# c976237222/HunyuanVideo_efficiency

Hardware: AMD Instinct MI355X
Metric: denoise-steps/sec (720x1280x129f, HunyuanVideo DiT 20+40 blocks, bf16) (higher is better)
Workload: dtype bf16

## Files before the change

### hunyuanvideo_efficiency_amd/csrc/hv_attention.hip

```cpp
#include "hv_attention.hpp"

using namespace hv_attn;

namespace {

constexpr int QTILE = 256;

__global__ __launch_bounds__(256) void attn_combine_kernel(const float* __restrict__ part_o, const float* __restrict__ part_ml,
                                                            bf16_t* __restrict__ o, int64_t so, int n_q, int n_heads, int n_splits) {
    const int64_t idx = (int64_t)blockIdx.x * blockDim.x + threadIdx.x;
    const int64_t total = (int64_t)n_q * n_heads * 32;
    if (idx >= total) return;
    const int d4 = (int)(idx & 31);
    const int64_t rh = idx >> 5;
    const int head = (int)(rh % n_heads);
    const int64_t row = rh / n_heads;
    float m = -INFINITY;
    for (int s = 0; s < n_splits; ++s) m = fmaxf(m, part_ml[(((int64_t)s * n_q + row) * n_heads + head) * 2]);
    float4 acc = make_float4(0.f, 0.f, 0.f, 0.f);
    float l = 0.f;
    for (int s = 0; s < n_splits; ++s) {
        const int64_t ri = ((int64_t)s * n_q + row) * n_heads + head;
        const float w = __builtin_amdgcn_exp2f(part_ml[ri * 2] - m);
        const float4 v = *reinterpret_cast<const float4*>(part_o + ri * D + d4 * 4);
        acc.x += v.x * w; acc.y += v.y * w; acc.z += v.z * w; acc.w += v.w * w;
        l += part_ml[ri * 2 + 1] * w;
    }
    const float inv = 1.0f / l;
    u32x2 w2;
    w2[0] = pack_bf2(acc.x * inv, acc.y * inv);
    w2[1] = pack_bf2(acc.z * inv, acc.w * inv);
    *reinterpret_cast<u32x2*>(o + row * so + head * D + d4 * 4) = w2;
}

int attn_launch(const AttnArgs& a, dim3 grid, hipStream_t stream) { return launch_w4(a, grid, stream); }

constexpr int KMAX_ROWS = 2048;
__global__ __launch_bounds__(256) void attn_kmax_kernel(const bf16_t* __restrict__ k, int64_t sk, int n_kv, unsigned* __restrict__ out) {
    __shared__ float wmax[4];
    const int head = blockIdx.y, t = threadIdx.x, ch = t & 15;
    const int r0 = blockIdx.x * KMAX_ROWS, r1 = min(r0 + KMAX_ROWS, n_kv);
    float best = 0.f;
    for (int row = r0 + (t >> 4); row < r1; row += 16) {
        const u32x4 w = *reinterpret_cast<const u32x4*>(k + (int64_t)row * sk + head * D + ch * 8);
        float s = 0.f;
#pragma unroll
        for (int j = 0; j < 4; ++j) {
            const float lo = bf2f_lo(w[j]), hi = bf2f_hi(w[j]);
            s += lo * lo + hi * hi;
        }
#pragma unroll
        for (int o = 8; o > 0; o >>= 1) s += __shfl_xor(s, o, 64);
        best = fmaxf(best, s);
    }
    best = fmaxf(best, __shfl_xor(best, 16, 64));
    best = fmaxf(best, __shfl_xor(best, 32, 64));
    if ((t & 63) == 0) wmax[t >> 6] = best;
    __syncthreads();
    if (t == 0) atomicMax(out + head, __float_as_uint(fmaxf(fmaxf(wmax[0], wmax[1]), fmaxf(wmax[2], wmax[3]))));
}

int attn_prepare_kmax(AttnArgs& a, void* workspace, int64_t workspace_bytes, hipStream_t stream) {
    static_assert(HV_ATTN_BOUND_MIN_KV == 64 * KVT, "the pre-pass pays from 64 key tiles on");
    a.kmax2 = nullptr;
    if (!workspace || workspace_bytes < KMAX_BYTES || a.n_heads > KMAX_HEADS || a.n_kv < HV_ATTN_BOUND_MIN_KV) return HV_OK;
    if (hipMemsetAsync(workspace, 0, KMAX_BYTES, stream) != hipSuccess) return HV_ERR_LAUNCH;
    attn_kmax_kernel<<<dim3((unsigned)((a.n_kv + KMAX_ROWS - 1) / KMAX_ROWS), (unsigned)a.n_heads), dim3(256), 0, stream>>>(a.k, a.sk, a.n_kv, (unsigned*)workspace);
    a.kmax2 = (const unsigned*)workspace;
    return HV_OK;
}

int attn_kv_splits(int n_q, int n_kv, int n_heads) {
    const int64_t nwg = (int64_t)((n_q + QTILE - 1) / QTILE) * n_heads;
    const int ntile = (n_kv + KVT - 1) / KVT;
    const double r1 = (double)((nwg + 255) / 256), r2 = 0.5 * (double)((2 * nwg + 255) / 256);
    return (ntile >= 64 && r2 < 0.97 * r1) ? 2 : 1;
}

}

extern "C" int64_t hv_attn_workspace_bytes(int n_q, int n_kv, int n_heads) {
    (void)n_kv;
    return (int64_t)KMAX_BYTES + (int64_t)2 * n_q * n_heads * (128 + 2) * (int64_t)sizeof(float);
}

extern "C" int hv_attn_fwd_bf16(const void* q, const void* k, const void* v, void* o, int64_t stride_q, int64_t stride_k,
                                int64_t stride_v, int64_t stride_o, int n_q, int n_kv, int n_heads, int head_dim,
                                float scale, void* workspace, int64_t workspace_bytes, hipStream_t stream) {
    if (!q || !k || !v || !o || head_dim != D || n_heads <= 0 || n_q < 0 || n_kv < 0 || (stride_q & 7) || (stride_k & 7) ||
        (stride_v & 7) || (stride_o & 3))
        return HV_ERR_ARG;
    if (n_q == 0) return HV_OK;
    if (n_kv == 0) return HV_ERR_ARG;
    AttnArgs a;
    a.q = (const bf16_t*)q; a.k = (const bf16_t*)k; a.v = (const bf16_t*)v; a.o = (bf16_t*)o;
    a.sq = stride_q; a.sk = stride_k; a.sv = stride_v; a.so = stride_o;
    a.n_q = n_q; a.n_kv = n_kv; a.n_heads = n_heads;
    a.n_qtiles = (n_q + QTILE - 1) / QTILE;
    a.scale_log2e = scale * 1.4426950408889634f;
    a.n_splits = 1; a.split_keys = n_kv; a.part_o = nullptr; a.part_ml = nullptr; a.partial = 0;
    if (attn_prepare_kmax(a, workspace, workspace_bytes, stream) != HV_OK) return HV_ERR_LAUNCH;
    if (workspace && attn_kv_splits(n_q, n_kv, n_heads) == 2 && workspace_bytes >= hv_attn_workspace_bytes(n_q, n_kv, n_heads)) {
        a.n_splits = 2;
        a.split_keys = (((n_kv + KVT - 1) / KVT + 1) / 2) * KVT;
        a.part_o = (float*)((char*)workspace + KMAX_BYTES);
        a.part_ml = a.part_o + (int64_t)2 * n_q * n_heads * D;
    }
    if (attn_launch(a, dim3((unsigned)(a.n_qtiles * n_heads), (unsigned)a.n_splits), stream) != HV_OK) return HV_ERR_LAUNCH;
    if (a.n_splits > 1) {
        const int64_t total = (int64_t)n_q * n_heads * 32;
        attn_combine_kernel<<<dim3((unsigned)((total + 255) / 256)), dim3(256), 0, stream>>>(a.part_o, a.part_ml, a.o, a.so, n_q, n_heads,
                                                                                           a.n_splits);
    }
    return hv_check_launch();
}

extern "C" int hv_attn_partial_bf16(const void* q, const void* k, const void* v, int64_t stride_q, int64_t stride_k, int64_t stride_v,
                                    int n_q, int n_kv, int n_heads, int head_dim, float scale, void* part_o, void* part_ml,
                                    int n_slots, int slot, int splits, hipStream_t stream) {
    if (!q || !k || !v || !part_o || !part_ml || head_dim != D || n_heads <= 0 || n_q < 0 || n_kv <= 0 || (stride_q & 7) ||
        (stride_k & 7) || (stride_v & 7) || (splits != 1 && splits != 2) || slot < 0 || slot + splits > n_slots)
        return HV_ERR_ARG;
    if (n_q == 0) return HV_OK;
    const int ntile = (n_kv + KVT - 1) / KVT;
    if (splits == 2 && ntile < 2) return HV_ERR_ARG;
    AttnArgs a;
    a.q = (const bf16_t*)q; a.k = (const bf16_t*)k; a.v = (const bf16_t*)v; a.o = nullptr;
    a.sq = stride_q; a.sk = stride_k; a.sv = stride_v; a.so = 0;
    a.n_q = n_q; a.n_kv = n_kv; a.n_heads = n_heads;
    a.n_qtiles = (n_q + QTILE - 1) / QTILE;
    a.scale_log2e = scale * 1.4426950408889634f;
    a.n_splits = splits;
    a.split_keys = splits == 2 ? ((ntile + 1) / 2) * KVT : n_kv;
    a.part_o = (float*)part_o + (int64_t)slot * n_q * n_heads * D;
    a.part_ml = (float*)part_ml + (int64_t)slot * n_q * n_heads * 2;
    a.partial = 1;
    a.kmax2 = nullptr;
    if (attn_launch(a, dim3((unsigned)(a.n_qtiles * n_heads), (unsigned)splits), stream) != HV_OK) return HV_ERR_LAUNCH;
    return hv_check_launch();
}

extern "C" int hv_attn_merge_bf16(const void* part_o, const void* part_ml, void* o, int64_t stride_o, int n_q, int n_heads, int n_slots,
                                  hipStream_t stream) {
    if (!part_o || !part_ml || !o || n_heads <= 0 || n_q < 0 || n_slots <= 0 || (stride_o & 3)) return HV_ERR_ARG;
    if (n_q == 0) return HV_OK;
    const int64_t total = (int64_t)n_q * n_heads * 32;
    attn_combine_kernel<<<dim3((unsigned)((total + 255) / 256)), dim3(256), 0, stream>>>((const float*)part_o, (const float*)part_ml,
                                                                                       (bf16_t*)o, stride_o, n_q, n_heads, n_slots);
    return hv_check_launch();
}

extern "C" int hv_attn_suggest_splits(int n_q, int n_kv, int n_heads) { return attn_kv_splits(n_q, n_kv, n_heads); }
```

### hunyuanvideo_efficiency_amd/csrc/hv_attention.hpp

```cpp
#pragma once
#include "hv_common.hpp"
#include "../../include/hv_kernels.h"
#include <type_traits>

namespace hv_attn {

constexpr int D = 128;
constexpr int KVT = 64;
constexpr int KV_TILE_BYTES = KVT * D * 2;

struct AttnArgs {
    const bf16_t* q; const bf16_t* k; const bf16_t* v; bf16_t* o;
    int64_t sq, sk, sv, so;
    int n_q, n_kv, n_heads, n_qtiles;
    float scale_log2e;
    int n_splits, split_keys;
    float* part_o;
    float* part_ml;
    int partial;
    const unsigned* kmax2;
};
constexpr int KMAX_BYTES = HV_ATTN_MIN_WORKSPACE_BYTES;
constexpr int KMAX_HEADS = 62;

typedef __attribute__((ext_vector_type(4))) short s16x4;
typedef __attribute__((address_space(3))) s16x4* lds_s16x4_ptr;
typedef __attribute__((address_space(3))) void* lds_void_ptr;

__device__ __forceinline__ float half_swap_max(float v) {
    auto r = __builtin_amdgcn_permlane32_swap(__float_as_uint(v), __float_as_uint(v), false, false);
    return fmaxf(__uint_as_float(r[0]), __uint_as_float(r[1]));
}
__device__ __forceinline__ float half_swap_sum(float v) {
    auto r = __builtin_amdgcn_permlane32_swap(__float_as_uint(v), __float_as_uint(v), false, false);
    return __uint_as_float(r[0]) + __uint_as_float(r[1]);
}

template <int I, int N, typename F>
__device__ __forceinline__ void static_for(F&& f) {
    if constexpr (I < N) {
        f(std::integral_constant<int, I>{});
        static_for<I + 1, N>(f);
    }
}

int launch_w4(const AttnArgs& a, dim3 grid, hipStream_t stream);

}
```

### hunyuanvideo_efficiency_amd/csrc/hv_common.hpp

```cpp
#pragma once
#include <hip/hip_runtime.h>
#include <stdint.h>

#define HV_OK 0
#define HV_ERR_ARG (-1)
#define HV_ERR_LAUNCH (-2)

typedef __attribute__((ext_vector_type(8))) __bf16 bf16x8;
typedef __attribute__((ext_vector_type(4))) __bf16 bf16x4;
typedef __attribute__((ext_vector_type(2))) __bf16 bf16x2;
typedef __attribute__((ext_vector_type(4))) float f32x4;
typedef __attribute__((ext_vector_type(16))) float f32x16;
typedef __attribute__((ext_vector_type(4))) uint32_t u32x4;
typedef __attribute__((ext_vector_type(2))) uint32_t u32x2;
typedef __attribute__((ext_vector_type(2))) float f32x2;

typedef uint16_t bf16_t;

__device__ __forceinline__ float bf2f(bf16_t v) { return __uint_as_float(((uint32_t)v) << 16); }
__device__ __forceinline__ float bf2f_lo(uint32_t w) { return __uint_as_float(w << 16); }
__device__ __forceinline__ float bf2f_hi(uint32_t w) { return __uint_as_float(w & 0xFFFF0000u); }
__device__ __forceinline__ bf16_t f2bf(float f) {
    __bf16 h = (__bf16)f;
    return __builtin_bit_cast(bf16_t, h);
}
__device__ __forceinline__ uint32_t pack_bf2(float lo, float hi) {
    bf16x2 v;
    v[0] = (__bf16)lo;
    v[1] = (__bf16)hi;
    return __builtin_bit_cast(uint32_t, v);
}
__device__ __forceinline__ float rbf(float f) { return bf2f(f2bf(f)); }

__device__ __forceinline__ void unpack8(const u32x4& w, float (&f)[8]) {
#pragma unroll
    for (int i = 0; i < 4; ++i) {
        f[2 * i] = bf2f_lo(w[i]);
        f[2 * i + 1] = bf2f_hi(w[i]);
    }
}
__device__ __forceinline__ u32x4 pack8(const float (&f)[8]) {
    u32x4 w;
#pragma unroll
    for (int i = 0; i < 4; ++i) w[i] = pack_bf2(f[2 * i], f[2 * i + 1]);
    return w;
}

typedef _Float16 h16;
__device__ __forceinline__ float h2f(uint16_t v) { return (float)__builtin_bit_cast(h16, v); }
__device__ __forceinline__ uint16_t f2h(float f) { return __builtin_bit_cast(uint16_t, (h16)f); }
__device__ __forceinline__ float rh(float f) { return (float)(h16)f; }
__device__ __forceinline__ void unpack8h(const u32x4& w, float (&f)[8]) {
#pragma unroll
    for (int i = 0; i < 4; ++i) {
        f[2 * i] = h2f((uint16_t)(w[i] & 0xFFFFu));
        f[2 * i + 1] = h2f((uint16_t)(w[i] >> 16));
    }
}
__device__ __forceinline__ u32x4 pack8h(const float (&f)[8]) {
    u32x4 w;
#pragma unroll
    for (int i = 0; i < 4; ++i) w[i] = (uint32_t)f2h(f[2 * i]) | ((uint32_t)f2h(f[2 * i + 1]) << 16);
    return w;
}

template <typename T, typename Op>
__device__ __forceinline__ T wave_reduce(T v, Op op) {
#pragma unroll
    for (int o = 32; o > 0; o >>= 1) v = op(v, __shfl_xor(v, o, 64));
    return v;
}
struct WaveAdd {
    template <typename T> __device__ __forceinline__ T operator()(T a, T b) const { return a + b; }
};
struct WaveMax {
    __device__ __forceinline__ float operator()(float a, float b) const { return fmaxf(a, b); }
    __device__ __forceinline__ int operator()(int a, int b) const { return max(a, b); }
};
struct WaveMin {
    __device__ __forceinline__ int operator()(int a, int b) const { return min(a, b); }
};
template <typename T> __device__ __forceinline__ T wave_sum(T v) { return wave_reduce(v, WaveAdd{}); }
template <typename T> __device__ __forceinline__ T wave_max(T v) { return wave_reduce(v, WaveMax{}); }
template <typename T> __device__ __forceinline__ T wave_min(T v) { return wave_reduce(v, WaveMin{}); }

__device__ __forceinline__ float gelu_tanh_f(float x) {
    const float k0 = 0.7978845608028654f, k1 = 0.044715f;
    float u = k0 * (x + k1 * x * x * x);
    float e = __builtin_amdgcn_exp2f(u * 2.8853900817779268f);
    float t = 1.0f - 2.0f * __builtin_amdgcn_rcpf(e + 1.0f);
    return 0.5f * x * (1.0f + t);
}
__device__ __forceinline__ float silu_f(float x) { return x * __builtin_amdgcn_rcpf(1.0f + __expf(-x)); }

__device__ __forceinline__ uint32_t quantise(float x, int rescale) {
    if (rescale) x = __fmul_rn(__fadd_rn(x, 1.0f), 0.5f);
    x = fminf(fmaxf(x, 0.0f), 1.0f);
    return (uint32_t)(int)__fmul_rn(x, 255.0f);
}

namespace f32tile {
constexpr int kThreads = 256;
constexpr int BM = 128, BN = 64, BK = 32;
constexpr int LDA = BM + 2;

__device__ __forceinline__ void mma_chunk(const float* sA, const float* sB, int wm, int wn, int lr, int lk, f32x16& acc0, f32x16& acc1) {
#pragma unroll
    for (int ks = 0; ks < BK / 2; ++ks) {
        const int k = ks * 2 + lk;
        const float a0 = sA[k * LDA + wm + lr], a1 = sA[k * LDA + wm + 32 + lr];
        const float b = sB[k * BN + wn + lr];
        acc0 = __builtin_amdgcn_mfma_f32_32x32x2f32(a0, b, acc0, 0, 0, 0);
        acc1 = __builtin_amdgcn_mfma_f32_32x32x2f32(a1, b, acc1, 0, 0, 0);
    }
}
__device__ __forceinline__ int acc_row(int r, int lk) { return (r & 3) + 8 * (r >> 2) + 4 * lk; }
}

static inline bool hv_aligned16(const void* p) { return ((uintptr_t)p & 15) == 0; }

struct HvPerDeviceOnce { bool done[64] = {}; };
static inline int hv_set_max_lds(HvPerDeviceOnce& once, const void* fn, int bytes) {
    int dev = 0;
    if (hipGetDevice(&dev) != hipSuccess || dev < 0 || dev >= 64) return HV_ERR_LAUNCH;
    if (!once.done[dev]) {
        if (hipFuncSetAttribute(fn, hipFuncAttributeMaxDynamicSharedMemorySize, bytes) != hipSuccess) return HV_ERR_LAUNCH;
        once.done[dev] = true;
    }
    return HV_OK;
}

static inline int hv_check_launch() {
    hipError_t e = hipGetLastError();
    return e == hipSuccess ? HV_OK : HV_ERR_LAUNCH;
}

__device__ __forceinline__ f32x2 f16x2_minus(uint32_t w, float plo, float phi) {
    float lo, hi;
    asm("v_fma_mix_f32 %0, %1, 1.0, -%2 op_sel_hi:[1,0,0]" : "=v"(lo) : "v"(w), "v"(plo));
    asm("v_fma_mix_f32 %0, %1, 1.0, -%2 op_sel:[1,0,0] op_sel_hi:[1,0,0]" : "=v"(hi) : "v"(w), "v"(phi));
    return f32x2{lo, hi};
}
```

### hunyuanvideo_efficiency_amd/csrc/hv_rowwise.hip

```cpp
#include "hv_common.hpp"
#include "../../include/hv_kernels.h"
#include <type_traits>


template <int MAXC>
__device__ __forceinline__ float ln_load_row(const bf16_t* xr, int lane, int nchunk, float (&v)[MAXC][8]) {
    float s = 0.f;
#pragma unroll
    for (int c = 0; c < MAXC; ++c) {
        const int ch = lane + c * 64;
        if (ch < nchunk) {
            unpack8(*reinterpret_cast<const u32x4*>(xr + ch * 8), v[c]);
#pragma unroll
            for (int j = 0; j < 8; ++j) s += v[c][j];
        }
    }
    return s;
}
__device__ __forceinline__ void ln_load_coeffs(const bf16_t* mul, const bf16_t* add, int ch, int mode,
                                               float (&m)[8], float (&a)[8]) {
    if (mul) {
        unpack8(*reinterpret_cast<const u32x4*>(mul + ch * 8), m);
        if (mode == 0) {
#pragma unroll
            for (int j = 0; j < 8; ++j) m[j] = rbf(1.0f + m[j]);
        }
    } else {
#pragma unroll
        for (int j = 0; j < 8; ++j) m[j] = 1.0f;
    }
    if (add) {
        unpack8(*reinterpret_cast<const u32x4*>(add + ch * 8), a);
    } else {
#pragma unroll
        for (int j = 0; j < 8; ++j) a[j] = 0.0f;
    }
}

template <int MAXC>
__global__ __launch_bounds__(256) void ln_mod_kernel(const bf16_t* __restrict__ x, const bf16_t* __restrict__ add,
                                                      const bf16_t* __restrict__ mul, bf16_t* __restrict__ out,
                                                      int64_t M, int D, int64_t ldx, int64_t ldo, float eps, int mode) {
    const int lane = threadIdx.x & 63;
    const int64_t row = (int64_t)blockIdx.x * 4 + (threadIdx.x >> 6);
    if (row >= M) return;
    const int nchunk = D >> 3;
    float v[MAXC][8];
    const float mean = wave_sum(ln_load_row<MAXC>(x + row * ldx, lane, nchunk, v)) / (float)D;
    float q = 0.f;
#pragma unroll
    for (int c = 0; c < MAXC; ++c) {
        const int ch = lane + c * 64;
        if (ch < nchunk) {
#pragma unroll
            for (int j = 0; j < 8; ++j) {
                float d = v[c][j] - mean;
                q += d * d;
            }
        }
    }
    const float rstd = rsqrtf(wave_sum(q) / (float)D + eps);
    bf16_t* orow = out + row * ldo;
#pragma unroll
    for (int c = 0; c < MAXC; ++c) {
        const int ch = lane + c * 64;
        if (ch < nchunk) {
            float m[8], a[8], o[8];
            ln_load_coeffs(mul, add, ch, mode, m, a);
#pragma unroll
            for (int j = 0; j < 8; ++j) o[j] = (v[c][j] - mean) * rstd * m[j] + a[j];
            *reinterpret_cast<u32x4*>(orow + ch * 8) = pack8(o);
        }
    }
}

template <typename Launch>
static inline void ln_dispatch_maxc(int D, Launch launch) {
    if (D <= 512)
        launch(std::integral_constant<int, 1>{});
    else if (D <= 2048)
        launch(std::integral_constant<int, 4>{});
    else if (D <= 3072)
        launch(std::integral_constant<int, 6>{});
    else
        launch(std::integral_constant<int, 8>{});
}

extern "C" int hv_ln_modulate_bf16(const void* x, const void* shift_or_bias, const void* scale_or_weight, void* out,
                                   int64_t M, int D, int64_t ldx, int64_t ldo, float eps, int mode, hipStream_t stream) {
    if (!x || !out || M < 0 || D <= 0 || (D & 7) || D > 4096 || (ldx & 7) || (ldo & 7) || (mode != 0 && mode != 1))
        return HV_ERR_ARG;
    if (M == 0) return HV_OK;
    dim3 grid((unsigned)((M + 3) / 4)), block(256);
    const bf16_t *xp = (const bf16_t*)x, *ap = (const bf16_t*)shift_or_bias, *mp = (const bf16_t*)scale_or_weight;
    ln_dispatch_maxc(D, [&](auto maxc) {
        ln_mod_kernel<decltype(maxc)::value><<<grid, block, 0, stream>>>(xp, ap, mp, (bf16_t*)out, M, D, ldx, ldo, eps, mode);
    });
    return hv_check_launch();
}

__device__ __forceinline__ uint32_t pack4_fp8(float a, float b, float c, float d) {
    uint32_t w = 0;
    w = __builtin_amdgcn_cvt_pk_fp8_f32(a, b, w, false);
    w = __builtin_amdgcn_cvt_pk_fp8_f32(c, d, w, true);
    return w;
}
constexpr float HV_FP8_MIN_ROW_SCALE = 1.17549435e-38f;
__device__ __forceinline__ float fp8_row_scale(float amax) {
    return amax > 0.f ? fmaxf(amax * (1.0f / 448.0f), HV_FP8_MIN_ROW_SCALE) : 1.0f;
}
__device__ __forceinline__ float clamp448(float v) { return __builtin_amdgcn_fmed3f(v, -448.0f, 448.0f); }
__device__ __forceinline__ u32x2 pack8_fp8(const float (&v)[8], float inv) {
    u32x2 w;
    w[0] = pack4_fp8(clamp448(v[0] * inv), clamp448(v[1] * inv), clamp448(v[2] * inv), clamp448(v[3] * inv));
    w[1] = pack4_fp8(clamp448(v[4] * inv), clamp448(v[5] * inv), clamp448(v[6] * inv), clamp448(v[7] * inv));
    return w;
}
template <int MAXC>
__global__ __launch_bounds__(256) void ln_mod_fp8_kernel(const bf16_t* __restrict__ x, const bf16_t* __restrict__ add,
                                                          const bf16_t* __restrict__ mul, uint8_t* __restrict__ out,
                                                          float* __restrict__ row_scale, int64_t M, int D, int64_t ldx,
                                                          int64_t ldo, float eps) {
    const int lane = threadIdx.x & 63;
    const int64_t row = (int64_t)blockIdx.x * 4 + (threadIdx.x >> 6);
    if (row >= M) return;
    const int nchunk = D >> 3;
    float v[MAXC][8];
    const float mean = wave_sum(ln_load_row<MAXC>(x + row * ldx, lane, nchunk, v)) / (float)D;
    float q = 0.f;
#pragma unroll
    for (int c = 0; c < MAXC; ++c) {
        const int ch = lane + c * 64;
        if (ch < nchunk) {
#pragma unroll
            for (int j = 0; j < 8; ++j) {
                float d = v[c][j] - mean;
                q += d * d;
            }
        }
    }
    const float rstd = rsqrtf(wave_sum(q) / (float)D + eps);
    float amax = 0.f;
#pragma unroll
    for (int c = 0; c < MAXC; ++c) {
        const int ch = lane + c * 64;
        if (ch < nchunk) {
            float m[8], a[8];
            ln_load_coeffs(mul, add, ch, 0, m, a);
#pragma unroll
            for (int j = 0; j < 8; ++j) {
                v[c][j] = rbf((v[c][j] - mean) * rstd * m[j] + a[j]);
                amax = fmaxf(amax, fabsf(v[c][j]));
            }
        }
    }
    const float sc = fp8_row_scale(wave_max(amax));
    const float inv = 1.0f / sc;
    if (lane == 0) row_scale[row] = sc;
    uint8_t* orow = out + row * ldo;
#pragma unroll
    for (int c = 0; c < MAXC; ++c) {
        const int ch = lane + c * 64;
        if (ch < nchunk) *reinterpret_cast<u32x2*>(orow + ch * 8) = pack8_fp8(v[c], inv);
    }
}

extern "C" int hv_ln_modulate_fp8(const void* x, const void* shift, const void* scale, void* out_q, float* out_row_scale, int64_t M,
                                  int D, int64_t ldx, int64_t ldq, float eps, hipStream_t stream) {
    if (!x || !out_q || !out_row_scale || M < 0 || D <= 0 || (D & 7) || D > 4096 || (ldx & 7) || (ldq & 15)) return HV_ERR_ARG;
    if (M == 0) return HV_OK;
    dim3 grid((unsigned)((M + 3) / 4)), block(256);
    const bf16_t *xp = (const bf16_t*)x, *ap = (const bf16_t*)shift, *mp = (const bf16_t*)scale;
    ln_dispatch_maxc(D, [&](auto maxc) {
        ln_mod_fp8_kernel<decltype(maxc)::value><<<grid, block, 0, stream>>>(xp, ap, mp, (uint8_t*)out_q, out_row_scale, M, D, ldx, ldq, eps);
    });
    return hv_check_launch();
}

__global__ __launch_bounds__(256) void quant_rows_fp8_kernel(const bf16_t* __restrict__ x, int64_t ldx, uint8_t* __restrict__ out,
                                                              int64_t ldo, float* __restrict__ row_scale, int64_t M, int K) {
    const int lane = threadIdx.x & 63;
    const int64_t row = (int64_t)blockIdx.x * 4 + (threadIdx.x >> 6);
    if (row >= M) return;
    const bf16_t* xr = x + row * ldx;
    const int nchunk = K >> 3;
    float amax = 0.f;
    for (int ch = lane; ch < nchunk; ch += 64) {
        float f[8];
        unpack8(*reinterpret_cast<const u32x4*>(xr + ch * 8), f);
#pragma unroll
        for (int j = 0; j < 8; ++j) amax = fmaxf(amax, fabsf(f[j]));
    }
    const float sc = fp8_row_scale(wave_max(amax));
    const float inv = 1.0f / sc;
    if (lane == 0) row_scale[row] = sc;
    uint8_t* orow = out + row * ldo;
    for (int ch = lane; ch < nchunk; ch += 64) {
        float f[8];
        unpack8(*reinterpret_cast<const u32x4*>(xr + ch * 8), f);
        *reinterpret_cast<u32x2*>(orow + ch * 8) = pack8_fp8(f, inv);
    }
}

extern "C" int hv_quant_rows_fp8(const void* x, int64_t ldx, void* out_q, int64_t ldq, float* out_row_scale, int64_t M, int K,
                                 hipStream_t stream) {
    if (!x || !out_q || !out_row_scale || M < 0 || K <= 0 || (K & 7) || (ldx & 7) || (ldq & 15)) return HV_ERR_ARG;
    if (M == 0) return HV_OK;
    quant_rows_fp8_kernel<<<dim3((unsigned)((M + 3) / 4)), dim3(256), 0, stream>>>((const bf16_t*)x, ldx, (uint8_t*)out_q, ldq,
                                                                                  out_row_scale, M, K);
    return hv_check_launch();
}

__global__ __launch_bounds__(256) void qknorm_rope_kernel(bf16_t* __restrict__ qkv, const bf16_t* __restrict__ qw,
                                                           const bf16_t* __restrict__ kw, const float* __restrict__ cosT,
                                                           const float* __restrict__ sinT, int64_t n_rows, int64_t n_rope,
                                                           int H, int64_t ld, int64_t k_off, float eps, bf16_t* __restrict__ dst,
                                                           int64_t dst_ld, int hpb, int64_t dst_bs) {
    const int64_t row = blockIdx.x;
    const int sub = threadIdx.x & 15;
    const int grp = threadIdx.x >> 4;
    float wq[8], wk[8], c[8], s[8];
    unpack8(*reinterpret_cast<const u32x4*>(qw + sub * 8), wq);
    unpack8(*reinterpret_cast<const u32x4*>(kw + sub * 8), wk);
    const bool rope = row < n_rope;
    if (rope) {
        const float4* cp = reinterpret_cast<const float4*>(cosT + row * 128 + sub * 8);
        const float4* sp = reinterpret_cast<const float4*>(sinT + row * 128 + sub * 8);
        float4 c0 = cp[0], c1 = cp[1], s0 = sp[0], s1 = sp[1];
        c[0] = c0.x, c[1] = c0.y, c[2] = c0.z, c[3] = c0.w, c[4] = c1.x, c[5] = c1.y, c[6] = c1.z, c[7] = c1.w;
        s[0] = s0.x, s[1] = s0.y, s[2] = s0.z, s[3] = s0.w, s[4] = s1.x, s[5] = s1.y, s[6] = s1.z, s[7] = s1.w;
    }
    for (int hv = grp; hv < 2 * H; hv += 16) {
        const bool is_k = hv >= H;
        const int h = is_k ? hv - H : hv;
        bf16_t* p = qkv + row * ld + (is_k ? k_off : 0) + h * 128 + sub * 8;
        float x[8];
        unpack8(*reinterpret_cast<const u32x4*>(p), x);
        if (dst) p = dst + (int64_t)(hv / hpb) * dst_bs + row * dst_ld + (hv % hpb) * 128 + sub * 8;
        float ss = 0.f;
#pragma unroll
        for (int j = 0; j < 8; ++j) ss += x[j] * x[j];
#pragma unroll
        for (int o = 8; o > 0; o >>= 1) ss += __shfl_xor(ss, o, 16);
        const float r = rsqrtf(ss * (1.0f / 128.0f) + eps);
        float y[8];
#pragma unroll
        for (int j = 0; j < 8; ++j) y[j] = rbf(rbf(x[j] * r) * (is_k ? wk[j] : wq[j]));
        if (rope) {
            float o[8];
#pragma unroll
            for (int j = 0; j < 8; j += 2) {
                o[j] = y[j] * c[j] - y[j + 1] * s[j];
                o[j + 1] = y[j + 1] * c[j + 1] + y[j] * s[j + 1];
            }
            *reinterpret_cast<u32x4*>(p) = pack8(o);
        } else {
            *reinterpret_cast<u32x4*>(p) = pack8(y);
        }
    }
}

extern "C" int hv_qknorm_rope_bf16(void* qkv, const void* q_weight, const void* k_weight, const float* cos_tab,
                                   const float* sin_tab, int64_t n_rows, int64_t n_rope, int n_heads, int head_dim,
                                   int64_t ld, int64_t k_offset, float eps, hipStream_t stream) {
    if (!qkv || !q_weight || !k_weight || head_dim != 128 || n_heads <= 0 || n_rows < 0 || n_rope < 0 ||
        n_rope > n_rows || (ld & 7) || (k_offset & 7) || (n_rope > 0 && (!cos_tab || !sin_tab)))
        return HV_ERR_ARG;
    if (n_rows == 0) return HV_OK;
    qknorm_rope_kernel<<<dim3((unsigned)n_rows), dim3(256), 0, stream>>>((bf16_t*)qkv, (const bf16_t*)q_weight,
                                                                          (const bf16_t*)k_weight, cos_tab, sin_tab, n_rows,
                                                                          n_rope, n_heads, ld, k_offset, eps, nullptr, 0, 1, 0);
    return hv_check_launch();
}

extern "C" int hv_qknorm_rope_scatter_bf16(const void* qkv, const void* q_weight, const void* k_weight, const float* cos_tab,
                                           const float* sin_tab, int64_t n_rows, int64_t n_rope, int n_heads, int head_dim,
                                           int64_t ld, int64_t k_offset, float eps, void* dst, int64_t dst_ld,
                                           int heads_per_block, int64_t dst_block_stride, hipStream_t stream) {
    if (!qkv || !dst || !q_weight || !k_weight || head_dim != 128 || n_heads <= 0 || n_rows < 0 || n_rope < 0 || n_rope > n_rows ||
        (ld & 7) || (k_offset & 7) || (dst_ld & 7) || (dst_block_stride & 7) || heads_per_block <= 0 ||
        (n_rope > 0 && (!cos_tab || !sin_tab)))
        return HV_ERR_ARG;
    if (n_rows == 0) return HV_OK;
    qknorm_rope_kernel<<<dim3((unsigned)n_rows), dim3(256), 0, stream>>>((bf16_t*)const_cast<void*>(qkv), (const bf16_t*)q_weight,
                                                                          (const bf16_t*)k_weight, cos_tab, sin_tab, n_rows, n_rope,
                                                                          n_heads, ld, k_offset, eps, (bf16_t*)dst, dst_ld,
                                                                          heads_per_block, dst_block_stride);
    return hv_check_launch();
}

template <int MM>
__global__ __launch_bounds__(256) void gemv_kernel(const bf16_t* __restrict__ x, const bf16_t* __restrict__ W,
                                                    const bf16_t* __restrict__ b, const bf16_t* __restrict__ addend,
                                                    bf16_t* __restrict__ out, int N, int K, int64_t ldx, int64_t ldo, int act) {
    const int lane = threadIdx.x & 63;
    const int n = blockIdx.x * 4 + (threadIdx.x >> 6);
    if (n >= N) return;
    float acc[MM];
#pragma unroll
    for (int m = 0; m < MM; ++m) acc[m] = 0.f;
    const bf16_t* wr = W + (int64_t)n * K;
    for (int k0 = lane * 8; k0 < K; k0 += 512) {
        float w[8];
        unpack8(*reinterpret_cast<const u32x4*>(wr + k0), w);
#pragma unroll
        for (int m = 0; m < MM; ++m) {
            float xv[8];
            unpack8(*reinterpret_cast<const u32x4*>(x + m * ldx + k0), xv);
#pragma unroll
            for (int j = 0; j < 8; ++j) {
                float a = xv[j];
                if (act & 1) a = rbf(silu_f(a));
                acc[m] += a * w[j];
            }
        }
    }
#pragma unroll
    for (int m = 0; m < MM; ++m) {
        float r = wave_sum(acc[m]);
        if (lane == 0) {
            if (b) r += bf2f(b[n]);
            if (act & 2) r = silu_f(rbf(r));
            if (addend) r = rbf(r) + bf2f(addend[m * ldo + n]);
            out[m * ldo + n] = f2bf(r);
        }
    }
}

extern "C" int hv_linear_smallm_bf16(const void* x, const void* W, const void* bias, const void* addend, void* out, int M,
                                     int N, int K, int64_t ldx, int64_t ldo, int act, hipStream_t stream) {
    if (!x || !W || !out || M < 1 || M > 4 || N < 1 || K < 8 || (K & 7) || (ldx & 7)) return HV_ERR_ARG;
    dim3 grid((N + 3) / 4), block(256);
    const bf16_t *xp = (const bf16_t*)x, *wp = (const bf16_t*)W, *bp = (const bf16_t*)bias, *ap = (const bf16_t*)addend;
    bf16_t* op = (bf16_t*)out;
    switch (M) {
        case 1: gemv_kernel<1><<<grid, block, 0, stream>>>(xp, wp, bp, ap, op, N, K, ldx, ldo, act); break;
        case 2: gemv_kernel<2><<<grid, block, 0, stream>>>(xp, wp, bp, ap, op, N, K, ldx, ldo, act); break;
        case 3: gemv_kernel<3><<<grid, block, 0, stream>>>(xp, wp, bp, ap, op, N, K, ldx, ldo, act); break;
        default: gemv_kernel<4><<<grid, block, 0, stream>>>(xp, wp, bp, ap, op, N, K, ldx, ldo, act); break;
    }
    return hv_check_launch();
}

__global__ __launch_bounds__(256) void patchify_kernel(const float* __restrict__ x, bf16_t* __restrict__ A, int C, int T,
                                                        int H, int W) {
    const int Hp = H >> 1, Wp = W >> 1;
    const int64_t ntok = (int64_t)T * Hp * Wp;
    const int64_t idx = (int64_t)blockIdx.x * blockDim.x + threadIdx.x;
    if (idx >= ntok * C) return;
    const int c = (int)(idx % C);
    const int64_t tok = idx / C;
    const int w = (int)(tok % Wp), h = (int)((tok / Wp) % Hp), t = (int)(tok / ((int64_t)Wp * Hp));
    const float* p = x + (((int64_t)c * T + t) * H + 2 * h) * W + 2 * w;
    float2 r0 = *reinterpret_cast<const float2*>(p);
    float2 r1 = *reinterpret_cast<const float2*>(p + W);
    u32x2 o;
    o[0] = pack_bf2(r0.x, r0.y);
    o[1] = pack_bf2(r1.x, r1.y);
    *reinterpret_cast<u32x2*>(A + tok * (C * 4) + c * 4) = o;
}

extern "C" int hv_patchify_f32_bf16(const float* x, void* A, int C, int T, int H, int W, hipStream_t stream) {
    if (!x || !A || C <= 0 || T <= 0 || H <= 0 || W <= 0 || (H & 1) || (W & 1)) return HV_ERR_ARG;
    const int64_t n = (int64_t)T * (H / 2) * (W / 2) * C;
    patchify_kernel<<<dim3((unsigned)((n + 255) / 256)), dim3(256), 0, stream>>>(x, (bf16_t*)A, C, T, H, W);
    return hv_check_launch();
}

__global__ __launch_bounds__(256) void unpatchify_kernel(const bf16_t* __restrict__ y, bf16_t* __restrict__ out, int C,
                                                          int T, int H, int W, int64_t ldy) {
    const int Hp = H >> 1, Wp = W >> 1;
    const int64_t ntok = (int64_t)T * Hp * Wp;
    const int64_t idx = (int64_t)blockIdx.x * blockDim.x + threadIdx.x;
    if (idx >= ntok * C) return;
    const int64_t tok = idx % ntok;
    const int c = (int)(idx / ntok);
    const int w = (int)(tok % Wp), h = (int)((tok / Wp) % Hp), t = (int)(tok / ((int64_t)Wp * Hp));
    u32x2 v = *reinterpret_cast<const u32x2*>(y + tok * ldy + c * 4);
    bf16_t* p = out + (((int64_t)c * T + t) * H + 2 * h) * W + 2 * w;
    *reinterpret_cast<uint32_t*>(p) = v[0];
    *reinterpret_cast<uint32_t*>(p + W) = v[1];
}

extern "C" int hv_unpatchify_bf16(const void* y, void* out, int C, int T, int H, int W, int64_t ldy, hipStream_t stream) {
    if (!y || !out || C <= 0 || T <= 0 || (H & 1) || (W & 1) || (ldy & 3)) return HV_ERR_ARG;
    const int64_t n = (int64_t)T * (H / 2) * (W / 2) * C;
    unpatchify_kernel<<<dim3((unsigned)((n + 255) / 256)), dim3(256), 0, stream>>>((const bf16_t*)y, (bf16_t*)out, C, T, H,
                                                                                  W, ldy);
    return hv_check_launch();
}

__global__ __launch_bounds__(256) void euler_kernel(float* __restrict__ s, const bf16_t* __restrict__ v, float dt, int64_t n) {
    const int64_t i = ((int64_t)blockIdx.x * blockDim.x + threadIdx.x) * 4;
    if (i + 3 < n) {
        float4 a = *reinterpret_cast<float4*>(s + i);
        u32x2 w = *reinterpret_cast<const u32x2*>(v + i);
        a.x += bf2f_lo(w[0]) * dt, a.y += bf2f_hi(w[0]) * dt, a.z += bf2f_lo(w[1]) * dt, a.w += bf2f_hi(w[1]) * dt;
        *reinterpret_cast<float4*>(s + i) = a;
    } else {
        for (int64_t j = i; j < n; ++j) s[j] += bf2f(v[j]) * dt;
    }
}

extern "C" int hv_euler_step_f32(float* sample, const void* model_out_bf16, float dt, int64_t n, hipStream_t stream) {
    if (!sample || !model_out_bf16 || n < 0) return HV_ERR_ARG;
    if (n == 0) return HV_OK;
    euler_kernel<<<dim3((unsigned)((n / 4 + 256) / 256)), dim3(256), 0, stream>>>(sample, (const bf16_t*)model_out_bf16, dt, n);
    return hv_check_launch();
}

__global__ __launch_bounds__(256) void euler_f32_kernel(float* __restrict__ s, const float* __restrict__ v, float dt, int64_t n) {
    const int64_t i = ((int64_t)blockIdx.x * blockDim.x + threadIdx.x) * 4;
    if (i + 3 < n) {
        float4 a = *reinterpret_cast<float4*>(s + i);
        const float4 b = *reinterpret_cast<const float4*>(v + i);
        a.x += b.x * dt, a.y += b.y * dt, a.z += b.z * dt, a.w += b.w * dt;
        *reinterpret_cast<float4*>(s + i) = a;
    } else {
        for (int64_t j = i; j < n; ++j) s[j] += v[j] * dt;
    }
}

extern "C" int hv_euler_step_f32_f32(float* sample, const float* model_out_f32, float dt, int64_t n, hipStream_t stream) {
    if (!sample || !model_out_f32 || n < 0) return HV_ERR_ARG;
    if (n == 0) return HV_OK;
    euler_f32_kernel<<<dim3((unsigned)((n / 4 + 256) / 256)), dim3(256), 0, stream>>>(sample, model_out_f32, dt, n);
    return hv_check_launch();
}

__global__ __launch_bounds__(256) void masked_mean_kernel(const bf16_t* __restrict__ x, const int* __restrict__ mask,
                                                           bf16_t* __restrict__ out, int L, int D) {
    const int d = blockIdx.x * blockDim.x + threadIdx.x;
    if (d >= D) return;
    float s = 0.f, c = 0.f;
    for (int l = 0; l < L; ++l) {
        const float m = mask ? (float)mask[l] : 1.0f;
        s += bf2f(x[(int64_t)l * D + d]) * m;
        c += m;
    }
    out[d] = f2bf(s / c);
}

extern "C" int hv_masked_mean_bf16(const void* x, const int* mask, void* out, int L, int D, hipStream_t stream) {
    if (!x || !out || L <= 0 || D <= 0) return HV_ERR_ARG;
    masked_mean_kernel<<<dim3((D + 255) / 256), dim3(256), 0, stream>>>((const bf16_t*)x, mask, (bf16_t*)out, L, D);
    return hv_check_launch();
}

__global__ __launch_bounds__(256) void bcast_row_kernel(const bf16_t* __restrict__ src, bf16_t* __restrict__ dst, int64_t n,
                                                         int D, int64_t ld) {
    const int64_t i = (int64_t)blockIdx.x * blockDim.x + threadIdx.x;
    if (i >= n * D) return;
    dst[(i / D) * ld + (i % D)] = src[i % D];
}

extern "C" int hv_broadcast_row_bf16(const void* src, void* dst, int64_t n_rows, int D, int64_t ld, hipStream_t stream) {
    if (!src || !dst || n_rows < 0 || D <= 0) return HV_ERR_ARG;
    if (n_rows == 0) return HV_OK;
    bcast_row_kernel<<<dim3((unsigned)((n_rows * D + 255) / 256)), dim3(256), 0, stream>>>((const bf16_t*)src, (bf16_t*)dst,
                                                                                          n_rows, D, ld);
    return hv_check_launch();
}

__global__ void timestep_embedding_kernel(const float* __restrict__ t, bf16_t* __restrict__ out, int n_t, int dim, float max_period) {
    const int half = dim >> 1;
    const int idx = blockIdx.x * blockDim.x + threadIdx.x;
    if (idx >= n_t * half) return;
    const int b = idx / half, i = idx % half;
    const float f = expf(-logf(max_period) * (float)i / (float)half);
    const float a = t[b] * f;
    out[b * dim + i] = f2bf(cosf(a));
    out[b * dim + half + i] = f2bf(sinf(a));
}

extern "C" int hv_timestep_embedding_bf16(const float* t, void* out, int n_t, int dim, float max_period, hipStream_t stream) {
    if (!t || !out || n_t <= 0 || dim <= 0 || (dim & 1)) return HV_ERR_ARG;
    const int n = n_t * (dim / 2);
    timestep_embedding_kernel<<<dim3((n + 127) / 128), dim3(128), 0, stream>>>(t, (bf16_t*)out, n_t, dim, max_period);
    return hv_check_launch();
}

__global__ __launch_bounds__(256) void copy3d_kernel(const bf16_t* __restrict__ src, bf16_t* __restrict__ dst, int rows,
                                                      int cvec, int64_t src_bs, int64_t src_ld, int64_t dst_bs, int64_t dst_ld) {
    const int b = blockIdx.z;
    const int64_t total = (int64_t)rows * cvec;
    for (int64_t i = (int64_t)blockIdx.x * blockDim.x + threadIdx.x; i < total; i += (int64_t)gridDim.x * blockDim.x) {
        const int64_t r = i / cvec;
        const int c = (int)(i % cvec) * 8;
        *reinterpret_cast<u32x4*>(dst + b * dst_bs + r * dst_ld + c) =
            *reinterpret_cast<const u32x4*>(src + b * src_bs + r * src_ld + c);
    }
}

extern "C" int hv_copy3d_bf16(const void* src, void* dst, int n_batch, int64_t rows, int cols, int64_t src_batch_stride,
                              int64_t src_ld, int64_t dst_batch_stride, int64_t dst_ld, hipStream_t stream) {
    if (!src || !dst || n_batch < 0 || rows < 0 || cols <= 0 || (cols & 7) || (src_ld & 7) || (dst_ld & 7) ||
        (src_batch_stride & 7) || (dst_batch_stride & 7) || rows > 0x7fffffff)
        return HV_ERR_ARG;
    if (n_batch == 0 || rows == 0) return HV_OK;
    const int64_t total = rows * (cols / 8);
    const unsigned gx = (unsigned)((total + 255) / 256 > 4096 ? 4096 : (total + 255) / 256);
    copy3d_kernel<<<dim3(gx, 1, (unsigned)n_batch), dim3(256), 0, stream>>>((const bf16_t*)src, (bf16_t*)dst, (int)rows, cols / 8,
                                                                            src_batch_stride, src_ld, dst_batch_stride, dst_ld);
    return hv_check_launch();
}

__device__ __forceinline__ float e4m3fn_to_f32(uint32_t b) {
    const uint32_t s = (b & 0x80u) << 24, e = (b >> 3) & 0xFu, m = b & 7u;
    float v;
    if (e == 0) v = (float)m * 0.001953125f;
    else if (e == 15 && m == 7) v = __uint_as_float(0x7FC00000u);
    else v = __uint_as_float(((e + 120u) << 23) | (m << 20));
    return __uint_as_float(__float_as_uint(v) | s);
}

__global__ __launch_bounds__(256) void fp8_dequant_kernel(const uint8_t* __restrict__ w8, const bf16_t* __restrict__ scale,
                                                           bf16_t* __restrict__ out, int64_t n) {
    const float sc = bf2f(scale[0]);
    for (int64_t i = ((int64_t)blockIdx.x * blockDim.x + threadIdx.x) * 8; i < n; i += (int64_t)gridDim.x * blockDim.x * 8) {
        if (i + 8 <= n) {
            const u32x2 p = *reinterpret_cast<const u32x2*>(w8 + i);
            float f[8];
#pragma unroll
            for (int j = 0; j < 8; ++j) f[j] = e4m3fn_to_f32((p[j >> 2] >> ((j & 3) * 8)) & 0xFFu) * sc;
            *reinterpret_cast<u32x4*>(out + i) = pack8(f);
        } else {
            for (int64_t j = i; j < n; ++j) out[j] = f2bf(e4m3fn_to_f32(w8[j]) * sc);
        }
    }
}

extern "C" int hv_fp8_dequant_bf16(const void* w_e4m3fn, const void* scale_bf16, void* out_bf16, int64_t n, hipStream_t stream) {
    if (!w_e4m3fn || !scale_bf16 || !out_bf16 || n <= 0 || (n & 7)) return HV_ERR_ARG;
    const int64_t nv = n / 8;
    const unsigned gx = (unsigned)((nv + 255) / 256 > 16384 ? 16384 : (nv + 255) / 256);
    fp8_dequant_kernel<<<dim3(gx), dim3(256), 0, stream>>>((const uint8_t*)w_e4m3fn, (const bf16_t*)scale_bf16, (bf16_t*)out_bf16, n);
    return hv_check_launch();
}
```

### hunyuanvideo_efficiency_amd/csrc/hv_torch_ops.cpp

```cpp
#include <torch/library.h>
#include <ATen/core/Tensor.h>
#include <c10/hip/HIPStream.h>
#include <c10/hip/HIPGuard.h>
#include <optional>
#include <vector>
#include "../../include/hv_kernels.h"

namespace {
using OptT = std::optional<at::Tensor>;

struct Dev {
    c10::DeviceIndex idx = -1;
    const char* op;
    explicit Dev(const char* o) : op(o) {}
    void* p(const OptT& t, const char* name) {
        if (!t.has_value() || !t->defined()) return nullptr;
        TORCH_CHECK(t->is_cuda(), "hv::", op, ": ", name, " must be a GPU tensor (this library has no CPU path), got ", t->device());
        if (idx < 0) idx = t->device().index();
        TORCH_CHECK(t->device().index() == idx, "hv::", op, ": ", name, " is on a different GPU than the other tensors");
        return t->data_ptr();
    }
};

inline void check_rc(int rc, const char* op) {
    TORCH_CHECK(rc == 0, "hv::", op, " failed with code ", rc, rc == -1 ? " (bad argument)" : rc == -2 ? " (launch failure)" : "");
}

int64_t op_abi_version() {
    return (int64_t)hv_abi_version();
}

void op_ln_modulate_bf16(const OptT& x, const OptT& shift_or_bias, const OptT& scale_or_weight, const OptT& out, int64_t M, int64_t D, int64_t ldx, int64_t ldo, double eps, int64_t mode) {
    Dev dev("ln_modulate_bf16");
    auto a0 = (const void*)dev.p(x, "x");
    auto a1 = (const void*)dev.p(shift_or_bias, "shift_or_bias");
    auto a2 = (const void*)dev.p(scale_or_weight, "scale_or_weight");
    auto a3 = (void*)dev.p(out, "out");
    TORCH_CHECK(dev.idx >= 0, "hv::ln_modulate_bf16: needs at least one GPU tensor");
    c10::hip::HIPGuard guard(dev.idx);
    hipStream_t stream = c10::hip::getCurrentHIPStream(dev.idx).stream();
    check_rc(hv_ln_modulate_bf16(a0, a1, a2, a3, (int64_t)M, (int)D, (int64_t)ldx, (int64_t)ldo, (float)eps, (int)mode, stream), "ln_modulate_bf16");
}

void op_qknorm_rope_bf16(const OptT& qkv, const OptT& q_weight, const OptT& k_weight, const OptT& cos_tab, const OptT& sin_tab, int64_t n_rows, int64_t n_rope, int64_t n_heads, int64_t head_dim, int64_t ld, int64_t k_offset, double eps) {
    Dev dev("qknorm_rope_bf16");
    auto a0 = (void*)dev.p(qkv, "qkv");
    auto a1 = (const void*)dev.p(q_weight, "q_weight");
    auto a2 = (const void*)dev.p(k_weight, "k_weight");
    auto a3 = (const float*)dev.p(cos_tab, "cos_tab");
    auto a4 = (const float*)dev.p(sin_tab, "sin_tab");
    TORCH_CHECK(dev.idx >= 0, "hv::qknorm_rope_bf16: needs at least one GPU tensor");
    c10::hip::HIPGuard guard(dev.idx);
    hipStream_t stream = c10::hip::getCurrentHIPStream(dev.idx).stream();
    check_rc(hv_qknorm_rope_bf16(a0, a1, a2, a3, a4, (int64_t)n_rows, (int64_t)n_rope, (int)n_heads, (int)head_dim, (int64_t)ld, (int64_t)k_offset, (float)eps, stream), "qknorm_rope_bf16");
}

void op_qknorm_rope_scatter_bf16(const OptT& qkv, const OptT& q_weight, const OptT& k_weight, const OptT& cos_tab, const OptT& sin_tab, int64_t n_rows, int64_t n_rope, int64_t n_heads, int64_t head_dim, int64_t ld, int64_t k_offset, double eps, const OptT& dst, int64_t dst_ld, int64_t heads_per_block, int64_t dst_block_stride) {
    Dev dev("qknorm_rope_scatter_bf16");
    auto a0 = (const void*)dev.p(qkv, "qkv");
    auto a1 = (const void*)dev.p(q_weight, "q_weight");
    auto a2 = (const void*)dev.p(k_weight, "k_weight");
    auto a3 = (const float*)dev.p(cos_tab, "cos_tab");
    auto a4 = (const float*)dev.p(sin_tab, "sin_tab");
    auto a12 = (void*)dev.p(dst, "dst");
    TORCH_CHECK(dev.idx >= 0, "hv::qknorm_rope_scatter_bf16: needs at least one GPU tensor");
    c10::hip::HIPGuard guard(dev.idx);
    hipStream_t stream = c10::hip::getCurrentHIPStream(dev.idx).stream();
    check_rc(hv_qknorm_rope_scatter_bf16(a0, a1, a2, a3, a4, (int64_t)n_rows, (int64_t)n_rope, (int)n_heads, (int)head_dim, (int64_t)ld, (int64_t)k_offset, (float)eps, a12, (int64_t)dst_ld, (int)heads_per_block, (int64_t)dst_block_stride, stream), "qknorm_rope_scatter_bf16");
}

void op_gemm_bf16(const OptT& A, int64_t lda, const OptT& W, int64_t ldw, const OptT& bias, int64_t M, int64_t N, int64_t K, const OptT& out0, int64_t ld0, int64_t act0, int64_t n_split, const OptT& out1, int64_t ld1, int64_t act1, const OptT& gate, const OptT& res, int64_t ld_res) {
    Dev dev("gemm_bf16");
    auto a0 = (const void*)dev.p(A, "A");
    auto a2 = (const void*)dev.p(W, "W");
    auto a4 = (const void*)dev.p(bias, "bias");
    auto a8 = (void*)dev.p(out0, "out0");
    auto a12 = (void*)dev.p(out1, "out1");
    auto a15 = (const void*)dev.p(gate, "gate");
    auto a16 = (const void*)dev.p(res, "res");
    TORCH_CHECK(dev.idx >= 0, "hv::gemm_bf16: needs at least one GPU tensor");
    c10::hip::HIPGuard guard(dev.idx);
    hipStream_t stream = c10::hip::getCurrentHIPStream(dev.idx).stream();
    check_rc(hv_gemm_bf16(a0, (int64_t)lda, a2, (int64_t)ldw, a4, (int)M, (int)N, (int)K, a8, (int64_t)ld0, (int)act0, (int)n_split, a12, (int64_t)ld1, (int)act1, a15, a16, (int64_t)ld_res, stream), "gemm_bf16");
}

void op_linear_smallm_bf16(const OptT& x, const OptT& W, const OptT& bias, const OptT& addend, const OptT& out, int64_t M, int64_t N, int64_t K, int64_t ldx, int64_t ldo, int64_t act) {
    Dev dev("linear_smallm_bf16");
    auto a0 = (const void*)dev.p(x, "x");
    auto a1 = (const void*)dev.p(W, "W");
    auto a2 = (const void*)dev.p(bias, "bias");
    auto a3 = (const void*)dev.p(addend, "addend");
    auto a4 = (void*)dev.p(out, "out");
    TORCH_CHECK(dev.idx >= 0, "hv::linear_smallm_bf16: needs at least one GPU tensor");
    c10::hip::HIPGuard guard(dev.idx);
    hipStream_t stream = c10::hip::getCurrentHIPStream(dev.idx).stream();
    check_rc(hv_linear_smallm_bf16(a0, a1, a2, a3, a4, (int)M, (int)N, (int)K, (int64_t)ldx, (int64_t)ldo, (int)act, stream), "linear_smallm_bf16");
}

void op_timestep_embedding_bf16(const OptT& t, const OptT& out, int64_t n_t, int64_t dim, double max_period) {
    Dev dev("timestep_embedding_bf16");
    auto a0 = (const float*)dev.p(t, "t");
    auto a1 = (void*)dev.p(out, "out");
    TORCH_CHECK(dev.idx >= 0, "hv::timestep_embedding_bf16: needs at least one GPU tensor");
    c10::hip::HIPGuard guard(dev.idx);
    hipStream_t stream = c10::hip::getCurrentHIPStream(dev.idx).stream();
    check_rc(hv_timestep_embedding_bf16(a0, a1, (int)n_t, (int)dim, (float)max_period, stream), "timestep_embedding_bf16");
}

void op_attn_fwd_bf16(const OptT& q, const OptT& k, const OptT& v, const OptT& o, int64_t stride_q, int64_t stride_k, int64_t stride_v, int64_t stride_o, int64_t n_q, int64_t n_kv, int64_t n_heads, int64_t head_dim, double scale, const OptT& workspace, int64_t workspace_bytes) {
    Dev dev("attn_fwd_bf16");
    auto a0 = (const void*)dev.p(q, "q");
    auto a1 = (const void*)dev.p(k, "k");
    auto a2 = (const void*)dev.p(v, "v");
    auto a3 = (void*)dev.p(o, "o");
    auto a13 = (void*)dev.p(workspace, "workspace");
    TORCH_CHECK(dev.idx >= 0, "hv::attn_fwd_bf16: needs at least one GPU tensor");
    c10::hip::HIPGuard guard(dev.idx);
    hipStream_t stream = c10::hip::getCurrentHIPStream(dev.idx).stream();
    check_rc(hv_attn_fwd_bf16(a0, a1, a2, a3, (int64_t)stride_q, (int64_t)stride_k, (int64_t)stride_v, (int64_t)stride_o, (int)n_q, (int)n_kv, (int)n_heads, (int)head_dim, (float)scale, a13, (int64_t)workspace_bytes, stream), "attn_fwd_bf16");
}

int64_t op_attn_workspace_bytes(int64_t n_q, int64_t n_kv, int64_t n_heads) {
    return (int64_t)hv_attn_workspace_bytes((int)n_q, (int)n_kv, (int)n_heads);
}

int64_t op_attn_w4_loop_signature() {
    return (int64_t)hv_attn_w4_loop_signature();
}

void op_attn_partial_bf16(const OptT& q, const OptT& k, const OptT& v, int64_t stride_q, int64_t stride_k, int64_t stride_v, int64_t n_q, int64_t n_kv, int64_t n_heads, int64_t head_dim, double scale, const OptT& part_o, const OptT& part_ml, int64_t n_slots, int64_t slot, int64_t splits) {
    Dev dev("attn_partial_bf16");
    auto a0 = (const void*)dev.p(q, "q");
    auto a1 = (const void*)dev.p(k, "k");
    auto a2 = (const void*)dev.p(v, "v");
    auto a11 = (void*)dev.p(part_o, "part_o");
    auto a12 = (void*)dev.p(part_ml, "part_ml");
    TORCH_CHECK(dev.idx >= 0, "hv::attn_partial_bf16: needs at least one GPU tensor");
    c10::hip::HIPGuard guard(dev.idx);
    hipStream_t stream = c10::hip::getCurrentHIPStream(dev.idx).stream();
    check_rc(hv_attn_partial_bf16(a0, a1, a2, (int64_t)stride_q, (int64_t)stride_k, (int64_t)stride_v, (int)n_q, (int)n_kv, (int)n_heads, (int)head_dim, (float)scale, a11, a12, (int)n_slots, (int)slot, (int)splits, stream), "attn_partial_bf16");
}

void op_attn_merge_bf16(const OptT& part_o, const OptT& part_ml, const OptT& o, int64_t stride_o, int64_t n_q, int64_t n_heads, int64_t n_slots) {
    Dev dev("attn_merge_bf16");
    auto a0 = (const void*)dev.p(part_o, "part_o");
    auto a1 = (const void*)dev.p(part_ml, "part_ml");
    auto a2 = (void*)dev.p(o, "o");
    TORCH_CHECK(dev.idx >= 0, "hv::attn_merge_bf16: needs at least one GPU tensor");
    c10::hip::HIPGuard guard(dev.idx);
    hipStream_t stream = c10::hip::getCurrentHIPStream(dev.idx).stream();
    check_rc(hv_attn_merge_bf16(a0, a1, a2, (int64_t)stride_o, (int)n_q, (int)n_heads, (int)n_slots, stream), "attn_merge_bf16");
}

int64_t op_attn_suggest_splits(int64_t n_q, int64_t n_kv, int64_t n_heads) {
    return (int64_t)hv_attn_suggest_splits((int)n_q, (int)n_kv, (int)n_heads);
}

void op_patchify_f32_bf16(const OptT& x, const OptT& A, int64_t C, int64_t T, int64_t H, int64_t W) {
    Dev dev("patchify_f32_bf16");
    auto a0 = (const float*)dev.p(x, "x");
    auto a1 = (void*)dev.p(A, "A");
    TORCH_CHECK(dev.idx >= 0, "hv::patchify_f32_bf16: needs at least one GPU tensor");
    c10::hip::HIPGuard guard(dev.idx);
    hipStream_t stream = c10::hip::getCurrentHIPStream(dev.idx).stream();
    check_rc(hv_patchify_f32_bf16(a0, a1, (int)C, (int)T, (int)H, (int)W, stream), "patchify_f32_bf16");
}

void op_unpatchify_bf16(const OptT& y, const OptT& out, int64_t C, int64_t T, int64_t H, int64_t W, int64_t ldy) {
    Dev dev("unpatchify_bf16");
    auto a0 = (const void*)dev.p(y, "y");
    auto a1 = (void*)dev.p(out, "out");
    TORCH_CHECK(dev.idx >= 0, "hv::unpatchify_bf16: needs at least one GPU tensor");
    c10::hip::HIPGuard guard(dev.idx);
    hipStream_t stream = c10::hip::getCurrentHIPStream(dev.idx).stream();
    check_rc(hv_unpatchify_bf16(a0, a1, (int)C, (int)T, (int)H, (int)W, (int64_t)ldy, stream), "unpatchify_bf16");
}

void op_euler_step_f32(const OptT& sample, const OptT& model_out_bf16, double dt, int64_t n) {
    Dev dev("euler_step_f32");
    auto a0 = (float*)dev.p(sample, "sample");
    auto a1 = (const void*)dev.p(model_out_bf16, "model_out_bf16");
    TORCH_CHECK(dev.idx >= 0, "hv::euler_step_f32: needs at least one GPU tensor");
    c10::hip::HIPGuard guard(dev.idx);
    hipStream_t stream = c10::hip::getCurrentHIPStream(dev.idx).stream();
    check_rc(hv_euler_step_f32(a0, a1, (float)dt, (int64_t)n, stream), "euler_step_f32");
}

void op_euler_step_f32_f32(const OptT& sample, const OptT& model_out_f32, double dt, int64_t n) {
    Dev dev("euler_step_f32_f32");
    auto a0 = (float*)dev.p(sample, "sample");
    auto a1 = (const float*)dev.p(model_out_f32, "model_out_f32");
    TORCH_CHECK(dev.idx >= 0, "hv::euler_step_f32_f32: needs at least one GPU tensor");
    c10::hip::HIPGuard guard(dev.idx);
    hipStream_t stream = c10::hip::getCurrentHIPStream(dev.idx).stream();
    check_rc(hv_euler_step_f32_f32(a0, a1, (float)dt, (int64_t)n, stream), "euler_step_f32_f32");
}

void op_masked_mean_bf16(const OptT& x, const OptT& mask, const OptT& out, int64_t L, int64_t D) {
    Dev dev("masked_mean_bf16");
    auto a0 = (const void*)dev.p(x, "x");
    auto a1 = (const int*)dev.p(mask, "mask");
    auto a2 = (void*)dev.p(out, "out");
    TORCH_CHECK(dev.idx >= 0, "hv::masked_mean_bf16: needs at least one GPU tensor");
    c10::hip::HIPGuard guard(dev.idx);
    hipStream_t stream = c10::hip::getCurrentHIPStream(dev.idx).stream();
    check_rc(hv_masked_mean_bf16(a0, a1, a2, (int)L, (int)D, stream), "masked_mean_bf16");
}

void op_broadcast_row_bf16(const OptT& src, const OptT& dst, int64_t n_rows, int64_t D, int64_t ld) {
    Dev dev("broadcast_row_bf16");
    auto a0 = (const void*)dev.p(src, "src");
    auto a1 = (void*)dev.p(dst, "dst");
    TORCH_CHECK(dev.idx >= 0, "hv::broadcast_row_bf16: needs at least one GPU tensor");
    c10::hip::HIPGuard guard(dev.idx);
    hipStream_t stream = c10::hip::getCurrentHIPStream(dev.idx).stream();
    check_rc(hv_broadcast_row_bf16(a0, a1, (int64_t)n_rows, (int)D, (int64_t)ld, stream), "broadcast_row_bf16");
}

void op_copy3d_bf16(const OptT& src, const OptT& dst, int64_t n_batch, int64_t rows, int64_t cols, int64_t src_batch_stride, int64_t src_ld, int64_t dst_batch_stride, int64_t dst_ld) {
    Dev dev("copy3d_bf16");
    auto a0 = (const void*)dev.p(src, "src");
    auto a1 = (void*)dev.p(dst, "dst");
    TORCH_CHECK(dev.idx >= 0, "hv::copy3d_bf16: needs at least one GPU tensor");
    c10::hip::HIPGuard guard(dev.idx);
    hipStream_t stream = c10::hip::getCurrentHIPStream(dev.idx).stream();
    check_rc(hv_copy3d_bf16(a0, a1, (int)n_batch, (int64_t)rows, (int)cols, (int64_t)src_batch_stride, (int64_t)src_ld, (int64_t)dst_batch_stride, (int64_t)dst_ld, stream), "copy3d_bf16");
}

void op_fp8_dequant_bf16(const OptT& w_e4m3fn, const OptT& scale_bf16, const OptT& out_bf16, int64_t n) {
    Dev dev("fp8_dequant_bf16");
    auto a0 = (const void*)dev.p(w_e4m3fn, "w_e4m3fn");
    auto a1 = (const void*)dev.p(scale_bf16, "scale_bf16");
    auto a2 = (void*)dev.p(out_bf16, "out_bf16");
    TORCH_CHECK(dev.idx >= 0, "hv::fp8_dequant_bf16: needs at least one GPU tensor");
    c10::hip::HIPGuard guard(dev.idx);
    hipStream_t stream = c10::hip::getCurrentHIPStream(dev.idx).stream();
    check_rc(hv_fp8_dequant_bf16(a0, a1, a2, (int64_t)n, stream), "fp8_dequant_bf16");
}

void op_ln_modulate_fp8(const OptT& x, const OptT& shift, const OptT& scale, const OptT& out_q, const OptT& out_row_scale, int64_t M, int64_t D, int64_t ldx, int64_t ldq, double eps) {
    Dev dev("ln_modulate_fp8");
    auto a0 = (const void*)dev.p(x, "x");
    auto a1 = (const void*)dev.p(shift, "shift");
    auto a2 = (const void*)dev.p(scale, "scale");
    auto a3 = (void*)dev.p(out_q, "out_q");
    auto a4 = (float*)dev.p(out_row_scale, "out_row_scale");
    TORCH_CHECK(dev.idx >= 0, "hv::ln_modulate_fp8: needs at least one GPU tensor");
    c10::hip::HIPGuard guard(dev.idx);
    hipStream_t stream = c10::hip::getCurrentHIPStream(dev.idx).stream();
    check_rc(hv_ln_modulate_fp8(a0, a1, a2, a3, a4, (int64_t)M, (int)D, (int64_t)ldx, (int64_t)ldq, (float)eps, stream), "ln_modulate_fp8");
}

void op_quant_rows_fp8(const OptT& x, int64_t ldx, const OptT& out_q, int64_t ldq, const OptT& out_row_scale, int64_t M, int64_t K) {
    Dev dev("quant_rows_fp8");
    auto a0 = (const void*)dev.p(x, "x");
    auto a2 = (void*)dev.p(out_q, "out_q");
    auto a4 = (float*)dev.p(out_row_scale, "out_row_scale");
    TORCH_CHECK(dev.idx >= 0, "hv::quant_rows_fp8: needs at least one GPU tensor");
    c10::hip::HIPGuard guard(dev.idx);
    hipStream_t stream = c10::hip::getCurrentHIPStream(dev.idx).stream();
    check_rc(hv_quant_rows_fp8(a0, (int64_t)ldx, a2, (int64_t)ldq, a4, (int64_t)M, (int)K, stream), "quant_rows_fp8");
}

void op_gemm_fp8(const OptT& A_q, int64_t lda, const OptT& a_row_scale, const OptT& W_q, int64_t ldw, const OptT& w_scale_bf16, const OptT& bias, int64_t M, int64_t N, int64_t K, const OptT& out0, int64_t ld0, int64_t act0, int64_t n_split, const OptT& out1, int64_t ld1, int64_t act1, const OptT& gate, const OptT& res, int64_t ld_res) {
    Dev dev("gemm_fp8");
    auto a0 = (const void*)dev.p(A_q, "A_q");
    auto a2 = (const float*)dev.p(a_row_scale, "a_row_scale");
    auto a3 = (const void*)dev.p(W_q, "W_q");
    auto a5 = (const void*)dev.p(w_scale_bf16, "w_scale_bf16");
    auto a6 = (const void*)dev.p(bias, "bias");
    auto a10 = (void*)dev.p(out0, "out0");
    auto a14 = (void*)dev.p(out1, "out1");
    auto a17 = (const void*)dev.p(gate, "gate");
    auto a18 = (const void*)dev.p(res, "res");
    TORCH_CHECK(dev.idx >= 0, "hv::gemm_fp8: needs at least one GPU tensor");
    c10::hip::HIPGuard guard(dev.idx);
    hipStream_t stream = c10::hip::getCurrentHIPStream(dev.idx).stream();
    check_rc(hv_gemm_fp8(a0, (int64_t)lda, a2, a3, (int64_t)ldw, a5, a6, (int)M, (int)N, (int)K, a10, (int64_t)ld0, (int)act0, (int)n_split, a14, (int64_t)ld1, (int)act1, a17, a18, (int64_t)ld_res, stream), "gemm_fp8");
}

void op_gemm_f16(const OptT& A, int64_t lda, const OptT& W, int64_t ldw, const OptT& bias, int64_t M, int64_t N, int64_t K, const OptT& out, int64_t ldo, int64_t out_is_f32, const OptT& res, int64_t ld_res) {
    Dev dev("gemm_f16");
    auto a0 = (const void*)dev.p(A, "A");
    auto a2 = (const void*)dev.p(W, "W");
    auto a4 = (const void*)dev.p(bias, "bias");
    auto a8 = (void*)dev.p(out, "out");
    auto a11 = (const void*)dev.p(res, "res");
    TORCH_CHECK(dev.idx >= 0, "hv::gemm_f16: needs at least one GPU tensor");
    c10::hip::HIPGuard guard(dev.idx);
    hipStream_t stream = c10::hip::getCurrentHIPStream(dev.idx).stream();
    check_rc(hv_gemm_f16(a0, (int64_t)lda, a2, (int64_t)ldw, a4, (int)M, (int)N, (int)K, a8, (int64_t)ldo, (int)out_is_f32, a11, (int64_t)ld_res, stream), "gemm_f16");
}

void op_conv3d_causal_f16(const OptT& x, int64_t ldx, const OptT& w_taps, const OptT& bias, const OptT& out, int64_t ldo, int64_t T, int64_t H, int64_t W, int64_t Cin, int64_t Cout, int64_t up_t, int64_t up_hw, const OptT& res, int64_t ld_res, const OptT& gn_partial, int64_t gn_partial_floats) {
    Dev dev("conv3d_causal_f16");
    auto a0 = (const void*)dev.p(x, "x");
    auto a2 = (const void*)dev.p(w_taps, "w_taps");
    auto a3 = (const void*)dev.p(bias, "bias");
    auto a4 = (void*)dev.p(out, "out");
    auto a13 = (const void*)dev.p(res, "res");
    auto a15 = (float*)dev.p(gn_partial, "gn_partial");
    TORCH_CHECK(dev.idx >= 0, "hv::conv3d_causal_f16: needs at least one GPU tensor");
    c10::hip::HIPGuard guard(dev.idx);
    hipStream_t stream = c10::hip::getCurrentHIPStream(dev.idx).stream();
    check_rc(hv_conv3d_causal_f16(a0, (int64_t)ldx, a2, a3, a4, (int64_t)ldo, (int)T, (int)H, (int)W, (int)Cin, (int)Cout, (int)up_t, (int)up_hw, a13, (int64_t)ld_res, a15, (int64_t)gn_partial_floats, stream), "conv3d_causal_f16");
}

int64_t op_gn_partial_rows(int64_t M) {
    return (int64_t)hv_gn_partial_rows((int64_t)M);
}

int64_t op_subpixel_gn_partial_rows(int64_t sT, int64_t sH, int64_t sW, int64_t up_t) {
    return (int64_t)hv_subpixel_gn_partial_rows((int)sT, (int)sH, (int)sW, (int)up_t);
}

void op_conv3d_upsampled_subpixel_f16(const OptT& x, int64_t ldx, const OptT& w_sub, const OptT& tap_table, int64_t ntap, const OptT& bias, const OptT& out, int64_t ldo, int64_t sT, int64_t sH, int64_t sW, int64_t Cin, int64_t Cout, int64_t up_t, const OptT& gn_partial, int64_t gn_partial_floats) {
    Dev dev("conv3d_upsampled_subpixel_f16");
    auto a0 = (const void*)dev.p(x, "x");
    auto a2 = (const void*)dev.p(w_sub, "w_sub");
    auto a3 = (const void*)dev.p(tap_table, "tap_table");
    auto a5 = (const void*)dev.p(bias, "bias");
    auto a6 = (void*)dev.p(out, "out");
    auto a14 = (float*)dev.p(gn_partial, "gn_partial");
    TORCH_CHECK(dev.idx >= 0, "hv::conv3d_upsampled_subpixel_f16: needs at least one GPU tensor");
    c10::hip::HIPGuard guard(dev.idx);
    hipStream_t stream = c10::hip::getCurrentHIPStream(dev.idx).stream();
    check_rc(hv_conv3d_upsampled_subpixel_f16(a0, (int64_t)ldx, a2, a3, (int)ntap, a5, a6, (int64_t)ldo, (int)sT, (int)sH, (int)sW, (int)Cin, (int)Cout, (int)up_t, a14, (int64_t)gn_partial_floats, stream), "conv3d_upsampled_subpixel_f16");
}

void op_conv3d_cout4_f16(const OptT& x, int64_t ldx, const OptT& affine, int64_t silu, const OptT& w_frag, const OptT& bias, const OptT& out, int64_t ldo, int64_t T, int64_t H, int64_t W, int64_t Cin, int64_t Cout, const OptT& planes, int64_t planes_floats) {
    Dev dev("conv3d_cout4_f16");
    auto a0 = (const void*)dev.p(x, "x");
    auto a2 = (const float*)dev.p(affine, "affine");
    auto a4 = (const void*)dev.p(w_frag, "w_frag");
    auto a5 = (const void*)dev.p(bias, "bias");
    auto a6 = (void*)dev.p(out, "out");
    auto a13 = (float*)dev.p(planes, "planes");
    TORCH_CHECK(dev.idx >= 0, "hv::conv3d_cout4_f16: needs at least one GPU tensor");
    c10::hip::HIPGuard guard(dev.idx);
    hipStream_t stream = c10::hip::getCurrentHIPStream(dev.idx).stream();
    check_rc(hv_conv3d_cout4_f16(a0, (int64_t)ldx, a2, (int)silu, a4, a5, a6, (int64_t)ldo, (int)T, (int)H, (int)W, (int)Cin, (int)Cout, a13, (int64_t)planes_floats, stream), "conv3d_cout4_f16");
}

int64_t op_conv3d_cout4_planes_floats(int64_t M) {
    return (int64_t)hv_conv3d_cout4_planes_floats((int64_t)M);
}

void op_conv3d_causal_strided_f16(const OptT& x, int64_t ldx, const OptT& w_taps, const OptT& bias, const OptT& out, int64_t ldo, int64_t sT, int64_t sH, int64_t sW, int64_t Cin, int64_t Cout, int64_t stride_t, int64_t stride_h, int64_t stride_w) {
    Dev dev("conv3d_causal_strided_f16");
    auto a0 = (const void*)dev.p(x, "x");
    auto a2 = (const void*)dev.p(w_taps, "w_taps");
    auto a3 = (const void*)dev.p(bias, "bias");
    auto a4 = (void*)dev.p(out, "out");
    TORCH_CHECK(dev.idx >= 0, "hv::conv3d_causal_strided_f16: needs at least one GPU tensor");
    c10::hip::HIPGuard guard(dev.idx);
    hipStream_t stream = c10::hip::getCurrentHIPStream(dev.idx).stream();
    check_rc(hv_conv3d_causal_strided_f16(a0, (int64_t)ldx, a2, a3, a4, (int64_t)ldo, (int)sT, (int)sH, (int)sW, (int)Cin, (int)Cout, (int)stride_t, (int)stride_h, (int)stride_w, stream), "conv3d_causal_strided_f16");
}

void op_temporal_resample_f16(const OptT& x, int64_t ldx, const OptT& out, int64_t ldo, int64_t T_in, int64_t HW, int64_t C, int64_t mode, int64_t k, int64_t s) {
    Dev dev("temporal_resample_f16");
    auto a0 = (const void*)dev.p(x, "x");
    auto a2 = (void*)dev.p(out, "out");
    TORCH_CHECK(dev.idx >= 0, "hv::temporal_resample_f16: needs at least one GPU tensor");
    c10::hip::HIPGuard guard(dev.idx);
    hipStream_t stream = c10::hip::getCurrentHIPStream(dev.idx).stream();
    check_rc(hv_temporal_resample_f16(a0, (int64_t)ldx, a2, (int64_t)ldo, (int)T_in, (int64_t)HW, (int)C, (int)mode, (int)k, (int)s, stream), "temporal_resample_f16");
}

void op_groupnorm_affine_f16(const OptT& x, int64_t ldx, int64_t M, int64_t C, int64_t groups, double eps, const OptT& weight, const OptT& bias, const OptT& partial_ws, int64_t partial_ws_floats, const OptT& affine_out) {
    Dev dev("groupnorm_affine_f16");
    auto a0 = (const void*)dev.p(x, "x");
    auto a6 = (const void*)dev.p(weight, "weight");
    auto a7 = (const void*)dev.p(bias, "bias");
    auto a8 = (float*)dev.p(partial_ws, "partial_ws");
    auto a10 = (float*)dev.p(affine_out, "affine_out");
    TORCH_CHECK(dev.idx >= 0, "hv::groupnorm_affine_f16: needs at least one GPU tensor");
    c10::hip::HIPGuard guard(dev.idx);
    hipStream_t stream = c10::hip::getCurrentHIPStream(dev.idx).stream();
    check_rc(hv_groupnorm_affine_f16(a0, (int64_t)ldx, (int64_t)M, (int)C, (int)groups, (float)eps, a6, a7, a8, (int64_t)partial_ws_floats, a10, stream), "groupnorm_affine_f16");
}

void op_groupnorm_finalize_f16(const OptT& partial, int64_t partial_floats, int64_t nrow, int64_t M, int64_t C, int64_t groups, double eps, const OptT& weight, const OptT& bias, const OptT& affine_out) {
    Dev dev("groupnorm_finalize_f16");
    auto a0 = (const float*)dev.p(partial, "partial");
    auto a7 = (const void*)dev.p(weight, "weight");
    auto a8 = (const void*)dev.p(bias, "bias");
    auto a9 = (float*)dev.p(affine_out, "affine_out");
    TORCH_CHECK(dev.idx >= 0, "hv::groupnorm_finalize_f16: needs at least one GPU tensor");
    c10::hip::HIPGuard guard(dev.idx);
    hipStream_t stream = c10::hip::getCurrentHIPStream(dev.idx).stream();
    check_rc(hv_groupnorm_finalize_f16(a0, (int64_t)partial_floats, (int64_t)nrow, (int64_t)M, (int)C, (int)groups, (float)eps, a7, a8, a9, stream), "groupnorm_finalize_f16");
}

void op_groupnorm_apply_f16(const OptT& x, int64_t ldx, const OptT& y, int64_t ldy, int64_t M, int64_t C, const OptT& affine, int64_t silu) {
    Dev dev("groupnorm_apply_f16");
    auto a0 = (const void*)dev.p(x, "x");
    auto a2 = (void*)dev.p(y, "y");
    auto a6 = (const float*)dev.p(affine, "affine");
    TORCH_CHECK(dev.idx >= 0, "hv::groupnorm_apply_f16: needs at least one GPU tensor");
    c10::hip::HIPGuard guard(dev.idx);
    hipStream_t stream = c10::hip::getCurrentHIPStream(dev.idx).stream();
    check_rc(hv_groupnorm_apply_f16(a0, (int64_t)ldx, a2, (int64_t)ldy, (int64_t)M, (int)C, a6, (int)silu, stream), "groupnorm_apply_f16");
}

void op_softmax_rows_f32_f16(const OptT& S, int64_t ld_s, const OptT& P, int64_t ld_p, int64_t rows, int64_t cols, int64_t cols_pad, double scale, int64_t causal_block) {
    Dev dev("softmax_rows_f32_f16");
    auto a0 = (const float*)dev.p(S, "S");
    auto a2 = (void*)dev.p(P, "P");
    TORCH_CHECK(dev.idx >= 0, "hv::softmax_rows_f32_f16: needs at least one GPU tensor");
    c10::hip::HIPGuard guard(dev.idx);
    hipStream_t stream = c10::hip::getCurrentHIPStream(dev.idx).stream();
    check_rc(hv_softmax_rows_f32_f16(a0, (int64_t)ld_s, a2, (int64_t)ld_p, (int)rows, (int)cols, (int)cols_pad, (float)scale, (int)causal_block, stream), "softmax_rows_f32_f16");
}

void op_transpose_16b(const OptT& src, int64_t ld_src, const OptT& dst, int64_t ld_dst, int64_t R, int64_t C) {
    Dev dev("transpose_16b");
    auto a0 = (const void*)dev.p(src, "src");
    auto a2 = (void*)dev.p(dst, "dst");
    TORCH_CHECK(dev.idx >= 0, "hv::transpose_16b: needs at least one GPU tensor");
    c10::hip::HIPGuard guard(dev.idx);
    hipStream_t stream = c10::hip::getCurrentHIPStream(dev.idx).stream();
    check_rc(hv_transpose_16b(a0, (int64_t)ld_src, a2, (int64_t)ld_dst, (int)R, (int)C, stream), "transpose_16b");
}

void op_vae_latent_tile_f16(const OptT& z, int64_t sc, int64_t st, int64_t sh, int64_t sw, int64_t C, int64_t T, int64_t H, int64_t W, int64_t Cpad, const OptT& out) {
    Dev dev("vae_latent_tile_f16");
    auto a0 = (const float*)dev.p(z, "z");
    auto a10 = (void*)dev.p(out, "out");
    TORCH_CHECK(dev.idx >= 0, "hv::vae_latent_tile_f16: needs at least one GPU tensor");
    c10::hip::HIPGuard guard(dev.idx);
    hipStream_t stream = c10::hip::getCurrentHIPStream(dev.idx).stream();
    check_rc(hv_vae_latent_tile_f16(a0, (int64_t)sc, (int64_t)st, (int64_t)sh, (int64_t)sw, (int)C, (int)T, (int)H, (int)W, (int)Cpad, a10, stream), "vae_latent_tile_f16");
}

void op_vae_blend_f16(const OptT& a, at::IntArrayRef a_strides, const OptT& b, at::IntArrayRef b_strides, at::IntArrayRef dims, int64_t axis, int64_t extent) {
    Dev dev("vae_blend_f16");
    TORCH_CHECK(a_strides.size() == 4, "hv::vae_blend_f16: a_strides must have 4 elements, got ", a_strides.size());
    TORCH_CHECK(b_strides.size() == 4, "hv::vae_blend_f16: b_strides must have 4 elements, got ", b_strides.size());
    TORCH_CHECK(dims.size() == 4, "hv::vae_blend_f16: dims must have 4 elements, got ", dims.size());
    std::vector<int> dims_i(dims.begin(), dims.end());
    auto a0 = (const void*)dev.p(a, "a");
    auto a2 = (void*)dev.p(b, "b");
    TORCH_CHECK(dev.idx >= 0, "hv::vae_blend_f16: needs at least one GPU tensor");
    c10::hip::HIPGuard guard(dev.idx);
    hipStream_t stream = c10::hip::getCurrentHIPStream(dev.idx).stream();
    check_rc(hv_vae_blend_f16(a0, a_strides.data(), a2, b_strides.data(), dims_i.data(), (int)axis, (int)extent, stream), "vae_blend_f16");
}

void op_copy4d_16b(const OptT& src, at::IntArrayRef src_strides, const OptT& dst, at::IntArrayRef dst_strides, at::IntArrayRef dims) {
    Dev dev("copy4d_16b");
    TORCH_CHECK(src_strides.size() == 4, "hv::copy4d_16b: src_strides must have 4 elements, got ", src_strides.size());
    TORCH_CHECK(dst_strides.size() == 4, "hv::copy4d_16b: dst_strides must have 4 elements, got ", dst_strides.size());
    TORCH_CHECK(dims.size() == 4, "hv::copy4d_16b: dims must have 4 elements, got ", dims.size());
    std::vector<int> dims_i(dims.begin(), dims.end());
    auto a0 = (const void*)dev.p(src, "src");
    auto a2 = (void*)dev.p(dst, "dst");
    TORCH_CHECK(dev.idx >= 0, "hv::copy4d_16b: needs at least one GPU tensor");
    c10::hip::HIPGuard guard(dev.idx);
    hipStream_t stream = c10::hip::getCurrentHIPStream(dev.idx).stream();
    check_rc(hv_copy4d_16b(a0, src_strides.data(), a2, dst_strides.data(), dims_i.data(), stream), "copy4d_16b");
}

void op_vae_postprocess_f16_f32(const OptT& x, const OptT& out, int64_t n) {
    Dev dev("vae_postprocess_f16_f32");
    auto a0 = (const void*)dev.p(x, "x");
    auto a1 = (float*)dev.p(out, "out");
    TORCH_CHECK(dev.idx >= 0, "hv::vae_postprocess_f16_f32: needs at least one GPU tensor");
    c10::hip::HIPGuard guard(dev.idx);
    hipStream_t stream = c10::hip::getCurrentHIPStream(dev.idx).stream();
    check_rc(hv_vae_postprocess_f16_f32(a0, a1, (int64_t)n, stream), "vae_postprocess_f16_f32");
}

void op_video_metrics(const OptT& a, int64_t a_sc, int64_t a_st, int64_t a_sh, const OptT& b, int64_t b_sc, int64_t b_st, int64_t b_sh, int64_t dtype, int64_t C, int64_t T, int64_t H, int64_t W, int64_t rescale, int64_t passes, const OptT& sse, const OptT& minmax, const OptT& ssim_sum, const OptT& workspace, int64_t workspace_bytes) {
    Dev dev("video_metrics");
    auto a0 = (const void*)dev.p(a, "a");
    auto a4 = (const void*)dev.p(b, "b");
    auto a15 = (void*)dev.p(sse, "sse");
    auto a16 = (void*)dev.p(minmax, "minmax");
    auto a17 = (void*)dev.p(ssim_sum, "ssim_sum");
    auto a18 = (void*)dev.p(workspace, "workspace");
    TORCH_CHECK(dev.idx >= 0, "hv::video_metrics: needs at least one GPU tensor");
    c10::hip::HIPGuard guard(dev.idx);
    hipStream_t stream = c10::hip::getCurrentHIPStream(dev.idx).stream();
    check_rc(hv_video_metrics(a0, (int64_t)a_sc, (int64_t)a_st, (int64_t)a_sh, a4, (int64_t)b_sc, (int64_t)b_st, (int64_t)b_sh, (int)dtype, (int)C, (int)T, (int)H, (int)W, (int)rescale, (int)passes, a15, a16, a17, a18, (int64_t)workspace_bytes, stream), "video_metrics");
}

int64_t op_video_metrics_workspace_bytes(int64_t C, int64_t T, int64_t H, int64_t W) {
    return (int64_t)hv_video_metrics_workspace_bytes((int)C, (int)T, (int)H, (int)W);
}

void op_lpips_conv1_f32(const OptT& a, int64_t a_sc, int64_t a_st, int64_t a_sh, const OptT& b, int64_t b_sc, int64_t b_st, int64_t b_sh, int64_t dtype, int64_t T, int64_t H, int64_t W, int64_t rescale, const OptT& lut, const OptT& w, const OptT& bias, const OptT& y) {
    Dev dev("lpips_conv1_f32");
    auto a0 = (const void*)dev.p(a, "a");
    auto a4 = (const void*)dev.p(b, "b");
    auto a13 = (const float*)dev.p(lut, "lut");
    auto a14 = (const float*)dev.p(w, "w");
    auto a15 = (const float*)dev.p(bias, "bias");
    auto a16 = (float*)dev.p(y, "y");
    TORCH_CHECK(dev.idx >= 0, "hv::lpips_conv1_f32: needs at least one GPU tensor");
    c10::hip::HIPGuard guard(dev.idx);
    hipStream_t stream = c10::hip::getCurrentHIPStream(dev.idx).stream();
    check_rc(hv_lpips_conv1_f32(a0, (int64_t)a_sc, (int64_t)a_st, (int64_t)a_sh, a4, (int64_t)b_sc, (int64_t)b_st, (int64_t)b_sh, (int)dtype, (int)T, (int)H, (int)W, (int)rescale, a13, a14, a15, a16, stream), "lpips_conv1_f32");
}

void op_lpips_conv2d_f32(const OptT& x, const OptT& w, const OptT& bias, const OptT& y, int64_t N, int64_t H, int64_t W, int64_t Cin, int64_t Cout, int64_t ksize, int64_t pad) {
    Dev dev("lpips_conv2d_f32");
    auto a0 = (const float*)dev.p(x, "x");
    auto a1 = (const float*)dev.p(w, "w");
    auto a2 = (const float*)dev.p(bias, "bias");
    auto a3 = (float*)dev.p(y, "y");
    TORCH_CHECK(dev.idx >= 0, "hv::lpips_conv2d_f32: needs at least one GPU tensor");
    c10::hip::HIPGuard guard(dev.idx);
    hipStream_t stream = c10::hip::getCurrentHIPStream(dev.idx).stream();
    check_rc(hv_lpips_conv2d_f32(a0, a1, a2, a3, (int)N, (int)H, (int)W, (int)Cin, (int)Cout, (int)ksize, (int)pad, stream), "lpips_conv2d_f32");
}

void op_lpips_maxpool_f32(const OptT& x, const OptT& y, int64_t N, int64_t H, int64_t W, int64_t C) {
    Dev dev("lpips_maxpool_f32");
    auto a0 = (const float*)dev.p(x, "x");
    auto a1 = (float*)dev.p(y, "y");
    TORCH_CHECK(dev.idx >= 0, "hv::lpips_maxpool_f32: needs at least one GPU tensor");
    c10::hip::HIPGuard guard(dev.idx);
    hipStream_t stream = c10::hip::getCurrentHIPStream(dev.idx).stream();
    check_rc(hv_lpips_maxpool_f32(a0, a1, (int)N, (int)H, (int)W, (int)C, stream), "lpips_maxpool_f32");
}

void op_lpips_distance_f32(const OptT& f, const OptT& lin, int64_t T, int64_t P, int64_t C, int64_t layer, const OptT& out, const OptT& workspace, int64_t workspace_bytes) {
    Dev dev("lpips_distance_f32");
    auto a0 = (const float*)dev.p(f, "f");
    auto a1 = (const float*)dev.p(lin, "lin");
    auto a6 = (double*)dev.p(out, "out");
    auto a7 = (void*)dev.p(workspace, "workspace");
    TORCH_CHECK(dev.idx >= 0, "hv::lpips_distance_f32: needs at least one GPU tensor");
    c10::hip::HIPGuard guard(dev.idx);
    hipStream_t stream = c10::hip::getCurrentHIPStream(dev.idx).stream();
    check_rc(hv_lpips_distance_f32(a0, a1, (int)T, (int64_t)P, (int)C, (int)layer, a6, a7, (int64_t)workspace_bytes, stream), "lpips_distance_f32");
}

int64_t op_lpips_distance_workspace_bytes(int64_t T, int64_t P) {
    return (int64_t)hv_lpips_distance_workspace_bytes((int)T, (int64_t)P);
}

void op_temporal_spectrum(const OptT& x, int64_t sc, int64_t st, int64_t sh, int64_t dtype, int64_t mode, int64_t C, int64_t T, int64_t H, int64_t W, int64_t rescale, int64_t wr, int64_t wg, int64_t wb, int64_t round, int64_t shift, const OptT& twiddle, int64_t twiddle_floats, const OptT& mag_sum, const OptT& pow_sum, const OptT& workspace, int64_t workspace_bytes) {
    Dev dev("temporal_spectrum");
    auto a0 = (const void*)dev.p(x, "x");
    auto a16 = (const float*)dev.p(twiddle, "twiddle");
    auto a18 = (double*)dev.p(mag_sum, "mag_sum");
    auto a19 = (double*)dev.p(pow_sum, "pow_sum");
    auto a20 = (void*)dev.p(workspace, "workspace");
    TORCH_CHECK(dev.idx >= 0, "hv::temporal_spectrum: needs at least one GPU tensor");
    c10::hip::HIPGuard guard(dev.idx);
    hipStream_t stream = c10::hip::getCurrentHIPStream(dev.idx).stream();
    check_rc(hv_temporal_spectrum(a0, (int64_t)sc, (int64_t)st, (int64_t)sh, (int)dtype, (int)mode, (int)C, (int)T, (int)H, (int)W, (int)rescale, (int)wr, (int)wg, (int)wb, (int)round, (int)shift, a16, (int64_t)twiddle_floats, a18, a19, a20, (int64_t)workspace_bytes, stream), "temporal_spectrum");
}

int64_t op_temporal_spectrum_workspace_bytes(int64_t mode, int64_t C, int64_t T, int64_t H, int64_t W) {
    return (int64_t)hv_temporal_spectrum_workspace_bytes((int)mode, (int)C, (int)T, (int)H, (int)W);
}

void op_i3d_preprocess(const OptT& x, int64_t x_sc, int64_t x_st, int64_t x_sh, int64_t dtype, int64_t T, int64_t H, int64_t W, int64_t RH, int64_t RW, int64_t rescale, const OptT& y) {
    Dev dev("i3d_preprocess");
    auto a0 = (const void*)dev.p(x, "x");
    auto a11 = (float*)dev.p(y, "y");
    TORCH_CHECK(dev.idx >= 0, "hv::i3d_preprocess: needs at least one GPU tensor");
    c10::hip::HIPGuard guard(dev.idx);
    hipStream_t stream = c10::hip::getCurrentHIPStream(dev.idx).stream();
    check_rc(hv_i3d_preprocess(a0, (int64_t)x_sc, (int64_t)x_st, (int64_t)x_sh, (int)dtype, (int)T, (int)H, (int)W, (int)RH, (int)RW, (int)rescale, a11, stream), "i3d_preprocess");
}

void op_i3d_conv3d_f32(const OptT& x, int64_t ldx, const OptT& w, const OptT& sc, const OptT& sh, const OptT& y, int64_t ldy, int64_t T, int64_t H, int64_t W, int64_t Cin, int64_t Cout, int64_t kt, int64_t kh, int64_t kw, int64_t stride_t, int64_t stride_h, int64_t stride_w, int64_t pad_t, int64_t pad_h, int64_t pad_w, int64_t relu) {
    Dev dev("i3d_conv3d_f32");
    auto a0 = (const float*)dev.p(x, "x");
    auto a2 = (const float*)dev.p(w, "w");
    auto a3 = (const float*)dev.p(sc, "sc");
    auto a4 = (const float*)dev.p(sh, "sh");
    auto a5 = (float*)dev.p(y, "y");
    TORCH_CHECK(dev.idx >= 0, "hv::i3d_conv3d_f32: needs at least one GPU tensor");
    c10::hip::HIPGuard guard(dev.idx);
    hipStream_t stream = c10::hip::getCurrentHIPStream(dev.idx).stream();
    check_rc(hv_i3d_conv3d_f32(a0, (int64_t)ldx, a2, a3, a4, a5, (int64_t)ldy, (int)T, (int)H, (int)W, (int)Cin, (int)Cout, (int)kt, (int)kh, (int)kw, (int)stride_t, (int)stride_h, (int)stride_w, (int)pad_t, (int)pad_h, (int)pad_w, (int)relu, stream), "i3d_conv3d_f32");
}

void op_i3d_maxpool3d_f32(const OptT& x, int64_t ldx, const OptT& y, int64_t ldy, int64_t T, int64_t H, int64_t W, int64_t C, int64_t kt, int64_t kh, int64_t kw, int64_t stride_t, int64_t stride_h, int64_t stride_w, int64_t pad_t, int64_t pad_h, int64_t pad_w) {
    Dev dev("i3d_maxpool3d_f32");
    auto a0 = (const float*)dev.p(x, "x");
    auto a2 = (float*)dev.p(y, "y");
    TORCH_CHECK(dev.idx >= 0, "hv::i3d_maxpool3d_f32: needs at least one GPU tensor");
    c10::hip::HIPGuard guard(dev.idx);
    hipStream_t stream = c10::hip::getCurrentHIPStream(dev.idx).stream();
    check_rc(hv_i3d_maxpool3d_f32(a0, (int64_t)ldx, a2, (int64_t)ldy, (int)T, (int)H, (int)W, (int)C, (int)kt, (int)kh, (int)kw, (int)stride_t, (int)stride_h, (int)stride_w, (int)pad_t, (int)pad_h, (int)pad_w, stream), "i3d_maxpool3d_f32");
}

void op_i3d_head_f32(const OptT& x, int64_t ldx, const OptT& w, const OptT& bias, const OptT& out, int64_t T, int64_t H, int64_t W, int64_t C, const OptT& workspace, int64_t workspace_floats) {
    Dev dev("i3d_head_f32");
    auto a0 = (const float*)dev.p(x, "x");
    auto a2 = (const float*)dev.p(w, "w");
    auto a3 = (const float*)dev.p(bias, "bias");
    auto a4 = (float*)dev.p(out, "out");
    auto a9 = (float*)dev.p(workspace, "workspace");
    TORCH_CHECK(dev.idx >= 0, "hv::i3d_head_f32: needs at least one GPU tensor");
    c10::hip::HIPGuard guard(dev.idx);
    hipStream_t stream = c10::hip::getCurrentHIPStream(dev.idx).stream();
    check_rc(hv_i3d_head_f32(a0, (int64_t)ldx, a2, a3, a4, (int)T, (int)H, (int)W, (int)C, a9, (int64_t)workspace_floats, stream), "i3d_head_f32");
}

}

TORCH_LIBRARY(hv, m) {
    m.def("abi_version() -> int");
    m.def("ln_modulate_bf16(Tensor? x, Tensor? shift_or_bias, Tensor? scale_or_weight, Tensor(a!)? out, int M, int D, int ldx, int ldo, float eps, int mode) -> ()");
    m.def("qknorm_rope_bf16(Tensor(a!)? qkv, Tensor? q_weight, Tensor? k_weight, Tensor? cos_tab, Tensor? sin_tab, int n_rows, int n_rope, int n_heads, int head_dim, int ld, int k_offset, float eps) -> ()");
    m.def("qknorm_rope_scatter_bf16(Tensor? qkv, Tensor? q_weight, Tensor? k_weight, Tensor? cos_tab, Tensor? sin_tab, int n_rows, int n_rope, int n_heads, int head_dim, int ld, int k_offset, float eps, Tensor(a!)? dst, int dst_ld, int heads_per_block, int dst_block_stride) -> ()");
    m.def("gemm_bf16(Tensor? A, int lda, Tensor? W, int ldw, Tensor? bias, int M, int N, int K, Tensor(a!)? out0, int ld0, int act0, int n_split, Tensor(b!)? out1, int ld1, int act1, Tensor? gate, Tensor? res, int ld_res) -> ()");
    m.def("linear_smallm_bf16(Tensor? x, Tensor? W, Tensor? bias, Tensor? addend, Tensor(a!)? out, int M, int N, int K, int ldx, int ldo, int act) -> ()");
    m.def("timestep_embedding_bf16(Tensor? t, Tensor(a!)? out, int n_t, int dim, float max_period) -> ()");
    m.def("attn_fwd_bf16(Tensor? q, Tensor? k, Tensor? v, Tensor(a!)? o, int stride_q, int stride_k, int stride_v, int stride_o, int n_q, int n_kv, int n_heads, int head_dim, float scale, Tensor(b!)? workspace, int workspace_bytes) -> ()");
    m.def("attn_workspace_bytes(int n_q, int n_kv, int n_heads) -> int");
    m.def("attn_w4_loop_signature() -> int");
    m.def("attn_partial_bf16(Tensor? q, Tensor? k, Tensor? v, int stride_q, int stride_k, int stride_v, int n_q, int n_kv, int n_heads, int head_dim, float scale, Tensor(a!)? part_o, Tensor(b!)? part_ml, int n_slots, int slot, int splits) -> ()");
    m.def("attn_merge_bf16(Tensor? part_o, Tensor? part_ml, Tensor(a!)? o, int stride_o, int n_q, int n_heads, int n_slots) -> ()");
    m.def("attn_suggest_splits(int n_q, int n_kv, int n_heads) -> int");
    m.def("patchify_f32_bf16(Tensor? x, Tensor(a!)? A, int C, int T, int H, int W) -> ()");
    m.def("unpatchify_bf16(Tensor? y, Tensor(a!)? out, int C, int T, int H, int W, int ldy) -> ()");
    m.def("euler_step_f32(Tensor(a!)? sample, Tensor? model_out_bf16, float dt, int n) -> ()");
    m.def("euler_step_f32_f32(Tensor(a!)? sample, Tensor? model_out_f32, float dt, int n) -> ()");
    m.def("masked_mean_bf16(Tensor? x, Tensor? mask, Tensor(a!)? out, int L, int D) -> ()");
    m.def("broadcast_row_bf16(Tensor? src, Tensor(a!)? dst, int n_rows, int D, int ld) -> ()");
    m.def("copy3d_bf16(Tensor? src, Tensor(a!)? dst, int n_batch, int rows, int cols, int src_batch_stride, int src_ld, int dst_batch_stride, int dst_ld) -> ()");
    m.def("fp8_dequant_bf16(Tensor? w_e4m3fn, Tensor? scale_bf16, Tensor(a!)? out_bf16, int n) -> ()");
    m.def("ln_modulate_fp8(Tensor? x, Tensor? shift, Tensor? scale, Tensor(a!)? out_q, Tensor(b!)? out_row_scale, int M, int D, int ldx, int ldq, float eps) -> ()");
    m.def("quant_rows_fp8(Tensor? x, int ldx, Tensor(a!)? out_q, int ldq, Tensor(b!)? out_row_scale, int M, int K) -> ()");
    m.def("gemm_fp8(Tensor? A_q, int lda, Tensor? a_row_scale, Tensor? W_q, int ldw, Tensor? w_scale_bf16, Tensor? bias, int M, int N, int K, Tensor(a!)? out0, int ld0, int act0, int n_split, Tensor(b!)? out1, int ld1, int act1, Tensor? gate, Tensor? res, int ld_res) -> ()");
    m.def("gemm_f16(Tensor? A, int lda, Tensor? W, int ldw, Tensor? bias, int M, int N, int K, Tensor(a!)? out, int ldo, int out_is_f32, Tensor? res, int ld_res) -> ()");
    m.def("conv3d_causal_f16(Tensor? x, int ldx, Tensor? w_taps, Tensor? bias, Tensor(a!)? out, int ldo, int T, int H, int W, int Cin, int Cout, int up_t, int up_hw, Tensor? res, int ld_res, Tensor(b!)? gn_partial, int gn_partial_floats) -> ()");
    m.def("gn_partial_rows(int M) -> int");
    m.def("subpixel_gn_partial_rows(int sT, int sH, int sW, int up_t) -> int");
    m.def("conv3d_upsampled_subpixel_f16(Tensor? x, int ldx, Tensor? w_sub, Tensor? tap_table, int ntap, Tensor? bias, Tensor(a!)? out, int ldo, int sT, int sH, int sW, int Cin, int Cout, int up_t, Tensor(b!)? gn_partial, int gn_partial_floats) -> ()");
    m.def("conv3d_cout4_f16(Tensor? x, int ldx, Tensor? affine, int silu, Tensor? w_frag, Tensor? bias, Tensor(a!)? out, int ldo, int T, int H, int W, int Cin, int Cout, Tensor(b!)? planes, int planes_floats) -> ()");
    m.def("conv3d_cout4_planes_floats(int M) -> int");
    m.def("conv3d_causal_strided_f16(Tensor? x, int ldx, Tensor? w_taps, Tensor? bias, Tensor(a!)? out, int ldo, int sT, int sH, int sW, int Cin, int Cout, int stride_t, int stride_h, int stride_w) -> ()");
    m.def("temporal_resample_f16(Tensor? x, int ldx, Tensor(a!)? out, int ldo, int T_in, int HW, int C, int mode, int k, int s) -> ()");
    m.def("groupnorm_affine_f16(Tensor? x, int ldx, int M, int C, int groups, float eps, Tensor? weight, Tensor? bias, Tensor(a!)? partial_ws, int partial_ws_floats, Tensor(b!)? affine_out) -> ()");
    m.def("groupnorm_finalize_f16(Tensor? partial, int partial_floats, int nrow, int M, int C, int groups, float eps, Tensor? weight, Tensor? bias, Tensor(a!)? affine_out) -> ()");
    m.def("groupnorm_apply_f16(Tensor? x, int ldx, Tensor(a!)? y, int ldy, int M, int C, Tensor? affine, int silu) -> ()");
    m.def("softmax_rows_f32_f16(Tensor? S, int ld_s, Tensor(a!)? P, int ld_p, int rows, int cols, int cols_pad, float scale, int causal_block) -> ()");
    m.def("transpose_16b(Tensor? src, int ld_src, Tensor(a!)? dst, int ld_dst, int R, int C) -> ()");
    m.def("vae_latent_tile_f16(Tensor? z, int sc, int st, int sh, int sw, int C, int T, int H, int W, int Cpad, Tensor(a!)? out) -> ()");
    m.def("vae_blend_f16(Tensor? a, int[] a_strides, Tensor(a!)? b, int[] b_strides, int[] dims, int axis, int extent) -> ()");
    m.def("copy4d_16b(Tensor? src, int[] src_strides, Tensor(a!)? dst, int[] dst_strides, int[] dims) -> ()");
    m.def("vae_postprocess_f16_f32(Tensor? x, Tensor(a!)? out, int n) -> ()");
    m.def("video_metrics(Tensor? a, int a_sc, int a_st, int a_sh, Tensor? b, int b_sc, int b_st, int b_sh, int dtype, int C, int T, int H, int W, int rescale, int passes, Tensor(a!)? sse, Tensor(b!)? minmax, Tensor(c!)? ssim_sum, Tensor(d!)? workspace, int workspace_bytes) -> ()");
    m.def("video_metrics_workspace_bytes(int C, int T, int H, int W) -> int");
    m.def("lpips_conv1_f32(Tensor? a, int a_sc, int a_st, int a_sh, Tensor? b, int b_sc, int b_st, int b_sh, int dtype, int T, int H, int W, int rescale, Tensor? lut, Tensor? w, Tensor? bias, Tensor(a!)? y) -> ()");
    m.def("lpips_conv2d_f32(Tensor? x, Tensor? w, Tensor? bias, Tensor(a!)? y, int N, int H, int W, int Cin, int Cout, int ksize, int pad) -> ()");
    m.def("lpips_maxpool_f32(Tensor? x, Tensor(a!)? y, int N, int H, int W, int C) -> ()");
    m.def("lpips_distance_f32(Tensor? f, Tensor? lin, int T, int P, int C, int layer, Tensor(a!)? out, Tensor(b!)? workspace, int workspace_bytes) -> ()");
    m.def("lpips_distance_workspace_bytes(int T, int P) -> int");
    m.def("temporal_spectrum(Tensor? x, int sc, int st, int sh, int dtype, int mode, int C, int T, int H, int W, int rescale, int wr, int wg, int wb, int round, int shift, Tensor? twiddle, int twiddle_floats, Tensor(a!)? mag_sum, Tensor(b!)? pow_sum, Tensor(c!)? workspace, int workspace_bytes) -> ()");
    m.def("temporal_spectrum_workspace_bytes(int mode, int C, int T, int H, int W) -> int");
    m.def("i3d_preprocess(Tensor? x, int x_sc, int x_st, int x_sh, int dtype, int T, int H, int W, int RH, int RW, int rescale, Tensor(a!)? y) -> ()");
    m.def("i3d_conv3d_f32(Tensor? x, int ldx, Tensor? w, Tensor? sc, Tensor? sh, Tensor(a!)? y, int ldy, int T, int H, int W, int Cin, int Cout, int kt, int kh, int kw, int stride_t, int stride_h, int stride_w, int pad_t, int pad_h, int pad_w, int relu) -> ()");
    m.def("i3d_maxpool3d_f32(Tensor? x, int ldx, Tensor(a!)? y, int ldy, int T, int H, int W, int C, int kt, int kh, int kw, int stride_t, int stride_h, int stride_w, int pad_t, int pad_h, int pad_w) -> ()");
    m.def("i3d_head_f32(Tensor? x, int ldx, Tensor? w, Tensor? bias, Tensor(a!)? out, int T, int H, int W, int C, Tensor(b!)? workspace, int workspace_floats) -> ()");
}

TORCH_LIBRARY_IMPL(hv, CUDA, m) {
    m.impl("ln_modulate_bf16", &op_ln_modulate_bf16);
    m.impl("qknorm_rope_bf16", &op_qknorm_rope_bf16);
    m.impl("qknorm_rope_scatter_bf16", &op_qknorm_rope_scatter_bf16);
    m.impl("gemm_bf16", &op_gemm_bf16);
    m.impl("linear_smallm_bf16", &op_linear_smallm_bf16);
    m.impl("timestep_embedding_bf16", &op_timestep_embedding_bf16);
    m.impl("attn_fwd_bf16", &op_attn_fwd_bf16);
    m.impl("attn_partial_bf16", &op_attn_partial_bf16);
    m.impl("attn_merge_bf16", &op_attn_merge_bf16);
    m.impl("patchify_f32_bf16", &op_patchify_f32_bf16);
    m.impl("unpatchify_bf16", &op_unpatchify_bf16);
    m.impl("euler_step_f32", &op_euler_step_f32);
    m.impl("euler_step_f32_f32", &op_euler_step_f32_f32);
    m.impl("masked_mean_bf16", &op_masked_mean_bf16);
    m.impl("broadcast_row_bf16", &op_broadcast_row_bf16);
    m.impl("copy3d_bf16", &op_copy3d_bf16);
    m.impl("fp8_dequant_bf16", &op_fp8_dequant_bf16);
    m.impl("ln_modulate_fp8", &op_ln_modulate_fp8);
    m.impl("quant_rows_fp8", &op_quant_rows_fp8);
    m.impl("gemm_fp8", &op_gemm_fp8);
    m.impl("gemm_f16", &op_gemm_f16);
    m.impl("conv3d_causal_f16", &op_conv3d_causal_f16);
    m.impl("conv3d_upsampled_subpixel_f16", &op_conv3d_upsampled_subpixel_f16);
    m.impl("conv3d_cout4_f16", &op_conv3d_cout4_f16);
    m.impl("conv3d_causal_strided_f16", &op_conv3d_causal_strided_f16);
    m.impl("temporal_resample_f16", &op_temporal_resample_f16);
    m.impl("groupnorm_affine_f16", &op_groupnorm_affine_f16);
    m.impl("groupnorm_finalize_f16", &op_groupnorm_finalize_f16);
    m.impl("groupnorm_apply_f16", &op_groupnorm_apply_f16);
    m.impl("softmax_rows_f32_f16", &op_softmax_rows_f32_f16);
    m.impl("transpose_16b", &op_transpose_16b);
    m.impl("vae_latent_tile_f16", &op_vae_latent_tile_f16);
    m.impl("vae_blend_f16", &op_vae_blend_f16);
    m.impl("copy4d_16b", &op_copy4d_16b);
    m.impl("vae_postprocess_f16_f32", &op_vae_postprocess_f16_f32);
    m.impl("video_metrics", &op_video_metrics);
    m.impl("lpips_conv1_f32", &op_lpips_conv1_f32);
    m.impl("lpips_conv2d_f32", &op_lpips_conv2d_f32);
    m.impl("lpips_maxpool_f32", &op_lpips_maxpool_f32);
    m.impl("lpips_distance_f32", &op_lpips_distance_f32);
    m.impl("temporal_spectrum", &op_temporal_spectrum);
    m.impl("i3d_preprocess", &op_i3d_preprocess);
    m.impl("i3d_conv3d_f32", &op_i3d_conv3d_f32);
    m.impl("i3d_maxpool3d_f32", &op_i3d_maxpool3d_f32);
    m.impl("i3d_head_f32", &op_i3d_head_f32);
}

TORCH_LIBRARY_IMPL(hv, CompositeExplicitAutograd, m) {
    m.impl("abi_version", &op_abi_version);
    m.impl("attn_workspace_bytes", &op_attn_workspace_bytes);
    m.impl("attn_w4_loop_signature", &op_attn_w4_loop_signature);
    m.impl("attn_suggest_splits", &op_attn_suggest_splits);
    m.impl("gn_partial_rows", &op_gn_partial_rows);
    m.impl("subpixel_gn_partial_rows", &op_subpixel_gn_partial_rows);
    m.impl("conv3d_cout4_planes_floats", &op_conv3d_cout4_planes_floats);
    m.impl("video_metrics_workspace_bytes", &op_video_metrics_workspace_bytes);
    m.impl("lpips_distance_workspace_bytes", &op_lpips_distance_workspace_bytes);
    m.impl("temporal_spectrum_workspace_bytes", &op_temporal_spectrum_workspace_bytes);
}
```

### hunyuanvideo_efficiency_amd/modules/attenion.py

```python
from __future__ import annotations

from typing import Optional

import torch

from .. import ops

BF16 = torch.bfloat16
def n_valid_text(text_mask: torch.Tensor) -> int:
    hit = getattr(text_mask, "_hv_n_valid", None)
    if hit is not None and hit[0] == text_mask._version:
        return hit[1]
    m = text_mask[0].to("cpu").to(torch.int64)
    n = int(m.sum())
    if not bool((m[:n] != 0).all()):
        raise NotImplementedError("text_mask must be a prefix mask (valid tokens first)")
    try:
        text_mask._hv_n_valid = (text_mask._version, n)
    except (AttributeError, RuntimeError):
        pass
    return n


def get_cu_seqlens(text_mask: torch.Tensor, img_len: int) -> torch.Tensor:
    batch_size = text_mask.shape[0]
    text_len = text_mask.sum(dim=1).to("cpu")
    max_len = text_mask.shape[1] + img_len
    cu = [0]
    for i in range(batch_size):
        cu.append(i * max_len + int(text_len[i]) + img_len)
        cu.append((i + 1) * max_len)
    return torch.tensor(cu, dtype=torch.int32, device=text_mask.device)


def _flat2d(t: torch.Tensor) -> torch.Tensor:
    if t.dim() == 4:
        assert t.shape[0] == 1
        t = t[0]
    s, h, d = t.shape
    assert t.stride(2) == 1 and t.stride(1) == d, "heads must be packed inside a token row"
    return t.as_strided((s, h * d), (t.stride(0), 1), t.storage_offset())


def attention(q, k, v, mode="flash", drop_rate=0, attn_mask=None, causal=False, cu_seqlens_q=None, cu_seqlens_kv=None,
              max_seqlen_q=None, max_seqlen_kv=None, batch_size=1):
    if drop_rate != 0 or causal:
        raise NotImplementedError("inference path: dropout 0, non-causal")
    if attn_mask is not None:
        raise NotImplementedError("attn_mask: use cu_seqlens segments (the DiT path never passes a mask here)")
    b, s, a, d = q.shape
    if b != 1:
        raise NotImplementedError("batch size 1")
    out = torch.empty(b, s, a * d, dtype=BF16, device=q.device)
    q2, k2, v2 = _flat2d(q), _flat2d(k), _flat2d(v)
    if mode == "flash":
        bounds = [int(x) for x in cu_seqlens_q.tolist()]
        assert list(cu_seqlens_kv.tolist()) == bounds, "self-attention: q and kv segments coincide"
    elif mode in ("torch", "vanilla"):
        bounds = [0, s]
    else:
        raise NotImplementedError(f"Unsupported attention mode: {mode}")
    for lo, hi in zip(bounds[:-1], bounds[1:]):
        if hi > lo:
            ops.attn_fwd(q2[lo:hi], k2[lo:hi], v2[lo:hi], out[0, lo:hi], a)
    return out


def segment_attention_(hybrid_seq_parallel_attn, qkv: torch.Tensor, cat: torch.Tensor, s_img: int, cu1: int, heads: int, d: int):
    s = qkv.shape[0]
    q, k, v, o = qkv[:, :d], qkv[:, d:2 * d], qkv[:, 2 * d:], cat[:, :d]
    if hybrid_seq_parallel_attn is None:
        if cu1 > 0:
            ops.attn_fwd(q[:cu1], k[:cu1], v[:cu1], o[:cu1], heads)
    else:
        hybrid_seq_parallel_attn.run_fused(qkv, cat, s_img, cu1, heads, d)
    if s > cu1:
        ops.attn_fwd(q[cu1:], k[cu1:], v[cu1:], o[cu1:], heads)


def pad_segment_attention_(qkv: torch.Tensor, cat: torch.Tensor, cu1: int, heads: int, d: int):
    if qkv.shape[0] > cu1:
        ops.attn_fwd(qkv[cu1:, :d], qkv[cu1:, d:2 * d], qkv[cu1:, 2 * d:], cat[cu1:, :d], heads)


def parallel_attention(hybrid_seq_parallel_attn, q, k, v, img_q_len, img_kv_len, cu_seqlens_q, cu_seqlens_kv):
    cu1 = int(cu_seqlens_q[1])
    attn1 = hybrid_seq_parallel_attn(
        None, q[:, :img_q_len], k[:, :img_kv_len], v[:, :img_kv_len], dropout_p=0.0, causal=False,
        joint_tensor_query=q[:, img_q_len:cu1], joint_tensor_key=k[:, img_kv_len:cu1],
        joint_tensor_value=v[:, img_kv_len:cu1], joint_strategy="rear")
    b, s, a, d = q.shape
    out = torch.empty(b, s, a * d, dtype=BF16, device=q.device)
    out[:, :cu1] = attn1.reshape(b, cu1, a * d)
    if s > cu1:
        ops.attn_fwd(_flat2d(q)[cu1:], _flat2d(k)[cu1:], _flat2d(v)[cu1:], out[0, cu1:], a)
    return out
```

### hunyuanvideo_efficiency_amd/modules/models.py

```python
from __future__ import annotations

from typing import Any, Dict, List, Optional, Tuple, Union

import torch
import torch.nn as nn

from .. import ops
from .attenion import get_cu_seqlens, n_valid_text, segment_attention_, pad_segment_attention_
from .token_refiner import SingleTokenRefiner
from .layers import ParamLinear, ParamNormWeight, ModulateDiT, MLP, MLPEmbedder, TimestepEmbedder, PatchEmbed, FinalLayer

BF16 = torch.bfloat16


class _Workspace:

    def __init__(self, s_img: int, s_txt: int, d: int, mlp: int, device):
        s = s_img + s_txt
        self.key = (s_img, s_txt, d, mlp, str(device))
        self.x = torch.empty(s, d, dtype=BF16, device=device)
        self.xmod = torch.empty(s, d, dtype=BF16, device=device)
        self.qkv = torch.empty(s, 3 * d, dtype=BF16, device=device)
        self.cat = torch.empty(s, d + mlp, dtype=BF16, device=device)
        self.patches = None
        self.final = None
        self.xq = self.xs = self.catq = self.cats = None

    def fp8_buffers(self):
        if self.xq is None:
            s, d = self.x.shape
            dev = self.x.device
            self.xq = torch.empty(s, d, dtype=torch.float8_e4m3fn, device=dev)
            self.xs = torch.empty(s, dtype=torch.float32, device=dev)
            self.catq = torch.empty(s, self.cat.shape[1], dtype=torch.float8_e4m3fn, device=dev)
            self.cats = torch.empty(s, dtype=torch.float32, device=dev)
        return self


def _use_fp8_mfma(block, *layers) -> bool:
    return bool(getattr(block, "fp8_mfma", False)) and all(
        l.weight.dtype == torch.float8_e4m3fn and l.in_features >= 384 and l.in_features % 128 == 0 for l in layers)


def _ln(ws: _Workspace, lo: int, hi: int, shift, scale, fp8: bool):
    if fp8:
        ws.fp8_buffers()
        ops.ln_modulate_fp8(ws.x[lo:hi], shift, scale, out_q=ws.xq[lo:hi], out_scale=ws.xs[lo:hi])
    else:
        ops.ln_modulate(ws.x[lo:hi], shift, scale, out=ws.xmod[lo:hi])


def _gemm(ws: _Workspace, layer, src: str, lo: int, hi: int, fp8: bool, wrows: Optional[slice] = None, **epi):
    d = ws.x.shape[1]
    cols = {"xmod": None, "attn": slice(0, d), "hid": slice(d, None), "cat": slice(None)}[src]
    b = layer.bias if wrows is None or layer.bias is None else layer.bias[wrows]
    if not fp8:
        a = ws.xmod[lo:hi] if src == "xmod" else ws.cat[lo:hi, cols]
        w = layer.w()
        return ops.gemm(a, w if wrows is None else w[wrows], b, **epi)
    ws.fp8_buffers()
    if src == "xmod":
        aq, asc = ws.xq[lo:hi], ws.xs[lo:hi]
    else:
        aq, asc = ops.quant_rows_fp8(ws.cat[lo:hi, cols], out_q=ws.catq[lo:hi, cols], out_scale=ws.cats[lo:hi])
    w8 = layer.weight if wrows is None else layer.weight[wrows]
    return ops.gemm_fp8(aq, asc, w8, layer.fp8_scale, b, **epi)


def _sp_chunked_qkv(sp, ws: _Workspace, layer, fp8, q_norm_w, k_norm_w, cos, sin, s_img: int, cu1: int, n_rope: int, H: int, d: int):
    ld = ws.qkv.stride(0)
    sp.begin(s_img, cu1 - s_img, H, ws.qkv.device)
    for c, which, norm_w in ((0, "q", q_norm_w), (1, "k", k_norm_w), (2, "v", None)):
        dst = sp.chunk_dst(which) if hasattr(sp, "chunk_dst") else None
        chunk = dst if dst is not None else ws.qkv[:s_img, c * d:(c + 1) * d]
        _gemm(ws, layer, "xmod", 0, s_img, fp8, wrows=slice(c * d, (c + 1) * d), out=chunk)
        joint = ws.qkv[s_img:cu1, c * d:(c + 1) * d]
        if norm_w is not None:
            packed = sp.pack_dst(which) if dst is None and hasattr(sp, "pack_dst") else None
            ops.qknorm_rope_(chunk, norm_w, norm_w, cos, sin, n_rope, H // 2, (H // 2) * 128, out=packed)
            if packed is not None:
                sp.send_packed(which, joint, ld)
                continue
        sp.send(which, chunk, chunk.stride(0), joint, ld)


class MMDoubleStreamBlock(nn.Module):

    def __init__(self, hidden_size: int, heads_num: int, mlp_width_ratio: float, mlp_act_type: str = "gelu_tanh",
                 qk_norm: bool = True, qk_norm_type: str = "rms", qkv_bias: bool = False,
                 dtype: Optional[torch.dtype] = None, device: Optional[torch.device] = None):
        super().__init__()
        if mlp_act_type != "gelu_tanh" or not qk_norm or qk_norm_type != "rms":
            raise NotImplementedError("only gelu_tanh MLP and RMS qk-norm have kernels (the shipped configuration)")
        fk = {"device": device, "dtype": dtype}
        self.deterministic = False
        self.heads_num = heads_num
        head_dim = hidden_size // heads_num
        mlp_hidden = int(hidden_size * mlp_width_ratio)
        for s in ("img", "txt"):
            setattr(self, f"{s}_mod", ModulateDiT(hidden_size, 6, **fk))
            setattr(self, f"{s}_attn_qkv", ParamLinear(hidden_size, hidden_size * 3, qkv_bias, **fk))
            setattr(self, f"{s}_attn_q_norm", ParamNormWeight(head_dim, **fk))
            setattr(self, f"{s}_attn_k_norm", ParamNormWeight(head_dim, **fk))
            setattr(self, f"{s}_attn_proj", ParamLinear(hidden_size, hidden_size, qkv_bias, **fk))
            setattr(self, f"{s}_mlp", MLP(hidden_size, mlp_hidden, **fk))
        self.hybrid_seq_parallel_attn = None

    def enable_deterministic(self):
        self.deterministic = True

    def disable_deterministic(self):
        self.deterministic = False

    def run(self, ws: _Workspace, s_img: int, s_txt: int, vec: torch.Tensor, cu1: int,
            cos: Optional[torch.Tensor], sin: Optional[torch.Tensor]):
        d = ws.x.shape[1]
        H = self.heads_num
        streams = (("txt", s_img, s_img + s_txt, 0), ("img", 0, s_img, s_img if cos is not None else 0))
        sp = self.hybrid_seq_parallel_attn
        overlap = sp is not None and hasattr(sp, "send") and H % 2 == 0
        mods = {}
        fp8 = {s: _use_fp8_mfma(self, getattr(self, f"{s}_attn_qkv"), getattr(self, f"{s}_attn_proj"), getattr(self, f"{s}_mlp").fc1,
                                getattr(self, f"{s}_mlp").fc2) for s in ("img", "txt")}
        for s, lo, hi, n_rope in streams:
            mod = getattr(self, f"{s}_mod")
            m = ops.linear_smallm(vec, mod.linear.w(), mod.linear.bias, silu_in=True)
            mods[s] = [m[0, i * d:(i + 1) * d] for i in range(6)]
            sh1, sc1 = mods[s][0], mods[s][1]
            _ln(ws, lo, hi, sh1, sc1, fp8[s])
            qkv_l = getattr(self, f"{s}_attn_qkv")
            qw, kw = getattr(self, f"{s}_attn_q_norm").weight, getattr(self, f"{s}_attn_k_norm").weight
            if overlap and s == "img":
                _sp_chunked_qkv(sp, ws, qkv_l, fp8[s], qw, kw, cos, sin, s_img, cu1, n_rope, H, d)
            else:
                _gemm(ws, qkv_l, "xmod", lo, hi, fp8[s], out=ws.qkv[lo:hi])
                ops.qknorm_rope_(ws.qkv[lo:hi], qw, kw, cos, sin, n_rope, H, d)
        segs = None
        if overlap:
            segs = sp.attend_async(ws.cat, ws.cat.stride(0))
            pad_segment_attention_(ws.qkv, ws.cat, cu1, H, d)
        else:
            segment_attention_(sp, ws.qkv, ws.cat, s_img, cu1, H, d)
        streams = (streams[1], streams[0])
        for s, lo, hi, _ in streams:
            _, _, g1, sh2, sc2, g2 = mods[s]
            proj, mlp = getattr(self, f"{s}_attn_proj"), getattr(self, f"{s}_mlp")
            x = ws.x[lo:hi]
            if s == "img" and segs is not None:
                for r0, r1, finish in segs:
                    finish()
                    r1 = min(r1, hi)
                    _gemm(ws, proj, "attn", r0, r1, fp8[s], out=ws.x[r0:r1], gate=g1, res=ws.x[r0:r1])
            else:
                _gemm(ws, proj, "attn", lo, hi, fp8[s], out=x, gate=g1, res=x)
            _ln(ws, lo, hi, sh2, sc2, fp8[s])
            _gemm(ws, mlp.fc1, "xmod", lo, hi, fp8[s], out=ws.cat[lo:hi, d:], act=ops.ACT_GELU_TANH)
            _gemm(ws, mlp.fc2, "hid", lo, hi, fp8[s], out=x, gate=g2, res=x)

    def forward(self, img, txt, vec, cu_seqlens_q=None, cu_seqlens_kv=None, max_seqlen_q=None, max_seqlen_kv=None,
                freqs_cis: tuple = None) -> Tuple[torch.Tensor, torch.Tensor]:
        assert img.shape[0] == 1, "batch 1 (cfg-distilled model, SURVEY.md top)"
        s_img, s_txt, d = img.shape[1], txt.shape[1], img.shape[2]
        ws = _Workspace(s_img, s_txt, d, self.img_mlp.fc1.weight.shape[0], img.device)
        ws.x[:s_img].copy_(img[0])
        ws.x[s_img:].copy_(txt[0])
        cu1 = int(cu_seqlens_q[1])
        cos, sin = freqs_cis if freqs_cis is not None else (None, None)
        self.run(ws, s_img, s_txt, vec.to(BF16).contiguous(), cu1, cos, sin)
        return ws.x[None, :s_img], ws.x[None, s_img:]


class MMSingleStreamBlock(nn.Module):

    def __init__(self, hidden_size: int, heads_num: int, mlp_width_ratio: float = 4.0, mlp_act_type: str = "gelu_tanh",
                 qk_norm: bool = True, qk_norm_type: str = "rms", qk_scale: float = None,
                 dtype: Optional[torch.dtype] = None, device: Optional[torch.device] = None):
        super().__init__()
        if mlp_act_type != "gelu_tanh" or not qk_norm or qk_norm_type != "rms" or qk_scale is not None:
            raise NotImplementedError("only gelu_tanh MLP, RMS qk-norm and the default scale have kernels")
        fk = {"device": device, "dtype": dtype}
        self.deterministic = False
        self.hidden_size = hidden_size
        self.heads_num = heads_num
        head_dim = hidden_size // heads_num
        self.mlp_hidden_dim = int(hidden_size * mlp_width_ratio)
        self.scale = head_dim ** -0.5
        self.linear1 = ParamLinear(hidden_size, hidden_size * 3 + self.mlp_hidden_dim, True, **fk)
        self.linear2 = ParamLinear(hidden_size + self.mlp_hidden_dim, hidden_size, True, **fk)
        self.q_norm = ParamNormWeight(head_dim, **fk)
        self.k_norm = ParamNormWeight(head_dim, **fk)
        self.modulation = ModulateDiT(hidden_size, 3, **fk)
        self.hybrid_seq_parallel_attn = None

    def enable_deterministic(self):
        self.deterministic = True

    def disable_deterministic(self):
        self.deterministic = False

    def run(self, ws: _Workspace, s_img: int, s_txt: int, vec: torch.Tensor, cu1: int,
            cos: Optional[torch.Tensor], sin: Optional[torch.Tensor]):
        d, H = self.hidden_size, self.heads_num
        m = ops.linear_smallm(vec, self.modulation.linear.w(), self.modulation.linear.bias, silu_in=True)
        shift, scale, gate = m[0, :d], m[0, d:2 * d], m[0, 2 * d:]
        fp8 = _use_fp8_mfma(self, self.linear1, self.linear2)
        s_all = ws.x.shape[0]
        _ln(ws, 0, s_all, shift, scale, fp8)
        sp = self.hybrid_seq_parallel_attn
        n_rope = s_img if cos is not None else 0
        if sp is not None and hasattr(sp, "send") and H % 2 == 0:
            _gemm(ws, self.linear1, "xmod", s_img, s_all, fp8, wrows=slice(0, 3 * d), out=ws.qkv[s_img:])
            ops.qknorm_rope_(ws.qkv[s_img:], self.q_norm.weight, self.k_norm.weight, None, None, 0, H, d)
            _sp_chunked_qkv(sp, ws, self.linear1, fp8, self.q_norm.weight, self.k_norm.weight, cos, sin, s_img, cu1, n_rope, H, d)
            _gemm(ws, self.linear1, "xmod", 0, s_all, fp8, wrows=slice(3 * d, None), out=ws.cat[:, d:], act=ops.ACT_GELU_TANH)
            segs = sp.attend_async(ws.cat, ws.cat.stride(0))
            pad_segment_attention_(ws.qkv, ws.cat, cu1, H, d)
            for i, (r0, r1, finish) in enumerate(segs):
                finish()
                r1 = s_all if i == len(segs) - 1 else r1
                _gemm(ws, self.linear2, "cat", r0, r1, fp8, out=ws.x[r0:r1], gate=gate, res=ws.x[r0:r1])
            return
        else:
            _gemm(ws, self.linear1, "xmod", 0, s_all, fp8, out=ws.qkv, n_split=3 * d, out1=ws.cat[:, d:], act1=ops.ACT_GELU_TANH)
            ops.qknorm_rope_(ws.qkv, self.q_norm.weight, self.k_norm.weight, cos, sin, n_rope, H, d)
            segment_attention_(sp, ws.qkv, ws.cat, s_img, cu1, H, d)
        _gemm(ws, self.linear2, "cat", 0, s_all, fp8, out=ws.x, gate=gate, res=ws.x)

    def forward(self, x, vec, txt_len, cu_seqlens_q=None, cu_seqlens_kv=None, max_seqlen_q=None, max_seqlen_kv=None,
                freqs_cis: Tuple[torch.Tensor, torch.Tensor] = None) -> torch.Tensor:
        assert x.shape[0] == 1
        s, d = x.shape[1], x.shape[2]
        ws = _Workspace(s - txt_len, txt_len, d, self.mlp_hidden_dim, x.device)
        ws.x.copy_(x[0])
        cos, sin = freqs_cis if freqs_cis is not None else (None, None)
        self.run(ws, s - txt_len, txt_len, vec.to(BF16).contiguous(), int(cu_seqlens_q[1]), cos, sin)
        return ws.x[None]


class _Config(dict):
    __getattr__ = dict.__getitem__


class HYVideoDiffusionTransformer(nn.Module):

    def __init__(self, args: Any, patch_size: list = [1, 2, 2], in_channels: int = 4, out_channels: int = None,
                 hidden_size: int = 3072, heads_num: int = 24, mlp_width_ratio: float = 4.0, mlp_act_type: str = "gelu_tanh",
                 mm_double_blocks_depth: int = 20, mm_single_blocks_depth: int = 40, rope_dim_list: List[int] = [16, 56, 56],
                 qkv_bias: bool = True, qk_norm: bool = True, qk_norm_type: str = "rms", guidance_embed: bool = False,
                 text_projection: str = "single_refiner", use_attention_mask: bool = True,
                 dtype: Optional[torch.dtype] = None, device: Optional[torch.device] = None):
        super().__init__()
        fk = {"device": device, "dtype": dtype}
        self.config = _Config(patch_size=patch_size, in_channels=in_channels, out_channels=out_channels,
                              hidden_size=hidden_size, heads_num=heads_num, mlp_width_ratio=mlp_width_ratio,
                              mlp_act_type=mlp_act_type, mm_double_blocks_depth=mm_double_blocks_depth,
                              mm_single_blocks_depth=mm_single_blocks_depth, rope_dim_list=rope_dim_list,
                              qkv_bias=qkv_bias, qk_norm=qk_norm, qk_norm_type=qk_norm_type,
                              guidance_embed=guidance_embed, text_projection=text_projection,
                              use_attention_mask=use_attention_mask)
        self.patch_size = patch_size
        self.in_channels = in_channels
        self.out_channels = in_channels if out_channels is None else out_channels
        self.unpatchify_channels = self.out_channels
        self.guidance_embed = guidance_embed
        self.rope_dim_list = rope_dim_list
        self.use_attention_mask = use_attention_mask
        self.text_projection = text_projection
        self.text_states_dim = args.text_states_dim
        self.text_states_dim_2 = args.text_states_dim_2
        if hidden_size % heads_num != 0:
            raise ValueError(f"Hidden size {hidden_size} must be divisible by heads_num {heads_num}")
        pe_dim = hidden_size // heads_num
        if sum(rope_dim_list) != pe_dim:
            raise ValueError(f"Got {rope_dim_list} but expected positional dim {pe_dim}")
        if pe_dim != 128:
            raise NotImplementedError("kernels are built for head_dim 128 (HunyuanVideo: 3072/24)")
        if list(patch_size) != [1, 2, 2]:
            raise NotImplementedError("kernels are built for patch_size [1,2,2]")
        if text_projection != "single_refiner":
            raise NotImplementedError(f"Unsupported text_projection: {text_projection}")
        self.hidden_size = hidden_size
        self.heads_num = heads_num
        self.mlp_hidden = int(hidden_size * mlp_width_ratio)

        self.img_in = PatchEmbed(self.patch_size, self.in_channels, self.hidden_size, **fk)
        self.txt_in = SingleTokenRefiner(self.text_states_dim, hidden_size, heads_num, depth=2, **fk)
        self.time_in = TimestepEmbedder(self.hidden_size, **fk)
        self.vector_in = MLPEmbedder(self.text_states_dim_2, self.hidden_size, **fk)
        self.guidance_in = TimestepEmbedder(self.hidden_size, **fk) if guidance_embed else None
        self.double_blocks = nn.ModuleList([
            MMDoubleStreamBlock(self.hidden_size, self.heads_num, mlp_width_ratio=mlp_width_ratio, mlp_act_type=mlp_act_type,
                                qk_norm=qk_norm, qk_norm_type=qk_norm_type, qkv_bias=qkv_bias, **fk)
            for _ in range(mm_double_blocks_depth)])
        self.single_blocks = nn.ModuleList([
            MMSingleStreamBlock(self.hidden_size, self.heads_num, mlp_width_ratio=mlp_width_ratio, mlp_act_type=mlp_act_type,
                                qk_norm=qk_norm, qk_norm_type=qk_norm_type, **fk)
            for _ in range(mm_single_blocks_depth)])
        self.final_layer = FinalLayer(self.hidden_size, self.patch_size, self.out_channels, **fk)
        self._ws: Optional[_Workspace] = None

    @property
    def dtype(self):
        return self.img_in.proj.weight.dtype

    def enable_deterministic(self):
        for b in list(self.double_blocks) + list(self.single_blocks):
            b.enable_deterministic()

    def disable_deterministic(self):
        for b in list(self.double_blocks) + list(self.single_blocks):
            b.disable_deterministic()

    def _workspace(self, s_img: int, s_txt: int, device) -> _Workspace:
        key = (s_img, s_txt, self.hidden_size, self.mlp_hidden, str(device))
        if self._ws is None or self._ws.key != key:
            self._ws = None
            self._ws = _Workspace(s_img, s_txt, self.hidden_size, self.mlp_hidden, device)
        return self._ws

    def forward(self, x: torch.Tensor, t: torch.Tensor, text_states: torch.Tensor = None, text_mask: torch.Tensor = None,
                text_states_2: Optional[torch.Tensor] = None, freqs_cos: Optional[torch.Tensor] = None,
                freqs_sin: Optional[torch.Tensor] = None, guidance: torch.Tensor = None,
                return_dict: bool = True) -> Union[torch.Tensor, Dict[str, torch.Tensor]]:
        if self.dtype != BF16:
            raise TypeError(f"parameters must be bf16 (got {self.dtype}); build with dtype=torch.bfloat16 or call .to()")
        B = x.shape[0]
        if B == 1:
            out = self._forward_one(x, t, text_states, text_mask, text_states_2, freqs_cos, freqs_sin, guidance, 0)
        else:
            t = t.reshape(-1)
            if t.numel() == 1:
                t = t.expand(B)
            outs = []
            for b in range(B):
                g_b = None if guidance is None else guidance.reshape(-1)[b:b + 1] if guidance.numel() > 1 else guidance
                outs.append(self._forward_one(x[b:b + 1], t[b:b + 1], text_states, text_mask,
                                              None if text_states_2 is None else text_states_2[b:b + 1], freqs_cos, freqs_sin, g_b, b))
            out = torch.cat(outs, 0)
        if return_dict:
            return {"x": out}
        return out

    def _forward_one(self, x, t, text_states, text_mask, text_states_2, freqs_cos, freqs_sin, guidance, b: int) -> torch.Tensor:
        dev = x.device
        _, _, ot, oh, ow = x.shape
        tt, th, tw = ot // self.patch_size[0], oh // self.patch_size[1], ow // self.patch_size[2]
        s_img, s_txt, d = tt * th * tw, text_states.shape[1], self.hidden_size
        ws = self._workspace(s_img, s_txt, dev)

        t32 = t.reshape(-1).to(torch.float32)
        vec = self.time_in.run(t32)
        vec = self.vector_in.run(text_states_2.to(BF16).reshape(1, -1), addend=vec)
        if self.guidance_embed:
            if guidance is None:
                raise ValueError("Didn't get guidance strength for guidance distilled model.")
            vec = self.guidance_in.run(guidance.reshape(-1).to(torch.float32), addend=vec)

        self.img_in.run(x[0].to(torch.float32).contiguous(), ws, s_img)
        mask_all = text_mask if self.use_attention_mask else None
        tc_all = getattr(text_states, "_hv_txt_cache", None)
        key = (text_states._version, None if mask_all is None else mask_all._version, id(self.txt_in),
               tuple(p._version for p in self.txt_in.parameters()))
        if tc_all is None or tc_all.get("key") != key or tc_all.get("mask") is not mask_all:
            tc_all = {"key": key, "mask": mask_all, "rows": {}}
            try:
                text_states._hv_txt_cache = tc_all
            except (AttributeError, RuntimeError):
                pass
        tc = tc_all["rows"].get(b)
        if tc is None:
            tc = tc_all["rows"][b] = {"text_bf16": text_states[b].to(BF16).contiguous(),
                                      "mask": None if mask_all is None else (mask_all if mask_all.shape[0] == 1 else mask_all[b:b + 1]),
                                      "mask_cu": None if text_mask is None else (text_mask if text_mask.shape[0] == 1 else text_mask[b:b + 1])}
        mask = tc["mask"]
        self.txt_in.run(tc["text_bf16"], t32, mask, out=ws.x[s_img:], cache=tc)

        if text_mask is not None and tc.get("mask_cu_src") is not text_mask:
            tc["mask_cu"] = text_mask if text_mask.shape[0] == 1 else text_mask[b:b + 1]
            tc["mask_cu_src"] = text_mask
        cu1 = s_img + (n_valid_text(tc["mask_cu"]) if text_mask is not None else s_txt)
        cos = freqs_cos.to(device=dev, dtype=torch.float32).contiguous() if freqs_cos is not None else None
        sin = freqs_sin.to(device=dev, dtype=torch.float32).contiguous() if freqs_sin is not None else None

        for block in self.double_blocks:
            block.run(ws, s_img, s_txt, vec, cu1, cos, sin)
        for block in self.single_blocks:
            block.run(ws, s_img, s_txt, vec, cu1, cos, sin)

        img = self.final_layer.run(ws, s_img, vec)
        out = ops.unpatchify(img, self.unpatchify_channels, ot, oh, ow)
        return out[None]

    def params_count(self):
        counts = {
            "double": sum(sum(p.numel() for p in m.parameters())
                          for b in self.double_blocks
                          for m in (b.img_attn_qkv, b.img_attn_proj, b.img_mlp, b.txt_attn_qkv, b.txt_attn_proj, b.txt_mlp)),
            "single": sum(sum(p.numel() for p in m.parameters()) for b in self.single_blocks for m in (b.linear1, b.linear2)),
            "total": sum(p.numel() for p in self.parameters()),
        }
        counts["attn+mlp"] = counts["double"] + counts["single"]
        return counts


HUNYUAN_VIDEO_CONFIG = {
    "HYVideo-T/2": dict(mm_double_blocks_depth=20, mm_single_blocks_depth=40, rope_dim_list=[16, 56, 56],
                        hidden_size=3072, heads_num=24, mlp_width_ratio=4),
    "HYVideo-T/2-cfgdistill": dict(mm_double_blocks_depth=20, mm_single_blocks_depth=40, rope_dim_list=[16, 56, 56],
                                   hidden_size=3072, heads_num=24, mlp_width_ratio=4, guidance_embed=True),
}
```

### hunyuanvideo_efficiency_amd/ops.py

```python
from __future__ import annotations

from typing import Optional

import torch

from . import _abi, _lib

BF16 = torch.bfloat16
ACT_NONE, ACT_GELU_TANH, ACT_SILU = 0, 1, 2
PROFILE_ATTN = None


def _chk(t: torch.Tensor, dtype, name: str, last_contig: bool = True):
    if not t.is_cuda:
        raise _lib.HVKernelError(f"{name}: expected a GPU tensor (this package has no CPU path), got {t.device}")
    if t.dtype != dtype:
        raise TypeError(f"{name}: expected {dtype}, got {t.dtype}")
    if last_contig and t.dim() > 0 and t.stride(-1) != 1:
        raise ValueError(f"{name}: innermost dimension must be contiguous")


def _rows(t: torch.Tensor, name: str):
    if t.dim() == 1:
        return 1, t.shape[0], t.shape[0]
    d = t.shape[-1]
    n = t.numel() // d
    ld = t.stride(-2)
    exp = ld
    for i in range(t.dim() - 2, -1, -1):
        if t.shape[i] != 1 and t.stride(i) != exp:
            raise ValueError(f"{name}: rows are not uniformly strided {t.shape} {t.stride()}")
        exp *= t.shape[i]
    return n, d, ld


def _chk_mod_vectors(shift, scale, d: int):
    for t, n in ((shift, "shift"), (scale, "scale")):
        if t is not None:
            _chk(t, BF16, n)
            assert t.numel() == d and t.is_contiguous(), f"{n} must be a contiguous [{d}] vector (batch 1)"


def ln_modulate(x, shift=None, scale=None, out=None, eps: float = 1e-6, affine: bool = False):
    _chk(x, BF16, "x")
    m, d, ldx = _rows(x, "x")
    if out is None:
        out = torch.empty(x.shape, dtype=BF16, device=x.device)
    _chk(out, BF16, "out")
    mo, do, ldo = _rows(out, "out")
    assert (mo, do) == (m, d)
    _chk_mod_vectors(shift, scale, d)
    _lib.call("ln_modulate_bf16", x, shift, scale, out, m, d, ldx, ldo, eps,
                                               1 if affine else 0)
    return out


def qknorm_rope_(qkv, q_weight, k_weight, cos, sin, n_rope: int, n_heads: int, k_offset: int, eps: float = 1e-6, out=None):
    _chk(qkv, BF16, "qkv")
    n, _, ld = _rows(qkv, "qkv")
    _chk(q_weight, BF16, "q_weight"), _chk(k_weight, BF16, "k_weight")
    if n_rope > 0:
        _chk(cos, torch.float32, "cos"), _chk(sin, torch.float32, "sin")
        assert cos.is_contiguous() and sin.is_contiguous() and cos.shape[-1] == 128 and cos.shape[0] >= n_rope
    if out is not None:
        _chk(out, BF16, "out", False)
        assert out.dim() == 3 and out.shape[0] == n and out.stride(2) == 1 and out.shape[2] % 128 == 0
        assert out.shape[1] * out.shape[2] == 2 * n_heads * 128, (out.shape, n_heads)
        _lib.call("qknorm_rope_scatter_bf16", qkv, q_weight, k_weight, cos, sin, n, n_rope, n_heads, 128, ld, k_offset, eps,
                  out, out.stride(0), out.shape[2] // 128, out.stride(1))
        return out
    _lib.call("qknorm_rope_bf16", qkv, q_weight, k_weight, cos, sin, n,
                                               n_rope, n_heads, 128, ld, k_offset, eps)
    return qkv


def _gemm_epilogue(out_shape, device, m: int, n: int, n_split: int, out, out1, bias, gate, res):
    n0 = n_split if 0 < n_split < n else n
    if out is None:
        out = torch.empty(*out_shape, n0, dtype=BF16, device=device)
    _chk(out, BF16, "out")
    mo, no, ld0 = _rows(out, "out")
    assert mo == m and no >= n0
    ld1 = 0
    if n0 < n:
        _chk(out1, BF16, "out1")
        m1, n1, ld1 = _rows(out1, "out1")
        assert m1 == m and n1 >= n - n0
    for t, nm in ((bias, "bias"), (gate, "gate")):
        if t is not None:
            _chk(t, BF16, nm)
            assert t.numel() == n and t.is_contiguous()
    ld_res = 0
    if res is not None:
        _chk(res, BF16, "res")
        mr, nr, ld_res = _rows(res, "res")
        assert mr == m and nr == n
    return out, n0, ld0, ld1, ld_res


def gemm(a, w, bias=None, out=None, act: int = ACT_NONE, n_split: int = 0, out1=None, act1: int = ACT_NONE,
         gate=None, res=None):
    _chk(a, BF16, "a"), _chk(w, BF16, "w")
    m, k, lda = _rows(a, "a")
    n, kw, ldw = _rows(w, "w")
    assert k == kw, (a.shape, w.shape)
    out, n0, ld0, ld1, ld_res = _gemm_epilogue(a.shape[:-1], a.device, m, n, n_split, out, out1, bias, gate, res)
    _lib.call("gemm_bf16", a, lda, w, ldw, bias, m, n, k, out, ld0, act, n0,
                                        out1, ld1, act1, gate, res, ld_res)
    return out


def linear_smallm(x, w, bias=None, silu_in: bool = False, silu_out: bool = False, out=None, addend=None):
    _chk(x, BF16, "x"), _chk(w, BF16, "w")
    m, k, ldx = _rows(x, "x")
    n, kw, ldw = _rows(w, "w")
    assert k == kw and ldw == k and m <= 4
    if out is None:
        out = torch.empty(*x.shape[:-1], n, dtype=BF16, device=x.device)
    _, _, ldo = _rows(out, "out")
    if bias is not None:
        _chk(bias, BF16, "bias")
    if addend is not None:
        _chk(addend, BF16, "addend")
        assert addend.shape == out.shape and addend.stride() == out.stride()
    _lib.call("linear_smallm_bf16", x, w, bias, addend, out, m, n, k, ldx, ldo,
                                                 (1 if silu_in else 0) | (2 if silu_out else 0))
    return out


_attn_ws = {}
ATTN_MIN_WORKSPACE = _abi.MACROS["HV_ATTN_MIN_WORKSPACE_BYTES"]


def _attn_workspace_bytes(n_q: int, n_kv: int, n_heads: int) -> int:
    if n_kv < _abi.MACROS["HV_ATTN_BOUND_MIN_KV"]:
        return 0
    if attn_suggest_splits(n_q, n_kv, n_heads) == 2:
        return int(_lib.host("attn_workspace_bytes", n_q, n_kv, n_heads))
    return ATTN_MIN_WORKSPACE


def _attn_workspace(n_q, n_kv, n_heads, device):
    need = _attn_workspace_bytes(n_q, n_kv, n_heads)
    if need == 0:
        return None
    key = str(device)
    ws = _attn_ws.get(key)
    if ws is None or ws.numel() < need:
        ws = torch.empty(need, dtype=torch.uint8, device=device)
        _attn_ws[key] = ws
    return ws


def attn_fwd(q, k, v, out, n_heads: int, scale: Optional[float] = None, kv_split_workspace: bool = True):
    for t, nm in ((q, "q"), (k, "k"), (v, "v"), (out, "out")):
        _chk(t, BF16, nm)
        assert t.dim() == 2
    n_q, n_kv = q.shape[0], k.shape[0]
    assert v.shape[0] == n_kv and out.shape[0] == n_q
    if scale is None:
        scale = 128 ** -0.5
    prof = PROFILE_ATTN
    if prof is not None:
        e0, e1 = torch.cuda.Event(enable_timing=True), torch.cuda.Event(enable_timing=True)
        e0.record()
    ws = _attn_workspace(n_q, n_kv, n_heads, q.device) if kv_split_workspace else None
    _lib.call("attn_fwd_bf16", q, k, v, out, q.stride(0), k.stride(0), v.stride(0),
                                            out.stride(0), n_q, n_kv, n_heads, 128, scale, ws,
                                            0 if ws is None else ws.numel())
    if prof is not None:
        e1.record()
        prof.append((e0, e1, n_q, n_kv, n_heads))
    return out


class AttnPartials:

    def __init__(self, n_slots: int, n_q: int, n_heads: int, device):
        self.n_slots, self.n_q, self.n_heads = n_slots, n_q, n_heads
        self.o = torch.empty(n_slots, n_q, n_heads, 128, dtype=torch.float32, device=device)
        self.ml = torch.empty(n_slots, n_q, n_heads, 2, dtype=torch.float32, device=device)
        self.used = 0


def attn_suggest_splits(n_q: int, n_kv: int, n_heads: int) -> int:
    return int(_lib.host("attn_suggest_splits", n_q, n_kv, n_heads))


def attn_partial(q, k, v, parts: AttnPartials, n_heads: int, splits: int = 1, scale: Optional[float] = None):
    for t, nm in ((q, "q"), (k, "k"), (v, "v")):
        _chk(t, BF16, nm)
        assert t.dim() == 2
    n_q, n_kv = q.shape[0], k.shape[0]
    assert v.shape[0] == n_kv and n_q == parts.n_q and n_heads == parts.n_heads and parts.used + splits <= parts.n_slots
    if scale is None:
        scale = 128 ** -0.5
    prof = PROFILE_ATTN
    if prof is not None:
        e0, e1 = torch.cuda.Event(enable_timing=True), torch.cuda.Event(enable_timing=True)
        e0.record()
    _lib.call("attn_partial_bf16", q, k, v, q.stride(0), k.stride(0), v.stride(0), n_q, n_kv, n_heads,
                                                128, scale, parts.o, parts.ml, parts.n_slots, parts.used, splits)
    if prof is not None:
        e1.record()
        prof.append((e0, e1, n_q, n_kv, n_heads))
    parts.used += splits


def attn_merge(parts: AttnPartials, out):
    _chk(out, BF16, "out")
    assert out.dim() == 2 and out.shape[0] == parts.n_q and parts.used >= 1
    _lib.call("attn_merge_bf16", parts.o, parts.ml, out, out.stride(0), parts.n_q, parts.n_heads,
                                              parts.used)
    return out


def patchify(x_f32, out=None):
    _chk(x_f32, torch.float32, "x")
    assert x_f32.is_contiguous() and x_f32.dim() == 4
    c, t, h, w = x_f32.shape
    if out is None:
        out = torch.empty(t * (h // 2) * (w // 2), c * 4, dtype=BF16, device=x_f32.device)
    _lib.call("patchify_f32_bf16", x_f32, out, c, t, h, w)
    return out


def unpatchify(y, c: int, t: int, h: int, w: int, out=None):
    _chk(y, BF16, "y")
    assert y.dim() == 2
    if out is None:
        out = torch.empty(c, t, h, w, dtype=BF16, device=y.device)
    _lib.call("unpatchify_bf16", y, out, c, t, h, w, y.stride(0))
    return out


def euler_step_(sample_f32, model_out_bf16, dt: float):
    _chk(sample_f32, torch.float32, "sample"), _chk(model_out_bf16, BF16, "model_out")
    assert sample_f32.is_contiguous() and model_out_bf16.is_contiguous() and sample_f32.numel() == model_out_bf16.numel()
    _lib.call("euler_step_f32", sample_f32, model_out_bf16, float(dt), sample_f32.numel())
    return sample_f32


def euler_step_f32_(sample_f32, model_out_f32, dt: float):
    _chk(sample_f32, torch.float32, "sample"), _chk(model_out_f32, torch.float32, "model_out")
    assert sample_f32.is_contiguous() and model_out_f32.is_contiguous() and sample_f32.numel() == model_out_f32.numel()
    _lib.call("euler_step_f32_f32", sample_f32, model_out_f32, float(dt), sample_f32.numel())
    return sample_f32


def masked_mean(x, mask_i32=None):
    _chk(x, BF16, "x")
    assert x.dim() == 2 and x.is_contiguous()
    out = torch.empty(x.shape[1], dtype=BF16, device=x.device)
    if mask_i32 is not None:
        _chk(mask_i32, torch.int32, "mask")
    _lib.call("masked_mean_bf16", x, mask_i32, out, x.shape[0], x.shape[1])
    return out


def broadcast_row_(src, dst):
    _chk(src, BF16, "src"), _chk(dst, BF16, "dst")
    assert dst.dim() == 2 and src.numel() == dst.shape[1]
    _lib.call("broadcast_row_bf16", src, dst, dst.shape[0], dst.shape[1], dst.stride(0))
    return dst


def timestep_embedding(t_f32, dim: int = 256, max_period: float = 10000.0):
    _chk(t_f32, torch.float32, "t")
    t_f32 = t_f32.reshape(-1).contiguous()
    out = torch.empty(t_f32.numel(), dim, dtype=BF16, device=t_f32.device)
    _lib.call("timestep_embedding_bf16", t_f32, out, t_f32.numel(), dim, max_period)
    return out


def fp8_dequant(w8, scale_bf16, out_bf16):
    if not w8.is_cuda or w8.dtype != torch.float8_e4m3fn:
        raise _lib.HVKernelError("fp8_dequant: expected a float8_e4m3fn GPU tensor")
    _chk(scale_bf16, BF16, "scale"), _chk(out_bf16, BF16, "out")
    assert w8.is_contiguous() and out_bf16.is_contiguous() and out_bf16.numel() == w8.numel()
    _lib.call("fp8_dequant_bf16", w8, scale_bf16, out_bf16, w8.numel())
    return out_bf16


FP8 = torch.float8_e4m3fn


def ln_modulate_fp8(x, shift=None, scale=None, out_q=None, out_scale=None, eps: float = 1e-6):
    _chk(x, BF16, "x")
    m, d, ldx = _rows(x, "x")
    if out_q is None:
        out_q = torch.empty(m, d, dtype=FP8, device=x.device)
    if out_scale is None:
        out_scale = torch.empty(m, dtype=torch.float32, device=x.device)
    assert out_q.dtype == FP8 and out_q.is_cuda and out_q.shape[-1] == d and out_q.stride(-1) == 1 and out_scale.numel() >= m
    _chk_mod_vectors(shift, scale, d)
    _lib.call("ln_modulate_fp8", x, shift, scale, out_q, out_scale, m, d, ldx, out_q.stride(-2) if out_q.dim() > 1 else d, eps)
    return out_q, out_scale


def quant_rows_fp8(x, out_q=None, out_scale=None):
    _chk(x, BF16, "x")
    m, k, ldx = _rows(x, "x")
    if out_q is None:
        out_q = torch.empty(m, k, dtype=FP8, device=x.device)
    if out_scale is None:
        out_scale = torch.empty(m, dtype=torch.float32, device=x.device)
    assert out_q.dtype == FP8 and out_q.is_cuda and out_q.shape[-1] == k and out_q.stride(-1) == 1 and out_scale.numel() >= m
    _lib.call("quant_rows_fp8", x, ldx, out_q, out_q.stride(-2) if out_q.dim() > 1 else k, out_scale, m, k)
    return out_q, out_scale


def gemm_fp8(a_q, a_scale, w_q, w_scale, bias=None, out=None, act: int = ACT_NONE, n_split: int = 0, out1=None,
             act1: int = ACT_NONE, gate=None, res=None):
    for t, nm in ((a_q, "a_q"), (w_q, "w_q")):
        if not t.is_cuda or t.dtype != FP8:
            raise _lib.HVKernelError(f"gemm_fp8: {nm} must be a float8_e4m3fn GPU tensor")
    _chk(a_scale, torch.float32, "a_scale"), _chk(w_scale, BF16, "w_scale")
    m, k, lda = _rows(a_q, "a_q")
    n, kw, ldw = _rows(w_q, "w_q")
    assert k == kw and a_scale.numel() >= m and w_scale.numel() == 1
    out, n0, ld0, ld1, ld_res = _gemm_epilogue((m,), a_q.device, m, n, n_split, out, out1, bias, gate, res)
    _lib.call("gemm_fp8", a_q, lda, a_scale, w_q, ldw, w_scale, bias, m, n, k, out, ld0, act, n0, out1, ld1, act1, gate, res, ld_res)
    return out


def copy3d(src, dst, n_batch: int, rows: int, cols: int, src_bs: int, src_ld: int, dst_bs: int, dst_ld: int):
    _chk(src, BF16, "src", False), _chk(dst, BF16, "dst", False)
    _lib.call("copy3d_bf16", src, dst, n_batch, rows, cols, src_bs, src_ld, dst_bs, dst_ld)
    return dst
```

### include/hv_kernels.h

```cpp
#ifndef HV_KERNELS_H
#define HV_KERNELS_H

#include <stdint.h>

#ifdef __cplusplus
extern "C" {
#endif

#ifndef __HIP__
typedef struct ihipStream_t* hipStream_t;
#endif

#define HV_ABI_VERSION 10
int hv_abi_version(void);

int hv_ln_modulate_bf16(const void* x, const void* shift_or_bias, const void* scale_or_weight, void* out,
                        int64_t M, int D, int64_t ldx, int64_t ldo, float eps, int mode, hipStream_t stream);

int hv_qknorm_rope_bf16(void* qkv, const void* q_weight, const void* k_weight, const float* cos_tab,
                        const float* sin_tab, int64_t n_rows, int64_t n_rope, int n_heads, int head_dim,
                        int64_t ld, int64_t k_offset, float eps, hipStream_t stream);

int hv_qknorm_rope_scatter_bf16(const void* qkv, const void* q_weight, const void* k_weight, const float* cos_tab,
                                const float* sin_tab, int64_t n_rows, int64_t n_rope, int n_heads, int head_dim, int64_t ld,
                                int64_t k_offset, float eps, void* dst, int64_t dst_ld, int heads_per_block,
                                int64_t dst_block_stride, hipStream_t stream);

int hv_gemm_bf16(const void* A, int64_t lda, const void* W, int64_t ldw, const void* bias, int M, int N, int K,
                 void* out0, int64_t ld0, int act0, int n_split, void* out1, int64_t ld1, int act1,
                 const void* gate, const void* res, int64_t ld_res, hipStream_t stream);

int hv_linear_smallm_bf16(const void* x, const void* W, const void* bias, const void* addend, void* out, int M,
                          int N, int K, int64_t ldx, int64_t ldo, int act, hipStream_t stream);

int hv_timestep_embedding_bf16(const float* t, void* out, int n_t, int dim, float max_period, hipStream_t stream);

#define HV_ATTN_MIN_WORKSPACE_BYTES 256
#define HV_ATTN_BOUND_MIN_KV 4096
int hv_attn_fwd_bf16(const void* q, const void* k, const void* v, void* o, int64_t stride_q, int64_t stride_k,
                     int64_t stride_v, int64_t stride_o, int n_q, int n_kv, int n_heads, int head_dim,
                     float scale, void* workspace, int64_t workspace_bytes, hipStream_t stream);

int64_t hv_attn_workspace_bytes(int n_q, int n_kv, int n_heads);
int hv_attn_w4_loop_signature(void);

int hv_attn_partial_bf16(const void* q, const void* k, const void* v, int64_t stride_q, int64_t stride_k, int64_t stride_v,
                         int n_q, int n_kv, int n_heads, int head_dim, float scale, void* part_o, void* part_ml,
                         int n_slots, int slot, int splits, hipStream_t stream);

int hv_attn_merge_bf16(const void* part_o, const void* part_ml, void* o, int64_t stride_o, int n_q, int n_heads, int n_slots,
                       hipStream_t stream);

int hv_attn_suggest_splits(int n_q, int n_kv, int n_heads);

int hv_patchify_f32_bf16(const float* x, void* A, int C, int T, int H, int W, hipStream_t stream);

int hv_unpatchify_bf16(const void* y, void* out, int C, int T, int H, int W, int64_t ldy, hipStream_t stream);

int hv_euler_step_f32(float* sample, const void* model_out_bf16, float dt, int64_t n, hipStream_t stream);

int hv_euler_step_f32_f32(float* sample, const float* model_out_f32, float dt, int64_t n, hipStream_t stream);

int hv_masked_mean_bf16(const void* x, const int* mask, void* out, int L, int D, hipStream_t stream);

int hv_broadcast_row_bf16(const void* src, void* dst, int64_t n_rows, int D, int64_t ld, hipStream_t stream);

int hv_copy3d_bf16(const void* src, void* dst, int n_batch, int64_t rows, int cols, int64_t src_batch_stride,
                   int64_t src_ld, int64_t dst_batch_stride, int64_t dst_ld, hipStream_t stream);

int hv_fp8_dequant_bf16(const void* w_e4m3fn, const void* scale_bf16, void* out_bf16, int64_t n, hipStream_t stream);


int hv_ln_modulate_fp8(const void* x, const void* shift, const void* scale, void* out_q, float* out_row_scale, int64_t M,
                       int D, int64_t ldx, int64_t ldq, float eps, hipStream_t stream);

int hv_quant_rows_fp8(const void* x, int64_t ldx, void* out_q, int64_t ldq, float* out_row_scale, int64_t M, int K,
                      hipStream_t stream);

int hv_gemm_fp8(const void* A_q, int64_t lda, const float* a_row_scale, const void* W_q, int64_t ldw, const void* w_scale_bf16,
                const void* bias, int M, int N, int K, void* out0, int64_t ld0, int act0, int n_split, void* out1, int64_t ld1,
                int act1, const void* gate, const void* res, int64_t ld_res, hipStream_t stream);


int hv_gemm_f16(const void* A, int64_t lda, const void* W, int64_t ldw, const void* bias, int M, int N, int K,
                void* out, int64_t ldo, int out_is_f32, const void* res, int64_t ld_res, hipStream_t stream);

int hv_conv3d_causal_f16(const void* x, int64_t ldx, const void* w_taps, const void* bias, void* out, int64_t ldo,
                         int T, int H, int W, int Cin, int Cout, int up_t, int up_hw, const void* res,
                         int64_t ld_res, float* gn_partial, int64_t gn_partial_floats, hipStream_t stream);

int64_t hv_gn_partial_rows(int64_t M);
int64_t hv_subpixel_gn_partial_rows(int sT, int sH, int sW, int up_t);

int hv_conv3d_upsampled_subpixel_f16(const void* x, int64_t ldx, const void* w_sub, const void* tap_table, int ntap,
                                     const void* bias, void* out, int64_t ldo, int sT, int sH, int sW, int Cin, int Cout,
                                     int up_t, float* gn_partial, int64_t gn_partial_floats, hipStream_t stream);

int hv_conv3d_cout4_f16(const void* x, int64_t ldx, const float* affine, int silu, const void* w_frag, const void* bias, void* out,
                        int64_t ldo, int T, int H, int W, int Cin, int Cout, float* planes, int64_t planes_floats, hipStream_t stream);
int64_t hv_conv3d_cout4_planes_floats(int64_t M);

int hv_conv3d_causal_strided_f16(const void* x, int64_t ldx, const void* w_taps, const void* bias, void* out, int64_t ldo,
                                 int sT, int sH, int sW, int Cin, int Cout, int stride_t, int stride_h, int stride_w,
                                 hipStream_t stream);

int hv_temporal_resample_f16(const void* x, int64_t ldx, void* out, int64_t ldo, int T_in, int64_t HW, int C, int mode,
                             int k, int s, hipStream_t stream);

int hv_groupnorm_affine_f16(const void* x, int64_t ldx, int64_t M, int C, int groups, float eps, const void* weight,
                            const void* bias, float* partial_ws, int64_t partial_ws_floats, float* affine_out,
                            hipStream_t stream);

#define HV_GN_FOLD_WS_FLOATS 16384
int hv_groupnorm_finalize_f16(const float* partial, int64_t partial_floats, int64_t nrow, int64_t M, int C, int groups, float eps,
                              const void* weight, const void* bias, float* affine_out, hipStream_t stream);

int hv_groupnorm_apply_f16(const void* x, int64_t ldx, void* y, int64_t ldy, int64_t M, int C, const float* affine,
                           int silu, hipStream_t stream);

int hv_softmax_rows_f32_f16(const float* S, int64_t ld_s, void* P, int64_t ld_p, int rows, int cols, int cols_pad,
                            float scale, int causal_block, hipStream_t stream);

int hv_transpose_16b(const void* src, int64_t ld_src, void* dst, int64_t ld_dst, int R, int C, hipStream_t stream);

int hv_vae_latent_tile_f16(const float* z, int64_t sc, int64_t st, int64_t sh, int64_t sw, int C, int T, int H, int W,
                           int Cpad, void* out, hipStream_t stream);

int hv_vae_blend_f16(const void* a, const int64_t* a_strides, void* b, const int64_t* b_strides, const int* dims,
                     int axis, int extent, hipStream_t stream);

int hv_copy4d_16b(const void* src, const int64_t* src_strides, void* dst, const int64_t* dst_strides, const int* dims,
                  hipStream_t stream);

int hv_vae_postprocess_f16_f32(const void* x, float* out, int64_t n, hipStream_t stream);

int hv_video_metrics(const void* a, int64_t a_sc, int64_t a_st, int64_t a_sh, const void* b, int64_t b_sc, int64_t b_st,
                     int64_t b_sh, int dtype, int C, int T, int H, int W, int rescale, int passes, void* sse, void* minmax,
                     void* ssim_sum, void* workspace, int64_t workspace_bytes, hipStream_t stream);
int64_t hv_video_metrics_workspace_bytes(int C, int T, int H, int W);

int hv_lpips_conv1_f32(const void* a, int64_t a_sc, int64_t a_st, int64_t a_sh, const void* b, int64_t b_sc, int64_t b_st,
                       int64_t b_sh, int dtype, int T, int H, int W, int rescale, const float* lut, const float* w,
                       const float* bias, float* y, hipStream_t stream);

int hv_lpips_conv2d_f32(const float* x, const float* w, const float* bias, float* y, int N, int H, int W, int Cin, int Cout,
                        int ksize, int pad, hipStream_t stream);

int hv_lpips_maxpool_f32(const float* x, float* y, int N, int H, int W, int C, hipStream_t stream);

int hv_lpips_distance_f32(const float* f, const float* lin, int T, int64_t P, int C, int layer, double* out, void* workspace,
                          int64_t workspace_bytes, hipStream_t stream);
int64_t hv_lpips_distance_workspace_bytes(int T, int64_t P);

#define HV_SPECTRUM_MAX_T 1024
#define HV_SPECTRUM_BK 32
#define HV_SPECTRUM_BINS 32
int hv_temporal_spectrum(const void* x, int64_t sc, int64_t st, int64_t sh, int dtype, int mode, int C, int T, int H, int W,
                         int rescale, int wr, int wg, int wb, int round, int shift, const float* twiddle, int64_t twiddle_floats,
                         double* mag_sum, double* pow_sum, void* workspace, int64_t workspace_bytes, hipStream_t stream);
int64_t hv_temporal_spectrum_workspace_bytes(int mode, int C, int T, int H, int W);

int hv_i3d_preprocess(const void* x, int64_t x_sc, int64_t x_st, int64_t x_sh, int dtype, int T, int H, int W, int RH, int RW, int rescale,
                      float* y, hipStream_t stream);

int hv_i3d_conv3d_f32(const float* x, int64_t ldx, const float* w, const float* sc, const float* sh, float* y, int64_t ldy, int T, int H,
                      int W, int Cin, int Cout, int kt, int kh, int kw, int stride_t, int stride_h, int stride_w, int pad_t, int pad_h,
                      int pad_w, int relu, hipStream_t stream);

int hv_i3d_maxpool3d_f32(const float* x, int64_t ldx, float* y, int64_t ldy, int T, int H, int W, int C, int kt, int kh, int kw,
                         int stride_t, int stride_h, int stride_w, int pad_t, int pad_h, int pad_w, hipStream_t stream);

#define HV_I3D_HEAD_MAX_T 4096
int hv_i3d_head_f32(const float* x, int64_t ldx, const float* w, const float* bias, float* out, int T, int H, int W, int C,
                    float* workspace, int64_t workspace_floats, hipStream_t stream);

#ifdef __cplusplus
}
#endif
#endif
```

Baseline: 0.1216.

## Fuse key-norm bound computation into QK-norm/RoPE kernel, skip attention pre-pass

```diff
diff --git a/hunyuanvideo_efficiency_amd/csrc/hv_attention.hip b/hunyuanvideo_efficiency_amd/csrc/hv_attention.hip
--- a/hunyuanvideo_efficiency_amd/csrc/hv_attention.hip
+++ b/hunyuanvideo_efficiency_amd/csrc/hv_attention.hip
@@ -42,16 +42,7 @@
     const int r0 = blockIdx.x * KMAX_ROWS, r1 = min(r0 + KMAX_ROWS, n_kv);
     float best = 0.f;
     for (int row = r0 + (t >> 4); row < r1; row += 16) {
-        const u32x4 w = *reinterpret_cast<const u32x4*>(k + (int64_t)row * sk + head * D + ch * 8);
-        float s = 0.f;
-#pragma unroll
-        for (int j = 0; j < 4; ++j) {
-            const float lo = bf2f_lo(w[j]), hi = bf2f_hi(w[j]);
-            s += lo * lo + hi * hi;
-        }
-#pragma unroll
-        for (int o = 8; o > 0; o >>= 1) s += __shfl_xor(s, o, 64);
-        best = fmaxf(best, s);
+        best = fmaxf(best, head_norm2_16(*reinterpret_cast<const u32x4*>(k + (int64_t)row * sk + head * D + ch * 8)));
     }
     best = fmaxf(best, __shfl_xor(best, 16, 64));
     best = fmaxf(best, __shfl_xor(best, 32, 64));
@@ -60,14 +51,31 @@
     if (t == 0) atomicMax(out + head, __float_as_uint(fmaxf(fmaxf(wmax[0], wmax[1]), fmaxf(wmax[2], wmax[3]))));
 }
 
+bool attn_takes_bound(const AttnArgs& a, const void* workspace, int64_t workspace_bytes) {
+    static_assert(HV_ATTN_BOUND_MIN_KV == 64 * KVT, "the pre-pass pays from 64 key tiles on");
+    static_assert((KMAX_HEADS + 2) * 4 == KMAX_BYTES, "bounds + two mode flags fill the workspace head");
+    return workspace && workspace_bytes >= KMAX_BYTES && a.n_heads <= KMAX_HEADS && a.n_kv >= HV_ATTN_BOUND_MIN_KV;
+}
 int attn_prepare_kmax(AttnArgs& a, void* workspace, int64_t workspace_bytes, hipStream_t stream) {
-    static_assert(HV_ATTN_BOUND_MIN_KV == 64 * KVT, "the pre-pass pays from 64 key tiles on");
     a.kmax2 = nullptr;
-    if (!workspace || workspace_bytes < KMAX_BYTES || a.n_heads > KMAX_HEADS || a.n_kv < HV_ATTN_BOUND_MIN_KV) return HV_OK;
+    if (!attn_takes_bound(a, workspace, workspace_bytes)) return HV_OK;
     if (hipMemsetAsync(workspace, 0, KMAX_BYTES, stream) != hipSuccess) return HV_ERR_LAUNCH;
     attn_kmax_kernel<<<dim3((unsigned)((a.n_kv + KMAX_ROWS - 1) / KMAX_ROWS), (unsigned)a.n_heads), dim3(256), 0, stream>>>(a.k, a.sk, a.n_kv, (unsigned*)workspace);
     a.kmax2 = (const unsigned*)workspace;
     return HV_OK;
+}
+
+__global__ __launch_bounds__(256) void attn_kbound_fold_kernel(const float* __restrict__ kpart, int64_t n_blocks, int n_heads,
+                                                                unsigned* __restrict__ out) {
+    __shared__ float wmax[4];
+    const int head = blockIdx.x, t = threadIdx.x;
+    float best = 0.f;
+    for (int64_t b = t; b < n_blocks; b += 256) best = fmaxf(best, kpart[b * KMAX_HEADS + head]);
+    best = wave_max(best);
+    if ((t & 63) == 0) wmax[t >> 6] = best;
+    __syncthreads();
+    if (t == 0) out[head] = __float_as_uint(fmaxf(fmaxf(wmax[0], wmax[1]), fmaxf(wmax[2], wmax[3])));
+    if (head == 0 && t >= n_heads && t < KMAX_BYTES / 4) out[t] = 0u;
 }
 
 int attn_kv_splits(int n_q, int n_kv, int n_heads) {
@@ -84,9 +92,9 @@
     return (int64_t)KMAX_BYTES + (int64_t)2 * n_q * n_heads * (128 + 2) * (int64_t)sizeof(float);
 }
 
-extern "C" int hv_attn_fwd_bf16(const void* q, const void* k, const void* v, void* o, int64_t stride_q, int64_t stride_k,
-                                int64_t stride_v, int64_t stride_o, int n_q, int n_kv, int n_heads, int head_dim,
-                                float scale, void* workspace, int64_t workspace_bytes, hipStream_t stream) {
+static int attn_fwd(const void* q, const void* k, const void* v, void* o, int64_t stride_q, int64_t stride_k, int64_t stride_v,
+                    int64_t stride_o, int n_q, int n_kv, int n_heads, int head_dim, float scale, void* workspace,
+                    int64_t workspace_bytes, bool bound_ready, hipStream_t stream) {
     if (!q || !k || !v || !o || head_dim != D || n_heads <= 0 || n_q < 0 || n_kv < 0 || (stride_q & 7) || (stride_k & 7) ||
         (stride_v & 7) || (stride_o & 3))
         return HV_ERR_ARG;
@@ -99,7 +107,10 @@
     a.n_qtiles = (n_q + QTILE - 1) / QTILE;
     a.scale_log2e = scale * 1.4426950408889634f;
     a.n_splits = 1; a.split_keys = n_kv; a.part_o = nullptr; a.part_ml = nullptr; a.partial = 0;
-    if (attn_prepare_kmax(a, workspace, workspace_bytes, stream) != HV_OK) return HV_ERR_LAUNCH;
+    if (bound_ready)
+        a.kmax2 = attn_takes_bound(a, workspace, workspace_bytes) ? (const unsigned*)workspace : nullptr;
+    else if (attn_prepare_kmax(a, workspace, workspace_bytes, stream) != HV_OK)
+        return HV_ERR_LAUNCH;
     if (workspace && attn_kv_splits(n_q, n_kv, n_heads) == 2 && workspace_bytes >= hv_attn_workspace_bytes(n_q, n_kv, n_heads)) {
         a.n_splits = 2;
         a.split_keys = (((n_kv + KVT - 1) / KVT + 1) / 2) * KVT;
@@ -112,6 +123,27 @@
         attn_combine_kernel<<<dim3((unsigned)((total + 255) / 256)), dim3(256), 0, stream>>>(a.part_o, a.part_ml, a.o, a.so, n_q, n_heads,
                                                                                            a.n_splits);
     }
+    return hv_check_launch();
+}
+
+extern "C" int hv_attn_fwd_bf16(const void* q, const void* k, const void* v, void* o, int64_t stride_q, int64_t stride_k,
+                                int64_t stride_v, int64_t stride_o, int n_q, int n_kv, int n_heads, int head_dim,
+                                float scale, void* workspace, int64_t workspace_bytes, hipStream_t stream) {
+    return attn_fwd(q, k, v, o, stride_q, stride_k, stride_v, stride_o, n_q, n_kv, n_heads, head_dim, scale, workspace, workspace_bytes,
+                    false, stream);
+}
+
+extern "C" int hv_attn_fwd_bf16_kbound(const void* q, const void* k, const void* v, void* o, int64_t stride_q, int64_t stride_k,
+                                       int64_t stride_v, int64_t stride_o, int n_q, int n_kv, int n_heads, int head_dim,
+                                       float scale, void* workspace, int64_t workspace_bytes, hipStream_t stream) {
+    return attn_fwd(q, k, v, o, stride_q, stride_k, stride_v, stride_o, n_q, n_kv, n_heads, head_dim, scale, workspace, workspace_bytes,
+                    true, stream);
+}
+
+extern "C" int hv_attn_kbound_fold(const float* kpart, int64_t n_blocks, int n_heads, void* workspace, int64_t workspace_bytes,
+                                   hipStream_t stream) {
+    if (!kpart || !workspace || workspace_bytes < KMAX_BYTES || n_blocks <= 0 || n_heads <= 0 || n_heads > KMAX_HEADS) return HV_ERR_ARG;
+    attn_kbound_fold_kernel<<<dim3((unsigned)n_heads), dim3(256), 0, stream>>>(kpart, n_blocks, n_heads, (unsigned*)workspace);
     return hv_check_launch();
 }
 
diff --git a/hunyuanvideo_efficiency_amd/csrc/hv_attention.hpp b/hunyuanvideo_efficiency_amd/csrc/hv_attention.hpp
--- a/hunyuanvideo_efficiency_amd/csrc/hv_attention.hpp
+++ b/hunyuanvideo_efficiency_amd/csrc/hv_attention.hpp
@@ -21,7 +21,7 @@
     const unsigned* kmax2;
 };
 constexpr int KMAX_BYTES = HV_ATTN_MIN_WORKSPACE_BYTES;
-constexpr int KMAX_HEADS = 62;
+constexpr int KMAX_HEADS = HV_ATTN_BOUND_MAX_HEADS;
 
 typedef __attribute__((ext_vector_type(4))) short s16x4;
 typedef __attribute__((address_space(3))) s16x4* lds_s16x4_ptr;
diff --git a/hunyuanvideo_efficiency_amd/csrc/hv_common.hpp b/hunyuanvideo_efficiency_amd/csrc/hv_common.hpp
--- a/hunyuanvideo_efficiency_amd/csrc/hv_common.hpp
+++ b/hunyuanvideo_efficiency_amd/csrc/hv_common.hpp
@@ -84,6 +84,18 @@
 template <typename T> __device__ __forceinline__ T wave_max(T v) { return wave_reduce(v, WaveMax{}); }
 template <typename T> __device__ __forceinline__ T wave_min(T v) { return wave_reduce(v, WaveMin{}); }
 
+__device__ __forceinline__ float head_norm2_16(const u32x4& w) {
+    float s = 0.f;
+#pragma unroll
+    for (int j = 0; j < 4; ++j) {
+        const float lo = bf2f_lo(w[j]), hi = bf2f_hi(w[j]);
+        s += lo * lo + hi * hi;
+    }
+#pragma unroll
+    for (int o = 8; o > 0; o >>= 1) s += __shfl_xor(s, o, 64);
+    return s;
+}
+
 __device__ __forceinline__ float gelu_tanh_f(float x) {
     const float k0 = 0.7978845608028654f, k1 = 0.044715f;
     float u = k0 * (x + k1 * x * x * x);
diff --git a/hunyuanvideo_efficiency_amd/csrc/hv_rowwise.hip b/hunyuanvideo_efficiency_amd/csrc/hv_rowwise.hip
--- a/hunyuanvideo_efficiency_amd/csrc/hv_rowwise.hip
+++ b/hunyuanvideo_efficiency_amd/csrc/hv_rowwise.hip
@@ -211,53 +211,119 @@
     return hv_check_launch();
 }
 
+constexpr int QKN_ROWS = HV_QKNORM_ROWS_PER_BLOCK;
+constexpr int QKN_HV = 3;
+struct QknRowLoads {
+    u32x4 x[QKN_HV];
+    float4 c0, c1, s0, s1;
+};
+
+template <bool KB, bool ROPE, int ROWS>
 __global__ __launch_bounds__(256) void qknorm_rope_kernel(bf16_t* __restrict__ qkv, const bf16_t* __restrict__ qw,
                                                            const bf16_t* __restrict__ kw, const float* __restrict__ cosT,
                                                            const float* __restrict__ sinT, int64_t n_rows, int64_t n_rope,
                                                            int H, int64_t ld, int64_t k_off, float eps, bf16_t* __restrict__ dst,
-                                                           int64_t dst_ld, int hpb, int64_t dst_bs) {
-    const int64_t row = blockIdx.x;
+                                                           int64_t dst_ld, int hpb, int64_t dst_bs, float* __restrict__ kpart) {
+    const int64_t r0 = (int64_t)blockIdx.x * ROWS;
+    const int64_t r1 = r0 + ROWS < n_rows ? r0 + ROWS : n_rows;
     const int sub = threadIdx.x & 15;
     const int grp = threadIdx.x >> 4;
-    float wq[8], wk[8], c[8], s[8];
+    float wq[8], wk[8];
     unpack8(*reinterpret_cast<const u32x4*>(qw + sub * 8), wq);
     unpack8(*reinterpret_cast<const u32x4*>(kw + sub * 8), wk);
-    const bool rope = row < n_rope;
-    if (rope) {
-        const float4* cp = reinterpret_cast<const float4*>(cosT + row * 128 + sub * 8);
-        const float4* sp = reinterpret_cast<const float4*>(sinT + row * 128 + sub * 8);
-        float4 c0 = cp[0], c1 = cp[1], s0 = sp[0], s1 = sp[1];
-        c[0] = c0.x, c[1] = c0.y, c[2] = c0.z, c[3] = c0.w, c[4] = c1.x, c[5] = c1.y, c[6] = c1.z, c[7] = c1.w;
-        s[0] = s0.x, s[1] = s0.y, s[2] = s0.z, s[3] = s0.w, s[4] = s1.x, s[5] = s1.y, s[6] = s1.z, s[7] = s1.w;
-    }
-    for (int hv = grp; hv < 2 * H; hv += 16) {
-        const bool is_k = hv >= H;
-        const int h = is_k ? hv - H : hv;
-        bf16_t* p = qkv + row * ld + (is_k ? k_off : 0) + h * 128 + sub * 8;
-        float x[8];
-        unpack8(*reinterpret_cast<const u32x4*>(p), x);
-        if (dst) p = dst + (int64_t)(hv / hpb) * dst_bs + row * dst_ld + (hv % hpb) * 128 + sub * 8;
-        float ss = 0.f;
-#pragma unroll
-        for (int j = 0; j < 8; ++j) ss += x[j] * x[j];
-#pragma unroll
-        for (int o = 8; o > 0; o >>= 1) ss += __shfl_xor(ss, o, 16);
-        const float r = rsqrtf(ss * (1.0f / 128.0f) + eps);
-        float y[8];
-#pragma unroll
-        for (int j = 0; j < 8; ++j) y[j] = rbf(rbf(x[j] * r) * (is_k ? wk[j] : wq[j]));
-        if (rope) {
-            float o[8];
-#pragma unroll
-            for (int j = 0; j < 8; j += 2) {
-                o[j] = y[j] * c[j] - y[j + 1] * s[j];
-                o[j + 1] = y[j + 1] * c[j + 1] + y[j] * s[j + 1];
-            }
-            *reinterpret_cast<u32x4*>(p) = pack8(o);
+    for (int hv0 = grp; hv0 < 2 * H; hv0 += 16 * QKN_HV) {
+        auto load = [&](int64_t row, QknRowLoads& t) {
+            row = row < r1 ? row : r1 - 1;
+#pragma unroll
+            for (int i = 0; i < QKN_HV; ++i) {
+                const int hv = hv0 + 16 * i < 2 * H ? hv0 + 16 * i : hv0;
+                t.x[i] = *reinterpret_cast<const u32x4*>(qkv + row * ld + (hv >= H ? k_off + (hv - H) * 128 : hv * 128) + sub * 8);
+            }
+            if (ROPE) {
+                const int64_t cr = row < n_rope ? row : n_rope - 1;
+                const float4* cp = reinterpret_cast<const float4*>(cosT + cr * 128 + sub * 8);
+                const float4* sp = reinterpret_cast<const float4*>(sinT + cr * 128 + sub * 8);
+                t.c0 = cp[0], t.c1 = cp[1], t.s0 = sp[0], t.s1 = sp[1];
+            }
+        };
+        float best[QKN_HV];
+#pragma unroll
+        for (int i = 0; i < QKN_HV; ++i) best[i] = 0.f;
+        auto norm_row = [&](int64_t row, const QknRowLoads& t) {
+            const bool rope = ROPE && row < n_rope;
+            const float c[8] = {t.c0.x, t.c0.y, t.c0.z, t.c0.w, t.c1.x, t.c1.y, t.c1.z, t.c1.w};
+            const float s[8] = {t.s0.x, t.s0.y, t.s0.z, t.s0.w, t.s1.x, t.s1.y, t.s1.z, t.s1.w};
+#pragma unroll
+            for (int i = 0; i < QKN_HV; ++i) {
+                const int hv = hv0 + 16 * i;
+                if (hv >= 2 * H) break;
+                const bool is_k = hv >= H;
+                bf16_t* p = dst ? dst + (int64_t)(hv / hpb) * dst_bs + row * dst_ld + (hv % hpb) * 128 + sub * 8
+                                : qkv + row * ld + (is_k ? k_off + (hv - H) * 128 : hv * 128) + sub * 8;
+                float x[8];
+                unpack8(t.x[i], x);
+                float ss = 0.f;
+#pragma unroll
+                for (int j = 0; j < 8; ++j) ss += x[j] * x[j];
+#pragma unroll
+                for (int o = 8; o > 0; o >>= 1) ss += __shfl_xor(ss, o, 16);
+                const float r = rsqrtf(ss * (1.0f / 128.0f) + eps);
+                float y[8];
+#pragma unroll
+                for (int j = 0; j < 8; ++j) y[j] = rbf(rbf(x[j] * r) * (is_k ? wk[j] : wq[j]));
+                u32x4 w;
+                if (rope) {
+                    float o[8];
+#pragma unroll
+                    for (int j = 0; j < 8; j += 2) {
+                        o[j] = y[j] * c[j] - y[j + 1] * s[j];
+                        o[j + 1] = y[j + 1] * c[j + 1] + y[j] * s[j + 1];
+                    }
+                    w = pack8(o);
+                } else {
+                    w = pack8(y);
+                }
+                *reinterpret_cast<u32x4*>(p) = w;
+                if (KB && is_k) best[i] = fmaxf(best[i], head_norm2_16(w));
+            }
+        };
+        QknRowLoads a, b;
+        load(r0, a);
+        if constexpr (ROWS == 1) {
+            norm_row(r0, a);
         } else {
-            *reinterpret_cast<u32x4*>(p) = pack8(y);
-        }
-    }
+            for (int64_t row = r0; row < r1; row += 2) {
+                load(row + 1, b);
+                norm_row(row, a);
+                load(row + 2, a);
+                if (row + 1 < r1) norm_row(row + 1, b);
+            }
+        }
+        if (KB && sub == 0) {
+#pragma unroll
+            for (int i = 0; i < QKN_HV; ++i) {
+                const int hv = hv0 + 16 * i;
+                if (hv >= H && hv < 2 * H) kpart[(int64_t)blockIdx.x * HV_ATTN_BOUND_MAX_HEADS + (hv - H)] = best[i];
+            }
+        }
+    }
+}
+
+static int qknorm_rope_launch(void* qkv, const void* q_weight, const void* k_weight, const float* cos_tab, const float* sin_tab,
+                              int64_t n_rows, int64_t n_rope, int n_heads, int64_t ld, int64_t k_offset, float eps, void* dst,
+                              int64_t dst_ld, int hpb, int64_t dst_bs, float* kpart, hipStream_t stream) {
+    auto launch = [&](auto kb, auto rope) {
+        constexpr int rows = decltype(kb)::value ? QKN_ROWS : 1;
+        const dim3 grid((unsigned)((n_rows + rows - 1) / rows)), block(256);
+        qknorm_rope_kernel<decltype(kb)::value, decltype(rope)::value, rows><<<grid, block, 0, stream>>>(
+            (bf16_t*)qkv, (const bf16_t*)q_weight, (const bf16_t*)k_weight, cos_tab, sin_tab, n_rows, n_rope, n_heads, ld, k_offset, eps,
+            (bf16_t*)dst, dst_ld, hpb, dst_bs, kpart);
+    };
+    if (kpart)
+        n_rope > 0 ? launch(std::true_type{}, std::true_type{}) : launch(std::true_type{}, std::false_type{});
+    else
+        n_rope > 0 ? launch(std::false_type{}, std::true_type{}) : launch(std::false_type{}, std::false_type{});
+    return hv_check_launch();
 }
 
 extern "C" int hv_qknorm_rope_bf16(void* qkv, const void* q_weight, const void* k_weight, const float* cos_tab,
@@ -267,10 +333,21 @@
         n_rope > n_rows || (ld & 7) || (k_offset & 7) || (n_rope > 0 && (!cos_tab || !sin_tab)))
         return HV_ERR_ARG;
     if (n_rows == 0) return HV_OK;
-    qknorm_rope_kernel<<<dim3((unsigned)n_rows), dim3(256), 0, stream>>>((bf16_t*)qkv, (const bf16_t*)q_weight,
-                                                                          (const bf16_t*)k_weight, cos_tab, sin_tab, n_rows,
-                                                                          n_rope, n_heads, ld, k_offset, eps, nullptr, 0, 1, 0);
-    return hv_check_launch();
+    return qknorm_rope_launch(qkv, q_weight, k_weight, cos_tab, sin_tab, n_rows, n_rope, n_heads, ld, k_offset, eps, nullptr, 0, 1, 0,
+                              nullptr, stream);
+}
+
+extern "C" int hv_qknorm_rope_kbound_bf16(void* qkv, const void* q_weight, const void* k_weight, const float* cos_tab,
+                                          const float* sin_tab, int64_t n_rows, int64_t n_rope, int n_heads, int head_dim,
+                                          int64_t ld, int64_t k_offset, float eps, float* kpart, int64_t kpart_blocks,
+                                          hipStream_t stream) {
+    if (!qkv || !q_weight || !k_weight || head_dim != 128 || n_heads <= 0 || n_heads > HV_ATTN_BOUND_MAX_HEADS || n_rows < 0 ||
+        n_rope < 0 || n_rope > n_rows || (ld & 7) || (k_offset & 7) || (n_rope > 0 && (!cos_tab || !sin_tab)) || !kpart ||
+        kpart_blocks < (n_rows + QKN_ROWS - 1) / QKN_ROWS)
+        return HV_ERR_ARG;
+    if (n_rows == 0) return HV_OK;
+    return qknorm_rope_launch(qkv, q_weight, k_weight, cos_tab, sin_tab, n_rows, n_rope, n_heads, ld, k_offset, eps, nullptr, 0, 1, 0,
+                              kpart, stream);
 }
 
 extern "C" int hv_qknorm_rope_scatter_bf16(const void* qkv, const void* q_weight, const void* k_weight, const float* cos_tab,
@@ -282,11 +359,8 @@
         (n_rope > 0 && (!cos_tab || !sin_tab)))
         return HV_ERR_ARG;
     if (n_rows == 0) return HV_OK;
-    qknorm_rope_kernel<<<dim3((unsigned)n_rows), dim3(256), 0, stream>>>((bf16_t*)const_cast<void*>(qkv), (const bf16_t*)q_weight,
-                                                                          (const bf16_t*)k_weight, cos_tab, sin_tab, n_rows, n_rope,
-                                                                          n_heads, ld, k_offset, eps, (bf16_t*)dst, dst_ld,
-                                                                          heads_per_block, dst_block_stride);
-    return hv_check_launch();
+    return qknorm_rope_launch(const_cast<void*>(qkv), q_weight, k_weight, cos_tab, sin_tab, n_rows, n_rope, n_heads, ld, k_offset, eps,
+                              dst, dst_ld, heads_per_block, dst_block_stride, nullptr, stream);
 }
 
 template <int MM>
diff --git a/hunyuanvideo_efficiency_amd/csrc/hv_torch_ops.cpp b/hunyuanvideo_efficiency_amd/csrc/hv_torch_ops.cpp
--- a/hunyuanvideo_efficiency_amd/csrc/hv_torch_ops.cpp
+++ b/hunyuanvideo_efficiency_amd/csrc/hv_torch_ops.cpp
@@ -69,6 +69,20 @@
     check_rc(hv_qknorm_rope_scatter_bf16(a0, a1, a2, a3, a4, (int64_t)n_rows, (int64_t)n_rope, (int)n_heads, (int)head_dim, (int64_t)ld, (int64_t)k_offset, (float)eps, a12, (int64_t)dst_ld, (int)heads_per_block, (int64_t)dst_block_stride, stream), "qknorm_rope_scatter_bf16");
 }
 
+void op_qknorm_rope_kbound_bf16(const OptT& qkv, const OptT& q_weight, const OptT& k_weight, const OptT& cos_tab, const OptT& sin_tab, int64_t n_rows, int64_t n_rope, int64_t n_heads, int64_t head_dim, int64_t ld, int64_t k_offset, double eps, const OptT& kpart, int64_t kpart_blocks) {
+    Dev dev("qknorm_rope_kbound_bf16");
+    auto a0 = (void*)dev.p(qkv, "qkv");
+    auto a1 = (const void*)dev.p(q_weight, "q_weight");
+    auto a2 = (const void*)dev.p(k_weight, "k_weight");
+    auto a3 = (const float*)dev.p(cos_tab, "cos_tab");
+    auto a4 = (const float*)dev.p(sin_tab, "sin_tab");
+    auto a12 = (float*)dev.p(kpart, "kpart");
+    TORCH_CHECK(dev.idx >= 0, "hv::qknorm_rope_kbound_bf16: needs at least one GPU tensor");
+    c10::hip::HIPGuard guard(dev.idx);
+    hipStream_t stream = c10::hip::getCurrentHIPStream(dev.idx).stream();
+    check_rc(hv_qknorm_rope_kbound_bf16(a0, a1, a2, a3, a4, (int64_t)n_rows, (int64_t)n_rope, (int)n_heads, (int)head_dim, (int64_t)ld, (int64_t)k_offset, (float)eps, a12, (int64_t)kpart_blocks, stream), "qknorm_rope_kbound_bf16");
+}
+
 void op_gemm_bf16(const OptT& A, int64_t lda, const OptT& W, int64_t ldw, const OptT& bias, int64_t M, int64_t N, int64_t K, const OptT& out0, int64_t ld0, int64_t act0, int64_t n_split, const OptT& out1, int64_t ld1, int64_t act1, const OptT& gate, const OptT& res, int64_t ld_res) {
     Dev dev("gemm_bf16");
     auto a0 = (const void*)dev.p(A, "A");
@@ -118,6 +132,29 @@
     c10::hip::HIPGuard guard(dev.idx);
     hipStream_t stream = c10::hip::getCurrentHIPStream(dev.idx).stream();
     check_rc(hv_attn_fwd_bf16(a0, a1, a2, a3, (int64_t)stride_q, (int64_t)stride_k, (int64_t)stride_v, (int64_t)stride_o, (int)n_q, (int)n_kv, (int)n_heads, (int)head_dim, (float)scale, a13, (int64_t)workspace_bytes, stream), "attn_fwd_bf16");
+}
+
+void op_attn_kbound_fold(const OptT& kpart, int64_t n_blocks, int64_t n_heads, const OptT& workspace, int64_t workspace_bytes) {
+    Dev dev("attn_kbound_fold");
+    auto a0 = (const float*)dev.p(kpart, "kpart");
+    auto a3 = (void*)dev.p(workspace, "workspace");
+    TORCH_CHECK(dev.idx >= 0, "hv::attn_kbound_fold: needs at least one GPU tensor");
+    c10::hip::HIPGuard guard(dev.idx);
+    hipStream_t stream = c10::hip::getCurrentHIPStream(dev.idx).stream();
+    check_rc(hv_attn_kbound_fold(a0, (int64_t)n_blocks, (int)n_heads, a3, (int64_t)workspace_bytes, stream), "attn_kbound_fold");
+}
+
+void op_attn_fwd_bf16_kbound(const OptT& q, const OptT& k, const OptT& v, const OptT& o, int64_t stride_q, int64_t stride_k, int64_t stride_v, int64_t stride_o, int64_t n_q, int64_t n_kv, int64_t n_heads, int64_t head_dim, double scale, const OptT& workspace, int64_t workspace_bytes) {
+    Dev dev("attn_fwd_bf16_kbound");
+    auto a0 = (const void*)dev.p(q, "q");
+    auto a1 = (const void*)dev.p(k, "k");
+    auto a2 = (const void*)dev.p(v, "v");
+    auto a3 = (void*)dev.p(o, "o");
+    auto a13 = (void*)dev.p(workspace, "workspace");
+    TORCH_CHECK(dev.idx >= 0, "hv::attn_fwd_bf16_kbound: needs at least one GPU tensor");
+    c10::hip::HIPGuard guard(dev.idx);
+    hipStream_t stream = c10::hip::getCurrentHIPStream(dev.idx).stream();
+    check_rc(hv_attn_fwd_bf16_kbound(a0, a1, a2, a3, (int64_t)stride_q, (int64_t)stride_k, (int64_t)stride_v, (int64_t)stride_o, (int)n_q, (int)n_kv, (int)n_heads, (int)head_dim, (float)scale, a13, (int64_t)workspace_bytes, stream), "attn_fwd_bf16_kbound");
 }
 
 int64_t op_attn_workspace_bytes(int64_t n_q, int64_t n_kv, int64_t n_heads) {
@@ -612,10 +649,13 @@
     m.def("ln_modulate_bf16(Tensor? x, Tensor? shift_or_bias, Tensor? scale_or_weight, Tensor(a!)? out, int M, int D, int ldx, int ldo, float eps, int mode) -> ()");
     m.def("qknorm_rope_bf16(Tensor(a!)? qkv, Tensor? q_weight, Tensor? k_weight, Tensor? cos_tab, Tensor? sin_tab, int n_rows, int n_rope, int n_heads, int head_dim, int ld, int k_offset, float eps) -> ()");
     m.def("qknorm_rope_scatter_bf16(Tensor? qkv, Tensor? q_weight, Tensor? k_weight, Tensor? cos_tab, Tensor? sin_tab, int n_rows, int n_rope, int n_heads, int head_dim, int ld, int k_offset, float eps, Tensor(a!)? dst, int dst_ld, int heads_per_block, int dst_block_stride) -> ()");
+    m.def("qknorm_rope_kbound_bf16(Tensor(a!)? qkv, Tensor? q_weight, Tensor? k_weight, Tensor? cos_tab, Tensor? sin_tab, int n_rows, int n_rope, int n_heads, int head_dim, int ld, int k_offset, float eps, Tensor(b!)? kpart, int kpart_blocks) -> ()");
     m.def("gemm_bf16(Tensor? A, int lda, Tensor? W, int ldw, Tensor? bias, int M, int N, int K, Tensor(a!)? out0, int ld0, int act0, int n_split, Tensor(b!)? out1, int ld1, int act1, Tensor? gate, Tensor? res, int ld_res) -> ()");
     m.def("linear_smallm_bf16(Tensor? x, Tensor? W, Tensor? bias, Tensor? addend, Tensor(a!)? out, int M, int N, int K, int ldx, int ldo, int act) -> ()");
     m.def("timestep_embedding_bf16(Tensor? t, Tensor(a!)? out, int n_t, int dim, float max_period) -> ()");
     m.def("attn_fwd_bf16(Tensor? q, Tensor? k, Tensor? v, Tensor(a!)? o, int stride_q, int stride_k, int stride_v, int stride_o, int n_q, int n_kv, int n_heads, int head_dim, float scale, Tensor(b!)? workspace, int workspace_bytes) -> ()");
+    m.def("attn_kbound_fold(Tensor? kpart, int n_blocks, int n_heads, Tensor(a!)? workspace, int workspace_bytes) -> ()");
+    m.def("attn_fwd_bf16_kbound(Tensor? q, Tensor? k, Tensor? v, Tensor(a!)? o, int stride_q, int stride_k, int stride_v, int stride_o, int n_q, int n_kv, int n_heads, int head_dim, float scale, Tensor(b!)? workspace, int workspace_bytes) -> ()");
     m.def("attn_workspace_bytes(int n_q, int n_kv, int n_heads) -> int");
     m.def("attn_w4_loop_signature() -> int");
     m.def("attn_partial_bf16(Tensor? q, Tensor? k, Tensor? v, int stride_q, int stride_k, int stride_v, int n_q, int n_kv, int n_heads, int head_dim, float scale, Tensor(a!)? part_o, Tensor(b!)? part_ml, int n_slots, int slot, int splits) -> ()");
@@ -669,10 +709,13 @@
     m.impl("ln_modulate_bf16", &op_ln_modulate_bf16);
     m.impl("qknorm_rope_bf16", &op_qknorm_rope_bf16);
     m.impl("qknorm_rope_scatter_bf16", &op_qknorm_rope_scatter_bf16);
+    m.impl("qknorm_rope_kbound_bf16", &op_qknorm_rope_kbound_bf16);
     m.impl("gemm_bf16", &op_gemm_bf16);
     m.impl("linear_smallm_bf16", &op_linear_smallm_bf16);
     m.impl("timestep_embedding_bf16", &op_timestep_embedding_bf16);
     m.impl("attn_fwd_bf16", &op_attn_fwd_bf16);
+    m.impl("attn_kbound_fold", &op_attn_kbound_fold);
+    m.impl("attn_fwd_bf16_kbound", &op_attn_fwd_bf16_kbound);
     m.impl("attn_partial_bf16", &op_attn_partial_bf16);
     m.impl("attn_merge_bf16", &op_attn_merge_bf16);
     m.impl("patchify_f32_bf16", &op_patchify_f32_bf16);
diff --git a/hunyuanvideo_efficiency_amd/modules/attenion.py b/hunyuanvideo_efficiency_amd/modules/attenion.py
--- a/hunyuanvideo_efficiency_amd/modules/attenion.py
+++ b/hunyuanvideo_efficiency_amd/modules/attenion.py
@@ -66,11 +66,15 @@
     return out
 
 
-def segment_attention_(hybrid_seq_parallel_attn, qkv: torch.Tensor, cat: torch.Tensor, s_img: int, cu1: int, heads: int, d: int):
+def segment_attention_(hybrid_seq_parallel_attn, qkv: torch.Tensor, cat: torch.Tensor, s_img: int, cu1: int, heads: int, d: int,
+                       kbound=None):
     s = qkv.shape[0]
     q, k, v, o = qkv[:, :d], qkv[:, d:2 * d], qkv[:, 2 * d:], cat[:, :d]
     if hybrid_seq_parallel_attn is None:
-        if cu1 > 0:
+        if kbound is not None:
+            ops.attn_kbound_fold(kbound[0], kbound[1], cu1, cu1, heads)
+            ops.attn_fwd(q[:cu1], k[:cu1], v[:cu1], o[:cu1], heads, kbound=True)
+        elif cu1 > 0:
             ops.attn_fwd(q[:cu1], k[:cu1], v[:cu1], o[:cu1], heads)
     else:
         hybrid_seq_parallel_attn.run_fused(qkv, cat, s_img, cu1, heads, d)
diff --git a/hunyuanvideo_efficiency_amd/modules/models.py b/hunyuanvideo_efficiency_amd/modules/models.py
--- a/hunyuanvideo_efficiency_amd/modules/models.py
+++ b/hunyuanvideo_efficiency_amd/modules/models.py
@@ -35,6 +35,20 @@
             self.catq = torch.empty(s, self.cat.shape[1], dtype=torch.float8_e4m3fn, device=dev)
             self.cats = torch.empty(s, dtype=torch.float32, device=dev)
         return self
+
+
+class _KBound:
+
+    def __init__(self, n0: int, n1: int, device):
+        self.nb = (ops.kbound_blocks(n0), ops.kbound_blocks(n1))
+        self.parts = ops.kbound_partials(sum(self.nb), device)
+
+    def rows(self, i: int):
+        lo = self.nb[0] if i else 0
+        return self.parts[lo:lo + self.nb[i]]
+
+    def folded(self):
+        return self.parts, sum(self.nb)
 
 
 def _use_fp8_mfma(block, *layers) -> bool:
@@ -122,6 +136,7 @@
         mods = {}
         fp8 = {s: _use_fp8_mfma(self, getattr(self, f"{s}_attn_qkv"), getattr(self, f"{s}_attn_proj"), getattr(self, f"{s}_mlp").fc1,
                                 getattr(self, f"{s}_mlp").fc2) for s in ("img", "txt")}
+        kb = _KBound(cu1 - s_img, s_img, ws.qkv.device) if sp is None and ops.kbound_applies(cu1, H) else None
         for s, lo, hi, n_rope in streams:
             mod = getattr(self, f"{s}_mod")
             m = ops.linear_smallm(vec, mod.linear.w(), mod.linear.bias, silu_in=True)
@@ -134,13 +149,21 @@
                 _sp_chunked_qkv(sp, ws, qkv_l, fp8[s], qw, kw, cos, sin, s_img, cu1, n_rope, H, d)
             else:
                 _gemm(ws, qkv_l, "xmod", lo, hi, fp8[s], out=ws.qkv[lo:hi])
-                ops.qknorm_rope_(ws.qkv[lo:hi], qw, kw, cos, sin, n_rope, H, d)
+                if kb is None:
+                    ops.qknorm_rope_(ws.qkv[lo:hi], qw, kw, cos, sin, n_rope, H, d)
+                elif s == "img":
+                    ops.qknorm_rope_(ws.qkv[lo:hi], qw, kw, cos, sin, n_rope, H, d, kbound=kb.rows(1))
+                else:
+                    if cu1 > lo:
+                        ops.qknorm_rope_(ws.qkv[lo:cu1], qw, kw, cos, sin, n_rope, H, d, kbound=kb.rows(0))
+                    if hi > cu1:
+                        ops.qknorm_rope_(ws.qkv[cu1:hi], qw, kw, cos, sin, n_rope, H, d)
         segs = None
         if overlap:
             segs = sp.attend_async(ws.cat, ws.cat.stride(0))
             pad_segment_attention_(ws.qkv, ws.cat, cu1, H, d)
         else:
-            segment_attention_(sp, ws.qkv, ws.cat, s_img, cu1, H, d)
+            segment_attention_(sp, ws.qkv, ws.cat, s_img, cu1, H, d, kbound=None if kb is None else kb.folded())
         streams = (streams[1], streams[0])
         for s, lo, hi, _ in streams:
             _, _, g1, sh2, sc2, g2 = mods[s]
@@ -222,8 +245,15 @@
             return
         else:
             _gemm(ws, self.linear1, "xmod", 0, s_all, fp8, out=ws.qkv, n_split=3 * d, out1=ws.cat[:, d:], act1=ops.ACT_GELU_TANH)
-            ops.qknorm_rope_(ws.qkv, self.q_norm.weight, self.k_norm.weight, cos, sin, n_rope, H, d)
-            segment_attention_(sp, ws.qkv, ws.cat, s_img, cu1, H, d)
+            if sp is None and ops.kbound_applies(cu1, H):
+                kb = _KBound(cu1, 0, ws.qkv.device)
+                ops.qknorm_rope_(ws.qkv[:cu1], self.q_norm.weight, self.k_norm.weight, cos, sin, n_rope, H, d, kbound=kb.rows(0))
+                if s_all > cu1:
+                    ops.qknorm_rope_(ws.qkv[cu1:], self.q_norm.weight, self.k_norm.weight, None, None, 0, H, d)
+                segment_attention_(sp, ws.qkv, ws.cat, s_img, cu1, H, d, kbound=kb.folded())
+            else:
+                ops.qknorm_rope_(ws.qkv, self.q_norm.weight, self.k_norm.weight, cos, sin, n_rope, H, d)
+                segment_attention_(sp, ws.qkv, ws.cat, s_img, cu1, H, d)
         _gemm(ws, self.linear2, "cat", 0, s_all, fp8, out=ws.x, gate=gate, res=ws.x)
 
     def forward(self, x, vec, txt_len, cu_seqlens_q=None, cu_seqlens_kv=None, max_seqlen_q=None, max_seqlen_kv=None,
diff --git a/hunyuanvideo_efficiency_amd/ops.py b/hunyuanvideo_efficiency_amd/ops.py
--- a/hunyuanvideo_efficiency_amd/ops.py
+++ b/hunyuanvideo_efficiency_amd/ops.py
@@ -55,13 +55,39 @@
     return out
 
 
-def qknorm_rope_(qkv, q_weight, k_weight, cos, sin, n_rope: int, n_heads: int, k_offset: int, eps: float = 1e-6, out=None):
+QKNORM_ROWS = _abi.MACROS["HV_QKNORM_ROWS_PER_BLOCK"]
+ATTN_BOUND_MAX_HEADS = _abi.MACROS["HV_ATTN_BOUND_MAX_HEADS"]
+_kbound_parts = {}
+
+
+def kbound_applies(n_kv: int, n_heads: int) -> bool:
+    return n_kv >= _abi.MACROS["HV_ATTN_BOUND_MIN_KV"] and n_heads <= ATTN_BOUND_MAX_HEADS
+
+
+def kbound_blocks(n_rows: int) -> int:
+    return -(-n_rows // QKNORM_ROWS)
+
+
+def kbound_partials(n_blocks: int, device):
+    dev = torch.device(device)
+    dev = torch.device(dev.type, torch.cuda.current_device() if dev.index is None else dev.index)
+    key = (str(dev), torch.cuda.current_stream(dev).cuda_stream)
+    buf = _kbound_parts.get(key)
+    if buf is None or buf.shape[0] < n_blocks:
+        buf = torch.empty(n_blocks, ATTN_BOUND_MAX_HEADS, dtype=torch.float32, device=dev)
+        _kbound_parts[key] = buf
+    return buf
+
+
+def qknorm_rope_(qkv, q_weight, k_weight, cos, sin, n_rope: int, n_heads: int, k_offset: int, eps: float = 1e-6, out=None,
+                 kbound=None):
     _chk(qkv, BF16, "qkv")
     n, _, ld = _rows(qkv, "qkv")
     _chk(q_weight, BF16, "q_weight"), _chk(k_weight, BF16, "k_weight")
     if n_rope > 0:
         _chk(cos, torch.float32, "cos"), _chk(sin, torch.float32, "sin")
         assert cos.is_contiguous() and sin.is_contiguous() and cos.shape[-1] == 128 and cos.shape[0] >= n_rope
+    assert out is None or kbound is None, "the scatter form leaves no key-norm partials"
     if out is not None:
         _chk(out, BF16, "out", False)
         assert out.dim() == 3 and out.shape[0] == n and out.stride(2) == 1 and out.shape[2] % 128 == 0
@@ -69,6 +95,12 @@
         _lib.call("qknorm_rope_scatter_bf16", qkv, q_weight, k_weight, cos, sin, n, n_rope, n_heads, 128, ld, k_offset, eps,
                   out, out.stride(0), out.shape[2] // 128, out.stride(1))
         return out
+    if kbound is not None:
+        _chk(kbound, torch.float32, "kbound")
+        assert kbound.dim() == 2 and kbound.shape[1] == ATTN_BOUND_MAX_HEADS and kbound.is_contiguous()
+        _lib.call("qknorm_rope_kbound_bf16", qkv, q_weight, k_weight, cos, sin, n, n_rope, n_heads, 128, ld, k_offset, eps,
+                  kbound, kbound.shape[0])
+        return qkv
     _lib.call("qknorm_rope_bf16", qkv, q_weight, k_weight, cos, sin, n,
                                                n_rope, n_heads, 128, ld, k_offset, eps)
     return qkv
@@ -152,7 +184,13 @@
     return ws
 
 
-def attn_fwd(q, k, v, out, n_heads: int, scale: Optional[float] = None, kv_split_workspace: bool = True):
+def attn_kbound_fold(parts, n_blocks: int, n_q: int, n_kv: int, n_heads: int):
+    assert kbound_applies(n_kv, n_heads) and 1 <= n_blocks <= parts.shape[0]
+    ws = _attn_workspace(n_q, n_kv, n_heads, parts.device)
+    _lib.call("attn_kbound_fold", parts, n_blocks, n_heads, ws, ws.numel())
+
+
+def attn_fwd(q, k, v, out, n_heads: int, scale: Optional[float] = None, kv_split_workspace: bool = True, kbound: bool = False):
     for t, nm in ((q, "q"), (k, "k"), (v, "v"), (out, "out")):
         _chk(t, BF16, nm)
         assert t.dim() == 2
@@ -164,8 +202,9 @@
     if prof is not None:
         e0, e1 = torch.cuda.Event(enable_timing=True), torch.cuda.Event(enable_timing=True)
         e0.record()
+    assert kv_split_workspace or not kbound
     ws = _attn_workspace(n_q, n_kv, n_heads, q.device) if kv_split_workspace else None
-    _lib.call("attn_fwd_bf16", q, k, v, out, q.stride(0), k.stride(0), v.stride(0),
+    _lib.call("attn_fwd_bf16_kbound" if kbound else "attn_fwd_bf16", q, k, v, out, q.stride(0), k.stride(0), v.stride(0),
                                             out.stride(0), n_q, n_kv, n_heads, 128, scale, ws,
                                             0 if ws is None else ws.numel())
     if prof is not None:
diff --git a/include/hv_kernels.h b/include/hv_kernels.h
--- a/include/hv_kernels.h
+++ b/include/hv_kernels.h
@@ -11,7 +11,7 @@
 typedef struct ihipStream_t* hipStream_t;
 #endif
 
-#define HV_ABI_VERSION 10
+#define HV_ABI_VERSION 11
 int hv_abi_version(void);
 
 int hv_ln_modulate_bf16(const void* x, const void* shift_or_bias, const void* scale_or_weight, void* out,
@@ -25,6 +25,12 @@
                                 const float* sin_tab, int64_t n_rows, int64_t n_rope, int n_heads, int head_dim, int64_t ld,
                                 int64_t k_offset, float eps, void* dst, int64_t dst_ld, int heads_per_block,
                                 int64_t dst_block_stride, hipStream_t stream);
+
+#define HV_QKNORM_ROWS_PER_BLOCK 8
+#define HV_ATTN_BOUND_MAX_HEADS 62
+int hv_qknorm_rope_kbound_bf16(void* qkv, const void* q_weight, const void* k_weight, const float* cos_tab,
+                               const float* sin_tab, int64_t n_rows, int64_t n_rope, int n_heads, int head_dim,
+                               int64_t ld, int64_t k_offset, float eps, float* kpart, int64_t kpart_blocks, hipStream_t stream);
 
 int hv_gemm_bf16(const void* A, int64_t lda, const void* W, int64_t ldw, const void* bias, int M, int N, int K,
                  void* out0, int64_t ld0, int act0, int n_split, void* out1, int64_t ld1, int act1,
@@ -40,6 +46,13 @@
 int hv_attn_fwd_bf16(const void* q, const void* k, const void* v, void* o, int64_t stride_q, int64_t stride_k,
                      int64_t stride_v, int64_t stride_o, int n_q, int n_kv, int n_heads, int head_dim,
                      float scale, void* workspace, int64_t workspace_bytes, hipStream_t stream);
+
+int hv_attn_kbound_fold(const float* kpart, int64_t n_blocks, int n_heads, void* workspace, int64_t workspace_bytes,
+                        hipStream_t stream);
+
+int hv_attn_fwd_bf16_kbound(const void* q, const void* k, const void* v, void* o, int64_t stride_q, int64_t stride_k,
+                            int64_t stride_v, int64_t stride_o, int n_q, int n_kv, int n_heads, int head_dim,
+                            float scale, void* workspace, int64_t workspace_bytes, hipStream_t stream);
 
 int64_t hv_attn_workspace_bytes(int n_q, int n_kv, int n_heads);
 int hv_attn_w4_loop_signature(void);
```

Result: no change. 0.1218, median of 6 (+0.1%).
